# fabiojbg/LLMApiGateway

Measured on NVIDIA B200. Metric: sse_chunks_per_sec, higher is better.
Workload: dtype u8

## Files before the change

### llmapigateway_b200/csrc/lgw_engine.cu

```cuda
#include <cuda_runtime.h>
#include <stdio.h>
#include <string.h>
#include <string>
#include <vector>

#include "../../include/llmgw_b200.h"
#include "stream_machine.cuh"
#include "sse_kernels.cuh"
#include "rollup.cuh"
#include "body_kernels.cuh"
#include "doc_kernels.cuh"
#include "transcript.cuh"

using namespace lgw;

static_assert(sizeof(Val) == sizeof(lgw_val), "lgw_val layout");
static_assert(sizeof(UsageRec) == sizeof(lgw_usage_rec), "lgw_usage_rec layout");
static_assert(sizeof(StreamState) == sizeof(lgw_stream_state), "lgw_stream_state layout");
static_assert(sizeof(RowEvent) == sizeof(lgw_row_event), "lgw_row_event layout");
static_assert(sizeof(SegResult) == sizeof(lgw_seg_result), "lgw_seg_result layout");
static_assert(sizeof(RollupRow) == sizeof(lgw_rollup_row), "lgw_rollup_row layout");
static_assert(sizeof(DocUsage) == sizeof(lgw_doc_usage), "lgw_doc_usage layout");
static_assert(sizeof(TextMark) == sizeof(lgw_text_mark), "lgw_text_mark layout");

static thread_local std::string g_create_error;

struct lgw_engine {
    int device = 0;
    lgw_limits lim{};
    cudaStream_t own_stream = nullptr, stream = nullptr;
    cudaStream_t s_in = nullptr, s_out = nullptr;
    cudaEvent_t ev_in[16]{}, ev_k[16]{};
    DeviceTables t{};
    uint32_t* d_rowq_count = nullptr;
    RowEvent* d_rowq = nullptr;
    StepScratch scratch{};
    uint8_t *d_in = nullptr, *d_out = nullptr;
    uint32_t *d_chunk_off = nullptr, *d_seg_chunk = nullptr, *d_seg_slot = nullptr;
    SegResult* d_seg_out = nullptr;
    uint32_t* d_slots = nullptr; int32_t* d_status = nullptr; StreamState* d_state_stage = nullptr;
    cudaEvent_t ev[7]{};
    cudaEvent_t rev[4]{};
    float rms[2]{0, 0};
    RollupRow* d_rows = nullptr; uint64_t d_rows_cap = 0; unsigned long long* d_nrows = nullptr;
    uint8_t* d_partial = nullptr; size_t d_partial_cap = 0; uint32_t* d_tiles = nullptr; uint32_t d_tiles_cap = 0;
    bool rollup_attr_set = false, rollup_force_global = false;
    uint8_t* d_details = nullptr; size_t d_details_cap = 0;
    bool last_direct = false;
    float ms[5]{0, 0, 0, 0, 0};
    bool timed = false;
    uint64_t launches = 0;
    BodyPlan* d_plans = nullptr; BodyOp* d_ops = nullptr; uint8_t* d_blob = nullptr; uint32_t n_plans = 0, n_ops = 0;
    uint8_t *b_in = nullptr, *b_slots = nullptr, *b_out = nullptr, *b_models = nullptr;
    uint64_t *b_off = nullptr, *b_out_off = nullptr; uint32_t* b_plan_idx = nullptr; BodyResult* b_results = nullptr; BodyScan* b_scans = nullptr;
    uint64_t b_in_cap = 0, b_slots_cap = 0, b_out_cap = 0, b_n_cap = 0, b_models_cap = 0, b_redo_cap = 0;
    uint32_t* b_redo = nullptr;
    int body_mode = 0;
    cudaEvent_t bev[4]{};
    float bms[3]{0, 0, 0};
    bool per_kernel_timing = false;
    bool kernel_times_valid = false;
    int mode = 0;
    int sm_count = 148;
    bool text_on = false, text_pending = false, text_ready = false;
    TextTap* d_tap = nullptr; uint8_t* d_tcarry = nullptr; uint8_t* d_tsparse = nullptr; uint8_t* d_ttext = nullptr;
    uint32_t *d_piece_len = nullptr, *d_tseg_len = nullptr, *d_tseg_flags = nullptr, *d_markq_count = nullptr;
    unsigned long long* d_tseg_off = nullptr; TextMark* d_markq = nullptr;
    uint64_t text_total = 0; uint32_t text_marks = 0;
    cudaEvent_t tev[2]{}; float tms = 0;
    const uint8_t* last_bytes = nullptr; const uint32_t *last_chunk_off = nullptr, *last_seg_chunk = nullptr, *last_seg_slot = nullptr;
    const SegResult* last_seg_out = nullptr; uint32_t last_n_chunks = 0, last_n_segs = 0; uint64_t last_n_bytes = 0;
    std::string err;
};

#define CK(e, call) do { cudaError_t _r = (call); if (_r != cudaSuccess) { \
    (e)->err = std::string(#call) + ": " + cudaGetErrorString(_r); return LGW_ERR_CUDA; } } while (0)

extern "C" int lgw_abi_version(void) { return LGW_ABI_VERSION; }

extern "C" const char* lgw_last_error(const lgw_engine* e) { return e ? e->err.c_str() : g_create_error.c_str(); }

extern "C" int lgw_engine_create(int device, const lgw_limits* limits, lgw_engine** out) {
    if (!out || !limits) { g_create_error = "null argument"; return LGW_ERR_ARG; }
    int n = 0;
    if (cudaGetDeviceCount(&n) != cudaSuccess || n <= 0 || device < 0 || device >= n) {
        g_create_error = "no usable CUDA device (this engine has no CPU path)";
        return LGW_ERR_NO_DEVICE;
    }
    lgw_engine* e = new lgw_engine();
    e->device = device; e->lim = *limits;
    if (e->lim.max_streams == 0 || e->lim.carry_cap < 64 || e->lim.detail_cap < 64 || e->lim.max_step_chunks == 0 || e->lim.max_step_bytes == 0) {
        g_create_error = "limits out of range"; delete e; return LGW_ERR_ARG;
    }
    auto fail = [&](const char* what, cudaError_t r) { g_create_error = std::string(what) + ": " + cudaGetErrorString(r); lgw_engine_destroy(e); return LGW_ERR_CUDA; };
    cudaError_t r;
    if ((r = cudaSetDevice(device)) != cudaSuccess) return fail("cudaSetDevice", r);
    cudaDeviceProp prop;
    if ((r = cudaGetDeviceProperties(&prop, device)) != cudaSuccess) return fail("cudaGetDeviceProperties", r);
    e->sm_count = prop.multiProcessorCount;
    if ((r = cudaStreamCreateWithFlags(&e->own_stream, cudaStreamNonBlocking)) != cudaSuccess) return fail("cudaStreamCreate", r);
    e->stream = e->own_stream;
    if ((r = cudaStreamCreateWithFlags(&e->s_in, cudaStreamNonBlocking)) != cudaSuccess) return fail("cudaStreamCreate", r);
    if ((r = cudaStreamCreateWithFlags(&e->s_out, cudaStreamNonBlocking)) != cudaSuccess) return fail("cudaStreamCreate", r);
    for (int i = 0; i < 16; ++i) { if ((r = cudaEventCreateWithFlags(&e->ev_in[i], cudaEventDisableTiming)) != cudaSuccess) return fail("cudaEventCreate", r); if ((r = cudaEventCreateWithFlags(&e->ev_k[i], cudaEventDisableTiming)) != cudaSuccess) return fail("cudaEventCreate", r); }
    for (auto& ev : e->ev) if ((r = cudaEventCreate(&ev)) != cudaSuccess) return fail("cudaEventCreate", r);
    for (auto& ev : e->rev) if ((r = cudaEventCreate(&ev)) != cudaSuccess) return fail("cudaEventCreate", r);
    for (auto& ev : e->bev) if ((r = cudaEventCreate(&ev)) != cudaSuccess) return fail("cudaEventCreate", r);
    const size_t S = e->lim.max_streams, C = e->lim.max_step_chunks, B = e->lim.max_step_bytes;
#define ALLOC(ptr, bytes) if ((r = cudaMalloc((void**)&(ptr), (bytes))) != cudaSuccess) return fail("cudaMalloc " #ptr, r)
    ALLOC(e->t.state, S * sizeof(StreamState));
    ALLOC(e->t.carry_a, S * (size_t)e->lim.carry_cap);
    ALLOC(e->t.carry_b, S * (size_t)e->lim.carry_cap);
    ALLOC(e->t.detail, S * (size_t)e->lim.detail_cap);
    ALLOC(e->t.pending, S * (size_t)LGW_PENDING_STRIDE);
    e->t.carry_cap = e->lim.carry_cap; e->t.detail_cap = e->lim.detail_cap; e->t.max_streams = e->lim.max_streams;
    ALLOC(e->d_rowq, (size_t)(e->lim.rowq_cap + 1) * sizeof(RowEvent));
    ALLOC(e->d_rowq_count, 16);
    ALLOC(e->d_in, B + 64); ALLOC(e->d_out, B + 64);
    ALLOC(e->d_chunk_off, (C + 1) * 4); ALLOC(e->d_seg_chunk, (S + 1) * 4); ALLOC(e->d_seg_slot, S * 4);
    ALLOC(e->d_seg_out, S * sizeof(SegResult));
    ALLOC(e->d_slots, S * 4); ALLOC(e->d_status, S * 4); ALLOC(e->d_state_stage, S * sizeof(StreamState));
    if ((r = scratch_alloc(e->scratch, S, B, e->sm_count)) != cudaSuccess) return fail("scratch_alloc", r);
#undef ALLOC
    if ((r = cudaMemset(e->t.state, 0, S * sizeof(StreamState))) != cudaSuccess) return fail("cudaMemset", r);
    if ((r = cudaMemset(e->d_rowq_count, 0, 16)) != cudaSuccess) return fail("cudaMemset", r);
    const char* m = getenv("LGW_FORCE_GENERAL");
    e->mode = (m && m[0] == '1') ? 1 : 0;
    *out = e;
    return LGW_OK;
}

extern "C" int lgw_engine_destroy(lgw_engine* e) {
    if (!e) return LGW_OK;
    cudaSetDevice(e->device);
    cudaFree(e->t.state); cudaFree(e->t.carry_a); cudaFree(e->t.carry_b); cudaFree(e->t.detail); cudaFree(e->t.pending);
    cudaFree(e->d_rowq); cudaFree(e->d_rowq_count); cudaFree(e->d_in); cudaFree(e->d_out);
    cudaFree(e->d_chunk_off); cudaFree(e->d_seg_chunk); cudaFree(e->d_seg_slot); cudaFree(e->d_seg_out);
    cudaFree(e->d_slots); cudaFree(e->d_status); cudaFree(e->d_state_stage);
    scratch_free(e->scratch);
    for (auto& ev : e->ev) if (ev) cudaEventDestroy(ev);
    for (auto& ev : e->rev) if (ev) cudaEventDestroy(ev);
    cudaFree(e->d_rows); cudaFree(e->d_nrows); cudaFree(e->d_partial); cudaFree(e->d_tiles); cudaFree(e->d_details);
    cudaFree(e->d_plans); cudaFree(e->d_ops); cudaFree(e->d_blob);
    cudaFree(e->b_in); cudaFree(e->b_slots); cudaFree(e->b_out); cudaFree(e->b_models); cudaFree(e->b_off); cudaFree(e->b_out_off);
    cudaFree(e->b_plan_idx); cudaFree(e->b_results); cudaFree(e->b_scans); cudaFree(e->b_redo);
    for (auto& ev : e->bev) if (ev) cudaEventDestroy(ev);
    cudaFree(e->d_tap); cudaFree(e->d_tcarry); cudaFree(e->d_tsparse); cudaFree(e->d_ttext); cudaFree(e->d_piece_len); cudaFree(e->d_tseg_len);
    cudaFree(e->d_tseg_flags); cudaFree(e->d_markq_count); cudaFree(e->d_tseg_off); cudaFree(e->d_markq);
    for (auto& ev : e->tev) if (ev) cudaEventDestroy(ev);
    for (int i = 0; i < 16; ++i) { if (e->ev_in[i]) cudaEventDestroy(e->ev_in[i]); if (e->ev_k[i]) cudaEventDestroy(e->ev_k[i]); }
    if (e->s_in) cudaStreamDestroy(e->s_in);
    if (e->s_out) cudaStreamDestroy(e->s_out);
    if (e->own_stream) cudaStreamDestroy(e->own_stream);
    delete e;
    return LGW_OK;
}

extern "C" int lgw_engine_set_stream(lgw_engine* e, void* s) {
    if (!e) return LGW_ERR_ARG;
    e->stream = s ? (cudaStream_t)s : e->own_stream;
    return LGW_OK;
}

extern "C" int lgw_engine_set_kernel_timing(lgw_engine* e, int on) {
    if (!e) return LGW_ERR_ARG;
    e->per_kernel_timing = on != 0;
    return LGW_OK;
}

extern "C" int lgw_engine_set_mode(lgw_engine* e, int mode) {
    if (!e) return LGW_ERR_ARG;
    e->mode = mode; e->body_mode = mode;
    return LGW_OK;
}

extern "C" int lgw_streams_open(lgw_engine* e, const uint32_t* slots, const int32_t* http_status, uint32_t n) {
    if (!e || !slots || !http_status) return LGW_ERR_ARG;
    if (n == 0) return LGW_OK;
    if (n > e->lim.max_streams) { e->err = "more slots than max_streams"; return LGW_ERR_CAPACITY; }
    for (uint32_t i = 0; i < n; ++i) if (slots[i] >= e->lim.max_streams) { e->err = "slot out of range"; return LGW_ERR_ARG; }
    CK(e, cudaSetDevice(e->device));
    CK(e, cudaMemcpyAsync(e->d_slots, slots, n * 4, cudaMemcpyHostToDevice, e->stream));
    CK(e, cudaMemcpyAsync(e->d_status, http_status, n * 4, cudaMemcpyHostToDevice, e->stream));
    k_streams_open<<<(n + 127) / 128, 128, 0, e->stream>>>(e->t, e->d_slots, e->d_status, n);
    ++e->launches;
    if (e->text_on) { k_text_open<<<(n + 127) / 128, 128, 0, e->stream>>>(e->d_tap, e->d_slots, n); ++e->launches; }
    CK(e, cudaGetLastError());
    CK(e, cudaStreamSynchronize(e->stream));
    return LGW_OK;
}

static int gather_states(lgw_engine* e, const uint32_t* slots, uint32_t n, lgw_stream_state* out, int free_after) {
    if (!e || !slots || !out) return LGW_ERR_ARG;
    if (n == 0) return LGW_OK;
    if (n > e->lim.max_streams) { e->err = "more slots than max_streams"; return LGW_ERR_CAPACITY; }
    for (uint32_t i = 0; i < n; ++i) if (slots[i] >= e->lim.max_streams) { e->err = "slot out of range"; return LGW_ERR_ARG; }
    CK(e, cudaSetDevice(e->device));
    CK(e, cudaMemcpyAsync(e->d_slots, slots, n * 4, cudaMemcpyHostToDevice, e->stream));
    k_streams_gather<<<(n + 127) / 128, 128, 0, e->stream>>>(e->t, e->d_slots, n, e->d_state_stage, free_after);
    ++e->launches;
    CK(e, cudaGetLastError());
    CK(e, cudaMemcpyAsync(out, e->d_state_stage, n * sizeof(StreamState), cudaMemcpyDeviceToHost, e->stream));
    CK(e, cudaStreamSynchronize(e->stream));
    return LGW_OK;
}

extern "C" int lgw_streams_state(lgw_engine* e, const uint32_t* slots, uint32_t n, lgw_stream_state* out) { return gather_states(e, slots, n, out, 0); }
extern "C" int lgw_streams_close(lgw_engine* e, const uint32_t* slots, uint32_t n, lgw_stream_state* out) { return gather_states(e, slots, n, out, 1); }

extern "C" int lgw_stream_detail(lgw_engine* e, uint32_t slot, uint8_t* buf, uint32_t cap, uint32_t* len) {
    if (!e || !buf || !len || slot >= e->lim.max_streams) return LGW_ERR_ARG;
    CK(e, cudaSetDevice(e->device));
    StreamState st;
    CK(e, cudaMemcpyAsync(&st, e->t.state + slot, sizeof(st), cudaMemcpyDeviceToHost, e->stream));
    CK(e, cudaStreamSynchronize(e->stream));
    uint32_t n = st.h.detail_len < cap ? st.h.detail_len : cap;
    if (n) CK(e, cudaMemcpyAsync(buf, e->t.detail + (size_t)slot * e->lim.detail_cap, n, cudaMemcpyDeviceToHost, e->stream));
    CK(e, cudaStreamSynchronize(e->stream));
    *len = n;
    return LGW_OK;
}

namespace lgw {
__global__ void k_details_gather(DeviceTables t, const uint32_t* slots, uint32_t n, uint8_t* out, uint32_t stride, uint32_t* lens) {
    const uint32_t w = (blockIdx.x * blockDim.x + threadIdx.x) >> 5, lane = threadIdx.x & 31;
    if (w >= n) return;
    const uint32_t slot = slots[w];
    uint32_t len = t.state[slot].h.detail_len;
    if (len > t.detail_cap) len = t.detail_cap;
    if (len > stride) len = stride;
    const uint8_t* src = t.detail + (size_t)slot * t.detail_cap;
    uint8_t* dst = out + (size_t)w * stride;
    for (uint32_t i = lane; i < len; i += 32) dst[i] = src[i];
    if (lane == 0) lens[w] = len;
}
}

extern "C" int lgw_streams_details(lgw_engine* e, const uint32_t* slots, uint32_t n, uint8_t* buf, uint32_t stride, uint32_t* lens) {
    if (!e || (n && (!slots || !buf || !lens)) || stride == 0) return LGW_ERR_ARG;
    if (n == 0) return LGW_OK;
    for (uint32_t i = 0; i < n; ++i) if (slots[i] >= e->lim.max_streams) return LGW_ERR_ARG;
    CK(e, cudaSetDevice(e->device));
    const size_t need = (size_t)n * 8 + (size_t)n * stride;
    if (need > e->d_details_cap) {
        cudaFree(e->d_details); e->d_details = nullptr; e->d_details_cap = 0;
        CK(e, cudaMalloc((void**)&e->d_details, need + need / 2));
        e->d_details_cap = need + need / 2;
    }
    uint32_t* d_slots = (uint32_t*)e->d_details; uint32_t* d_lens = d_slots + n; uint8_t* d_out = e->d_details + (size_t)n * 8;
    CK(e, cudaMemcpyAsync(d_slots, slots, (size_t)n * 4, cudaMemcpyHostToDevice, e->stream));
    lgw::k_details_gather<<<(n * 32 + 255) / 256, 256, 0, e->stream>>>(e->t, d_slots, n, d_out, stride, d_lens);
    ++e->launches;
    CK(e, cudaMemcpyAsync(lens, d_lens, (size_t)n * 4, cudaMemcpyDeviceToHost, e->stream));
    CK(e, cudaMemcpyAsync(buf, d_out, (size_t)n * stride, cudaMemcpyDeviceToHost, e->stream));
    CK(e, cudaStreamSynchronize(e->stream));
    return LGW_OK;
}

static int step_device(lgw_engine* e, const uint8_t* d_bytes, uint64_t n_bytes, const uint32_t* d_chunk_off, uint32_t n_chunks,
                       const uint32_t* d_seg_chunk, const uint32_t* d_seg_slot, uint32_t n_segs,
                       uint8_t* d_out, SegResult* d_seg_out,
                       uint32_t s0 = 0, uint32_t s1 = 0xFFFFFFFFu, uint32_t c0 = 0, uint32_t c1 = 0xFFFFFFFFu,
                       uint32_t b0 = 0, uint64_t b1 = ~0ull, bool reset_rows = true) {
    if (n_segs > e->lim.max_streams || n_chunks > e->lim.max_step_chunks || n_bytes > e->lim.max_step_bytes) {
        e->err = "step exceeds the limits given to lgw_engine_create"; return LGW_ERR_CAPACITY;
    }
    if (n_bytes >= 0xFFFF0000ull) { e->err = "step larger than 4 GiB - 64 KiB"; return LGW_ERR_CAPACITY; }
    if (s1 == 0xFFFFFFFFu) { s1 = n_segs; c1 = n_chunks; b1 = n_bytes; }
    StepArgs a{};
    a.t = e->t; a.data = d_bytes; a.n_bytes = (uint32_t)b1; a.chunk_off = d_chunk_off; a.n_chunks = n_chunks;
    a.tile_base = b0; a.chunk_lo = c0; a.chunk_hi = c1;
    a.seg_chunk = d_seg_chunk + s0; a.seg_slot = d_seg_slot + s0; a.n_segs = s1 - s0; a.out = d_out; a.seg_out = d_seg_out + s0;
    a.rowq = e->d_rowq; a.rowq_count = e->d_rowq_count; a.rowq_cap = e->lim.rowq_cap; a.s = e->scratch;
    if (reset_rows) CK(e, cudaMemsetAsync(e->d_rowq_count, 0, 4, e->stream));
    int launched = 0;
    const bool pk = e->per_kernel_timing || e->mode == 1;
    cudaError_t r = launch_step(a, e->mode, e->sm_count, e->stream, e->ev, &launched, pk);
    e->kernel_times_valid = pk;
    e->launches += (uint64_t)launched;
    if (r != cudaSuccess) { e->err = std::string("step launch: ") + cudaGetErrorString(r); return LGW_ERR_CUDA; }
    e->timed = true;
    return LGW_OK;
}

extern "C" int lgw_sse_step_device(lgw_engine* e, const uint8_t* d_bytes, uint64_t n_bytes, const uint32_t* d_chunk_off, uint32_t n_chunks,
                                   const uint32_t* d_seg_chunk, const uint32_t* d_seg_slot, uint32_t n_segs,
                                   uint8_t* d_out, lgw_seg_result* d_seg_out) {
    if (!e || (!d_bytes && n_bytes) || !d_chunk_off || !d_seg_chunk || !d_seg_slot || (!d_out && n_bytes) || !d_seg_out) return LGW_ERR_ARG;
    CK(e, cudaSetDevice(e->device));
    e->last_bytes = d_bytes; e->last_n_bytes = n_bytes; e->last_chunk_off = d_chunk_off; e->last_n_chunks = n_chunks;
    e->last_seg_chunk = d_seg_chunk; e->last_seg_slot = d_seg_slot; e->last_n_segs = n_segs; e->last_seg_out = (const SegResult*)d_seg_out;
    e->text_pending = e->text_on; e->text_ready = false;
    return step_device(e, d_bytes, n_bytes, d_chunk_off, n_chunks, d_seg_chunk, d_seg_slot, n_segs, d_out, (SegResult*)d_seg_out);
}

extern "C" int lgw_fetch_rows(lgw_engine* e, lgw_row_event* rows_out, uint32_t rows_cap, uint32_t* n_rows) {
    if (!e || !n_rows || (!rows_out && rows_cap)) return LGW_ERR_ARG;
    CK(e, cudaSetDevice(e->device));
    uint32_t cnt = 0;
    CK(e, cudaMemcpyAsync(&cnt, e->d_rowq_count, 4, cudaMemcpyDeviceToHost, e->stream));
    CK(e, cudaStreamSynchronize(e->stream));
    if (cnt > e->lim.rowq_cap) cnt = e->lim.rowq_cap;
    if (cnt > rows_cap) cnt = rows_cap;
    if (cnt) CK(e, cudaMemcpyAsync(rows_out, e->d_rowq, (size_t)cnt * sizeof(RowEvent), cudaMemcpyDeviceToHost, e->stream));
    CK(e, cudaStreamSynchronize(e->stream));
    *n_rows = cnt;
    return LGW_OK;
}

extern "C" int lgw_sync(lgw_engine* e) {
    if (!e) return LGW_ERR_ARG;
    CK(e, cudaSetDevice(e->device));
    CK(e, cudaStreamSynchronize(e->stream));
    return LGW_OK;
}

extern "C" int lgw_sse_step(lgw_engine* e, const uint8_t* bytes, uint64_t n_bytes, const uint32_t* chunk_off, uint32_t n_chunks,
                            const uint32_t* seg_chunk, const uint32_t* seg_slot, uint32_t n_segs,
                            uint8_t* out_bytes, lgw_seg_result* seg_out, lgw_row_event* rows_out, uint32_t rows_cap, uint32_t* n_rows) {
    if (!e || (!bytes && n_bytes) || !chunk_off || !seg_chunk || !seg_slot || !seg_out || !n_rows) return LGW_ERR_ARG;
    if (n_segs > e->lim.max_streams || n_chunks > e->lim.max_step_chunks || n_bytes > e->lim.max_step_bytes) {
        e->err = "step exceeds the limits given to lgw_engine_create"; return LGW_ERR_CAPACITY;
    }
    if (chunk_off[0] != 0 || chunk_off[n_chunks] != n_bytes) { e->err = "chunk_off must start at 0 and end at n_bytes"; return LGW_ERR_ARG; }
    if (n_segs && (seg_chunk[0] != 0 || seg_chunk[n_segs] != n_chunks)) { e->err = "seg_chunk must cover all chunks"; return LGW_ERR_ARG; }
    for (uint32_t s = 0; s < n_segs; ++s) if (seg_chunk[s] > seg_chunk[s + 1] || seg_slot[s] >= e->lim.max_streams) { e->err = "bad segment table"; return LGW_ERR_ARG; }
    CK(e, cudaSetDevice(e->device));
    CK(e, cudaEventRecord(e->ev[5], e->stream));
    static const int allow = [] { const char* v = getenv("LGW_DIRECT"); if (!v || v[0] == '0') return 0; if (v[0] == 'b') return 3; if (v[0] == 'o') return 2; return 1; }();
    static const bool trace = [] { const char* v = getenv("LGW_TRACE"); return v && v[0] == '1'; }();
    const uint8_t* direct_in = nullptr; uint8_t* direct_out = nullptr;
    {
        cudaPointerAttributes pa{};
        const bool big = e->mode == 0 && n_bytes >= (1u << 20);
        if (big && (allow & 1) && ((uintptr_t)bytes & 15) == 0 && cudaPointerGetAttributes(&pa, bytes) == cudaSuccess && pa.type == cudaMemoryTypeHost && pa.devicePointer)
            direct_in = (const uint8_t*)pa.devicePointer;
        if (big && out_bytes && (allow & 2) && ((uintptr_t)out_bytes & 15) == 0 && cudaPointerGetAttributes(&pa, out_bytes) == cudaSuccess && pa.type == cudaMemoryTypeHost && pa.devicePointer)
            direct_out = (uint8_t*)pa.devicePointer;
        cudaGetLastError();
        e->last_direct = direct_in || direct_out;
    }
    e->last_bytes = direct_in ? direct_in : e->d_in; e->last_n_bytes = n_bytes; e->last_chunk_off = e->d_chunk_off; e->last_n_chunks = n_chunks;
    e->last_seg_chunk = e->d_seg_chunk; e->last_seg_slot = e->d_seg_slot; e->last_n_segs = n_segs; e->last_seg_out = e->d_seg_out;
    e->text_pending = e->text_on; e->text_ready = false;
    uint32_t n_slices = n_bytes >= (8u << 20) && n_segs >= 16 ? 8u : 1u;
    if (direct_in && direct_out) n_slices = 1;
    if (const char* sl = getenv("LGW_SLICES")) { int v = atoi(sl); if (v >= 1 && v <= 14) n_slices = (uint32_t)v; }
    if (e->mode == 1 || n_segs < n_slices) n_slices = 1;
    uint32_t cut[18]; cut[0] = 0;
    for (uint32_t j = 1; j < n_slices; ++j) {
        const uint64_t want = n_bytes * j / n_slices;
        uint32_t lo = cut[j - 1], hi = n_segs;
        while (lo < hi) { const uint32_t mid = (lo + hi) >> 1; if ((uint64_t)chunk_off[seg_chunk[mid]] < want) lo = mid + 1; else hi = mid; }
        cut[j] = lo;
    }
    cut[n_slices] = n_segs;
    CK(e, cudaMemsetAsync(e->d_rowq_count, 0, 4, e->stream));
    const bool piped = n_slices > 1;
    cudaStream_t sin = piped ? e->s_in : e->stream, sout = piped ? e->s_out : e->stream;
    if (piped) { CK(e, cudaEventRecord(e->ev_k[15], e->stream)); CK(e, cudaStreamWaitEvent(sin, e->ev_k[15], 0)); }
    {
        const uint32_t s1 = cut[1], c1 = seg_chunk[s1];
        CK(e, cudaMemcpyAsync(e->d_chunk_off, chunk_off, (size_t)(c1 + 1) * 4, cudaMemcpyHostToDevice, sin));
        CK(e, cudaMemcpyAsync(e->d_seg_chunk, seg_chunk, (size_t)(n_segs + 1) * 4, cudaMemcpyHostToDevice, sin));
        if (n_segs) CK(e, cudaMemcpyAsync(e->d_seg_slot, seg_slot, (size_t)n_segs * 4, cudaMemcpyHostToDevice, sin));
    }
    cudaEvent_t tr[3][16]; float tms[3][16];
    if (trace) for (int k = 0; k < 3; ++k) for (uint32_t j = 0; j < n_slices; ++j) cudaEventCreate(&tr[k][j]);
    int rc = LGW_OK;
    for (uint32_t j = 0; j < n_slices; ++j) {
        const uint32_t s0 = cut[j], s1 = cut[j + 1];
        if (s1 <= s0 && piped) continue;
        const uint32_t c0 = seg_chunk[s0], c1 = seg_chunk[s1];
        const uint32_t b0 = chunk_off[c0]; const uint64_t b1 = chunk_off[c1];
        if (!direct_in && b1 > b0) CK(e, cudaMemcpyAsync(e->d_in + b0, bytes + b0, b1 - b0, cudaMemcpyHostToDevice, sin));
        if (piped && (j == 0 || !direct_in)) { CK(e, cudaEventRecord(e->ev_in[j], sin)); CK(e, cudaStreamWaitEvent(e->stream, e->ev_in[j], 0)); }
        if (trace) cudaEventRecord(tr[0][j], sin);
        if (j == 0 && n_slices > 1 && n_chunks > seg_chunk[cut[1]]) {
            const uint32_t cc = seg_chunk[cut[1]];
            CK(e, cudaMemcpyAsync(e->d_chunk_off + cc + 1, chunk_off + cc + 1, (size_t)(n_chunks - cc) * 4, cudaMemcpyHostToDevice, sin));
            if (direct_in) { CK(e, cudaEventRecord(e->ev_in[1], sin)); CK(e, cudaStreamWaitEvent(e->stream, e->ev_in[1], 0)); }
        }
        rc = step_device(e, direct_in ? direct_in : e->d_in, n_bytes, e->d_chunk_off, n_chunks, e->d_seg_chunk, e->d_seg_slot, n_segs,
                         direct_out ? direct_out : e->d_out, e->d_seg_out, s0, s1, c0, c1, b0, b1, false);
        if (rc != LGW_OK) return rc;
        if (trace) cudaEventRecord(tr[1][j], e->stream);
        if (!direct_out) {
            if (piped) { CK(e, cudaEventRecord(e->ev_k[j], e->stream)); CK(e, cudaStreamWaitEvent(sout, e->ev_k[j], 0)); }
            if (b1 > b0 && out_bytes) CK(e, cudaMemcpyAsync(out_bytes + b0, e->d_out + b0, b1 - b0, cudaMemcpyDeviceToHost, sout));
        }
        if (trace) cudaEventRecord(tr[2][j], sout);
    }
    if (n_segs) CK(e, cudaMemcpyAsync(seg_out, e->d_seg_out, (size_t)n_segs * sizeof(SegResult), cudaMemcpyDeviceToHost, e->stream));
    if (piped) {
        CK(e, cudaEventRecord(e->ev_k[14], sout)); CK(e, cudaStreamWaitEvent(e->stream, e->ev_k[14], 0));
        CK(e, cudaEventRecord(e->ev_in[15], sin)); CK(e, cudaStreamWaitEvent(e->stream, e->ev_in[15], 0));
    }
    CK(e, cudaEventRecord(e->ev[6], e->stream));
    rc = lgw_fetch_rows(e, rows_out, rows_cap, n_rows);
    if (rc != LGW_OK) return rc;
    if (piped) { CK(e, cudaStreamSynchronize(e->s_out)); CK(e, cudaStreamSynchronize(e->s_in)); }
    float t = 0; if (cudaEventElapsedTime(&t, e->ev[5], e->ev[6]) == cudaSuccess) e->ms[4] = t;
    if (trace) {
        cudaDeviceSynchronize();
        fprintf(stderr, "[lgw trace] direct_in=%d direct_out=%d slices=%u total=%.3f ms; per slice (ms after step start): upload done | kernels done | download done\n", direct_in != nullptr, direct_out != nullptr, n_slices, t);
        for (uint32_t j = 0; j < n_slices; ++j) {
            for (int k = 0; k < 3; ++k) { tms[k][j] = -1; cudaEventElapsedTime(&tms[k][j], e->ev[5], tr[k][j]); cudaEventDestroy(tr[k][j]); }
            fprintf(stderr, "[lgw trace]   %2u  %.3f | %.3f | %.3f\n", j, tms[0][j], tms[1][j], tms[2][j]);
        }
        cudaGetLastError();
    }
    return LGW_OK;
}

static int read_step_ms(lgw_engine* e) {
    if (e->timed) {
        CK(e, cudaSetDevice(e->device));
        CK(e, cudaEventSynchronize(e->ev[4]));
        if (e->kernel_times_valid) {
            for (int i = 0; i < 4; ++i) { float t = 0; if (cudaEventElapsedTime(&t, e->ev[i], e->ev[i + 1]) == cudaSuccess) e->ms[i] = t; }
        } else {
            float t = 0; e->ms[0] = e->ms[2] = e->ms[3] = 0;
            if (cudaEventElapsedTime(&t, e->ev[0], e->ev[4]) == cudaSuccess) e->ms[1] = t;
        }
    }
    return LGW_OK;
}
extern "C" int lgw_last_step_ms(lgw_engine* e, float ms[4]) {
    if (!e || !ms) return LGW_ERR_ARG;
    const int rc = read_step_ms(e);
    if (rc != LGW_OK) return rc;
    ms[0] = e->ms[0]; ms[1] = e->ms[1]; ms[2] = e->ms[2] + e->ms[3]; ms[3] = e->ms[4];
    return LGW_OK;
}
extern "C" int lgw_last_step_kernel_ms(lgw_engine* e, float ms[4]) {
    if (!e || !ms) return LGW_ERR_ARG;
    const int rc = read_step_ms(e);
    if (rc != LGW_OK) return rc;
    for (int i = 0; i < 4; ++i) ms[i] = e->ms[i];
    return LGW_OK;
}

extern "C" int lgw_last_step_direct(lgw_engine* e) { return e && e->last_direct ? 1 : 0; }

extern "C" int lgw_launch_count(lgw_engine* e, uint64_t* out) {
    if (!e || !out) return LGW_ERR_ARG;
    *out = e->launches;
    return LGW_OK;
}

extern "C" int lgw_alloc_pinned(lgw_engine* e, uint64_t bytes, void** out) {
    if (!e || !out) return LGW_ERR_ARG;
    CK(e, cudaSetDevice(e->device));
    CK(e, cudaHostAlloc(out, bytes, cudaHostAllocDefault));
    return LGW_OK;
}
extern "C" int lgw_free_pinned(lgw_engine* e, void* p) {
    if (!e) return LGW_ERR_ARG;
    CK(e, cudaFreeHost(p));
    return LGW_OK;
}

extern "C" int64_t lgw_rollup_bucket_of(int64_t ts_us, int period) { return bucket_of(ts_us, period); }

extern "C" int lgw_usage_rollup_accum(lgw_engine* e, const int64_t* d_ts_us, const int32_t* d_model_rank,
                                      const int32_t* d_prompt, const int32_t* d_completion, const int32_t* d_total,
                                      const int32_t* d_reasoning, const int32_t* d_cached, const double* d_cost, uint64_t n,
                                      int period, int has_start, int64_t start_us, int has_end, int64_t end_us,
                                      int64_t bucket0, uint32_t n_buckets, uint32_t n_models,
                                      uint64_t* d_table, uint32_t* d_inexact, uint32_t* d_oob) {
    if (!e || !d_table || !d_inexact || !d_oob || period < 0 || period > 3 || n_buckets == 0 || n_models == 0) return LGW_ERR_ARG;
    if (n && (!d_ts_us || !d_model_rank || !d_prompt || !d_completion || !d_total || !d_reasoning || !d_cached || !d_cost)) return LGW_ERR_ARG;
    CK(e, cudaSetDevice(e->device));
    RollupArgs a{};
    a.ts_us = d_ts_us; a.model_rank = d_model_rank; a.tok[0] = d_prompt; a.tok[1] = d_completion; a.tok[2] = d_total;
    a.tok[3] = d_reasoning; a.tok[4] = d_cached; a.cost = d_cost; a.n = n; a.period = period;
    a.start_us = start_us; a.end_us = end_us; a.has_start = has_start; a.has_end = has_end;
    a.bucket0 = bucket0; a.n_buckets = n_buckets; a.n_models = n_models;
    a.table = (unsigned long long*)d_table; a.inexact = d_inexact; a.oob = d_oob;
    const uint64_t groups = (uint64_t)n_buckets * n_models;
    const bool privatised = groups <= LGW_ROLLUP_SMEM_GROUPS && n >= 65536 && n < 0xFFFFFFFFull && !e->rollup_force_global;
    if (privatised) {
        const size_t need = (size_t)e->sm_count * groups * (LGW_ROLLUP_CELLS * 8 + 4);
        if (need > e->d_partial_cap) {
            cudaFree(e->d_partial); e->d_partial = nullptr; e->d_partial_cap = 0;
            CK(e, cudaMalloc((void**)&e->d_partial, need));
            e->d_partial_cap = need;
        }
        if (!e->rollup_attr_set) {
            CK(e, cudaFuncSetAttribute(k_rollup_accum_smem, cudaFuncAttributeMaxDynamicSharedMemorySize, (int)rollup_smem_bytes(LGW_ROLLUP_SMEM_GROUPS)));
            e->rollup_attr_set = true;
        }
    }
    CK(e, cudaEventRecord(e->rev[0], e->stream));
    if (n && privatised) {
        const unsigned grid = (unsigned)e->sm_count;
        unsigned long long* partial = (unsigned long long*)e->d_partial;
        uint32_t* pflag = (uint32_t*)(e->d_partial + (size_t)grid * groups * LGW_ROLLUP_CELLS * 8);
        k_rollup_accum_smem<<<grid, 1024, rollup_smem_bytes((uint32_t)groups), e->stream>>>(a, partial, pflag);
        k_rollup_merge<<<dim3((unsigned)((groups * LGW_ROLLUP_CELLS + 255) / 256), LGW_ROLLUP_MERGE_SLICES), 256, 0, e->stream>>>(partial, pflag, grid, (uint32_t)groups, a.table, a.inexact);
        e->launches += 2;
    } else if (n) {
        const uint64_t want = (n + 255) / 256;
        const unsigned grid = (unsigned)(want < (uint64_t)e->sm_count * 16 ? want : (uint64_t)e->sm_count * 16);
        k_rollup_accum<<<grid, 256, 0, e->stream>>>(a);
        ++e->launches;
    }
    CK(e, cudaEventRecord(e->rev[1], e->stream));
    CK(e, cudaGetLastError());
    return LGW_OK;
}

extern "C" int lgw_usage_rollup_emit(lgw_engine* e, const uint64_t* d_table, const uint32_t* d_inexact,
                                     int64_t bucket0, uint32_t n_buckets, uint32_t n_models,
                                     lgw_rollup_row* rows_out, uint64_t rows_cap, uint64_t* n_rows) {
    if (!e || !d_table || !d_inexact || !n_rows || (!rows_out && rows_cap) || n_buckets == 0 || n_models == 0) return LGW_ERR_ARG;
    CK(e, cudaSetDevice(e->device));
    const uint64_t groups = (uint64_t)n_buckets * n_models;
    const uint64_t cap = rows_cap < groups ? rows_cap : groups;
    if (cap > e->d_rows_cap) {
        cudaFree(e->d_rows); e->d_rows = nullptr; e->d_rows_cap = 0;
        CK(e, cudaMalloc((void**)&e->d_rows, (cap ? cap : 1) * sizeof(RollupRow)));
        e->d_rows_cap = cap;
    }
    if (!e->d_nrows) CK(e, cudaMalloc((void**)&e->d_nrows, 8));
    const uint32_t n_tiles = (uint32_t)((groups + 1023) / 1024);
    if (n_tiles > e->d_tiles_cap) {
        cudaFree(e->d_tiles); e->d_tiles = nullptr; e->d_tiles_cap = 0;
        CK(e, cudaMalloc((void**)&e->d_tiles, (size_t)n_tiles * 4));
        e->d_tiles_cap = n_tiles;
    }
    CK(e, cudaEventRecord(e->rev[2], e->stream));
    k_rollup_count<<<n_tiles, 1024, 0, e->stream>>>((const unsigned long long*)d_table, n_buckets, n_models, e->d_tiles);
    k_rollup_scan<<<1, 1024, 0, e->stream>>>(e->d_tiles, n_tiles, e->d_nrows);
    k_rollup_write<<<n_tiles, 1024, 0, e->stream>>>((const unsigned long long*)d_table, d_inexact, n_buckets, n_models, bucket0, e->d_tiles, e->d_rows, cap);
    e->launches += 3;
    CK(e, cudaEventRecord(e->rev[3], e->stream));
    CK(e, cudaGetLastError());
    unsigned long long cnt = 0;
    CK(e, cudaMemcpyAsync(&cnt, e->d_nrows, 8, cudaMemcpyDeviceToHost, e->stream));
    CK(e, cudaStreamSynchronize(e->stream));
    *n_rows = cnt;
    const uint64_t take = cnt < cap ? cnt : cap;
    if (take) CK(e, cudaMemcpyAsync(rows_out, e->d_rows, take * sizeof(RollupRow), cudaMemcpyDeviceToHost, e->stream));
    CK(e, cudaStreamSynchronize(e->stream));
    return LGW_OK;
}

extern "C" int lgw_rollup_set_path(lgw_engine* e, int force_global) {
    if (!e) return LGW_ERR_ARG;
    e->rollup_force_global = force_global != 0;
    return LGW_OK;
}

extern "C" int lgw_rollup_last_ms(lgw_engine* e, float ms[2]) {
    if (!e || !ms) return LGW_ERR_ARG;
    CK(e, cudaSetDevice(e->device));
    cudaEventSynchronize(e->rev[1]); cudaEventSynchronize(e->rev[3]);
    float t = 0;
    if (cudaEventElapsedTime(&t, e->rev[0], e->rev[1]) == cudaSuccess) e->rms[0] = t;
    if (cudaEventElapsedTime(&t, e->rev[2], e->rev[3]) == cudaSuccess) e->rms[1] = t;
    ms[0] = e->rms[0]; ms[1] = e->rms[1];
    return LGW_OK;
}

extern "C" int lgw_transcripts_enable(lgw_engine* e) {
    if (!e) return LGW_ERR_ARG;
    if (e->text_on) return LGW_OK;
    CK(e, cudaSetDevice(e->device));
    const size_t S = e->lim.max_streams, C = e->lim.max_step_chunks, B = e->lim.max_step_bytes, cc = e->lim.carry_cap;
    CK(e, cudaMalloc((void**)&e->d_tap, S * sizeof(TextTap)));
    CK(e, cudaMemset(e->d_tap, 0, S * sizeof(TextTap)));
    CK(e, cudaMalloc((void**)&e->d_tcarry, S * cc));
    CK(e, cudaMalloc((void**)&e->d_tsparse, 2 * (B + S * cc) + 64));
    CK(e, cudaMalloc((void**)&e->d_ttext, 2 * (B + S * cc) + 64));
    CK(e, cudaMalloc((void**)&e->d_piece_len, (C + 1) * 4));
    CK(e, cudaMalloc((void**)&e->d_tseg_len, (S + 1) * 4));
    CK(e, cudaMalloc((void**)&e->d_tseg_flags, (S + 1) * 4));
    CK(e, cudaMalloc((void**)&e->d_tseg_off, (S + 2) * 8));
    CK(e, cudaMalloc((void**)&e->d_markq, (size_t)(e->lim.rowq_cap + 1) * sizeof(TextMark)));
    CK(e, cudaMalloc((void**)&e->d_markq_count, 16));
    for (auto& ev : e->tev) CK(e, cudaEventCreate(&ev));
    e->text_on = true;
    return LGW_OK;
}

extern "C" int lgw_step_transcript_run(lgw_engine* e, uint64_t* text_bytes, uint32_t* n_marks) {
    if (!e || !text_bytes || !n_marks) return LGW_ERR_ARG;
    if (!e->text_on) { e->err = "transcripts are not enabled (lgw_transcripts_enable)"; return LGW_ERR_ARG; }
    if (!e->text_pending) { e->err = "no step to tap (the transcript pass runs once after each lgw_sse_step / lgw_sse_step_device)"; return LGW_ERR_ARG; }
    CK(e, cudaSetDevice(e->device));
    e->text_pending = false;
    TextArgs a{};
    a.data = e->last_bytes; a.chunk_off = e->last_chunk_off; a.seg_chunk = e->last_seg_chunk; a.seg_slot = e->last_seg_slot; a.n_segs = e->last_n_segs;
    a.seg_res = e->last_seg_out; a.tap = e->d_tap; a.carry = e->d_tcarry; a.carry_cap = e->lim.carry_cap; a.sparse = e->d_tsparse;
    a.piece_len = e->d_piece_len; a.seg_len = e->d_tseg_len; a.seg_flags = e->d_tseg_flags; a.seg_off = e->d_tseg_off; a.text = e->d_ttext;
    a.markq = e->d_markq; a.markq_count = e->d_markq_count; a.markq_cap = e->lim.rowq_cap;
    CK(e, cudaMemsetAsync(e->d_markq_count, 0, 4, e->stream));
    CK(e, cudaEventRecord(e->tev[0], e->stream));
    const uint32_t n = a.n_segs;
    if (n) {
        k_text_extract<<<(n + TX_WARPS - 1) / TX_WARPS, TX_WARPS * 32, 0, e->stream>>>(a);
        k_text_scan<<<1, 1024, 0, e->stream>>>(a.seg_len, n, a.seg_off);
        k_text_pack<<<(n + TX_WARPS - 1) / TX_WARPS, TX_WARPS * 32, 0, e->stream>>>(a);
        e->launches += 3;
    } else CK(e, cudaMemsetAsync(e->d_tseg_off, 0, 8, e->stream));
    CK(e, cudaEventRecord(e->tev[1], e->stream));
    CK(e, cudaGetLastError());
    unsigned long long total = 0; uint32_t marks = 0;
    CK(e, cudaMemcpyAsync(&total, e->d_tseg_off + n, 8, cudaMemcpyDeviceToHost, e->stream));
    CK(e, cudaMemcpyAsync(&marks, e->d_markq_count, 4, cudaMemcpyDeviceToHost, e->stream));
    CK(e, cudaStreamSynchronize(e->stream));
    if (marks > e->lim.rowq_cap) marks = e->lim.rowq_cap;
    e->text_total = total; e->text_marks = marks; e->text_ready = true;
    float t = 0; if (cudaEventElapsedTime(&t, e->tev[0], e->tev[1]) == cudaSuccess) e->tms = t;
    *text_bytes = total; *n_marks = marks;
    return LGW_OK;
}

extern "C" int lgw_step_transcript_fetch(lgw_engine* e, uint8_t* text_out, uint64_t* seg_text_off, uint32_t* seg_flags, lgw_text_mark* marks_out) {
    if (!e || !seg_text_off || !seg_flags || (!text_out && e->text_total) || (!marks_out && e->text_marks)) return LGW_ERR_ARG;
    if (!e->text_ready) { e->err = "lgw_step_transcript_run has not run for the last step"; return LGW_ERR_ARG; }
    CK(e, cudaSetDevice(e->device));
    const uint32_t n = e->last_n_segs;
    if (e->text_total) CK(e, cudaMemcpyAsync(text_out, e->d_ttext, e->text_total, cudaMemcpyDeviceToHost, e->stream));
    CK(e, cudaMemcpyAsync(seg_text_off, e->d_tseg_off, (size_t)(n + 1) * 8, cudaMemcpyDeviceToHost, e->stream));
    if (n) CK(e, cudaMemcpyAsync(seg_flags, e->d_tseg_flags, (size_t)n * 4, cudaMemcpyDeviceToHost, e->stream));
    if (e->text_marks) CK(e, cudaMemcpyAsync(marks_out, e->d_markq, (size_t)e->text_marks * sizeof(TextMark), cudaMemcpyDeviceToHost, e->stream));
    CK(e, cudaStreamSynchronize(e->stream));
    return LGW_OK;
}

extern "C" int lgw_transcript_last_ms(lgw_engine* e, float* ms) {
    if (!e || !ms) return LGW_ERR_ARG;
    *ms = e->tms;
    return LGW_OK;
}

extern "C" int lgw_device_alloc(lgw_engine* e, uint64_t bytes, void** out) {
    if (!e || !out) return LGW_ERR_ARG;
    CK(e, cudaSetDevice(e->device));
    CK(e, cudaMalloc(out, bytes ? bytes : 1));
    return LGW_OK;
}
extern "C" int lgw_device_free(lgw_engine* e, void* p) { if (!e) return LGW_ERR_ARG; CK(e, cudaSetDevice(e->device)); CK(e, cudaFree(p)); return LGW_OK; }
extern "C" int lgw_device_upload(lgw_engine* e, void* d, const void* h, uint64_t bytes) {
    if (!e || (bytes && (!d || !h))) return LGW_ERR_ARG;
    CK(e, cudaSetDevice(e->device));
    CK(e, cudaMemcpyAsync(d, h, bytes, cudaMemcpyHostToDevice, e->stream)); CK(e, cudaStreamSynchronize(e->stream));
    return LGW_OK;
}
extern "C" int lgw_device_download(lgw_engine* e, void* h, const void* d, uint64_t bytes) {
    if (!e || (bytes && (!d || !h))) return LGW_ERR_ARG;
    CK(e, cudaSetDevice(e->device));
    CK(e, cudaMemcpyAsync(h, d, bytes, cudaMemcpyDeviceToHost, e->stream)); CK(e, cudaStreamSynchronize(e->stream));
    return LGW_OK;
}
extern "C" int lgw_device_zero(lgw_engine* e, void* d, uint64_t bytes) {
    if (!e || (bytes && !d)) return LGW_ERR_ARG;
    CK(e, cudaSetDevice(e->device));
    CK(e, cudaMemsetAsync(d, 0, bytes, e->stream));
    return LGW_OK;
}

#ifdef LGW_DEBUG_TIMING
extern "C" int lgw_debug_read(unsigned long long* out) { return cudaMemcpyFromSymbol(out, lgw::g_dbg, sizeof(unsigned long long) * 16) == cudaSuccess ? 0 : -2; }
#endif


static_assert(sizeof(BodyOp) == sizeof(lgw_body_op), "lgw_body_op");
static_assert(sizeof(BodyPlan) == sizeof(lgw_body_plan), "lgw_body_plan");
static_assert(sizeof(BodyResult) == sizeof(lgw_body_result), "lgw_body_result");
static_assert(sizeof(BodyScan) == sizeof(lgw_body_scan), "lgw_body_scan");

template <class T>
static cudaError_t grow(T*& p, uint64_t& cap, uint64_t need) {
    if (need <= cap && p) return cudaSuccess;
    if (p) { cudaError_t r = cudaFree(p); p = nullptr; cap = 0; if (r != cudaSuccess) return r; }
    const uint64_t n = need + need / 4 + 64;
    cudaError_t r = cudaMalloc((void**)&p, n * sizeof(T));
    if (r == cudaSuccess) cap = n;
    return r;
}

extern "C" int lgw_rules_load(lgw_engine* e, const lgw_body_plan* plans, uint32_t n_plans,
                              const lgw_body_op* ops, uint32_t n_ops, const uint8_t* blob, uint32_t blob_len) {
    if (!e || (n_plans && !plans) || (n_ops && !ops) || (blob_len && !blob)) return LGW_ERR_ARG;
    for (uint32_t i = 0; i < n_plans; ++i) {
        if (plans[i].op_begin > plans[i].op_end || plans[i].op_end > n_ops || plans[i].op_end - plans[i].op_begin > 32 || (plans[i].mode & 0xffu) > 2 || (plans[i].mode & ~0x1ffu)) {
            e->err = "lgw_rules_load: malformed plan"; return LGW_ERR_ARG; }
    }
    for (uint32_t i = 0; i < n_ops; ++i) {
        const lgw_body_op& o = ops[i];
        if ((uint64_t)o.key_off + o.key_len > blob_len || (uint64_t)o.rkey_off + o.rkey_len > blob_len || (uint64_t)o.rval_off + o.rval_len > blob_len) {
            e->err = "lgw_rules_load: op outside the blob"; return LGW_ERR_ARG; }
    }
    CK(e, cudaSetDevice(e->device));
    CK(e, cudaStreamSynchronize(e->stream));
    cudaFree(e->d_plans); cudaFree(e->d_ops); cudaFree(e->d_blob); e->d_plans = nullptr; e->d_ops = nullptr; e->d_blob = nullptr;
    CK(e, cudaMalloc((void**)&e->d_plans, (n_plans + 1) * sizeof(BodyPlan)));
    CK(e, cudaMalloc((void**)&e->d_ops, (n_ops + 1) * sizeof(BodyOp)));
    CK(e, cudaMalloc((void**)&e->d_blob, blob_len + 16));
    if (n_plans) CK(e, cudaMemcpyAsync(e->d_plans, plans, n_plans * sizeof(BodyPlan), cudaMemcpyHostToDevice, e->stream));
    if (n_ops) CK(e, cudaMemcpyAsync(e->d_ops, ops, n_ops * sizeof(BodyOp), cudaMemcpyHostToDevice, e->stream));
    if (blob_len) CK(e, cudaMemcpyAsync(e->d_blob, blob, blob_len, cudaMemcpyHostToDevice, e->stream));
    CK(e, cudaStreamSynchronize(e->stream));
    e->n_plans = n_plans; e->n_ops = n_ops;
    return LGW_OK;
}

static int bodies_stage_in(lgw_engine* e, const uint8_t* bodies, const uint64_t* body_off, uint32_t n) {
    const uint64_t n_bytes = body_off[n];
    for (uint32_t i = 0; i < n; ++i) if (body_off[i + 1] < body_off[i] || body_off[i + 1] - body_off[i] > 0xFFFFFFF0ull) { e->err = "body offsets not monotonic"; return LGW_ERR_ARG; }
    CK(e, grow(e->b_in, e->b_in_cap, n_bytes + 64));
    uint64_t ncap = e->b_n_cap;
    if (n + 1 > e->b_n_cap || !e->b_off) {
        uint64_t c1 = e->b_n_cap, c2 = e->b_n_cap, c3 = e->b_n_cap, c4 = e->b_n_cap, c5 = e->b_n_cap;
        CK(e, grow(e->b_off, c1, n + 1)); CK(e, grow(e->b_out_off, c2, n + 1)); CK(e, grow(e->b_plan_idx, c3, n + 1));
        CK(e, grow(e->b_results, c4, n + 1)); CK(e, grow(e->b_scans, c5, n + 1));
        ncap = c1;
    }
    e->b_n_cap = ncap;
    if (n_bytes) CK(e, cudaMemcpyAsync(e->b_in, bodies, n_bytes, cudaMemcpyHostToDevice, e->stream));
    CK(e, cudaMemcpyAsync(e->b_off, body_off, (n + 1) * sizeof(uint64_t), cudaMemcpyHostToDevice, e->stream));
    return LGW_OK;
}

extern "C" int lgw_bodies_scan(lgw_engine* e, const uint8_t* bodies, const uint64_t* body_off, uint32_t n,
                               uint32_t model_cap, lgw_body_scan* scans_out, uint8_t* models_out) {
    if (!e || !body_off || (!bodies && n && body_off[n]) || !scans_out || (model_cap && !models_out)) return LGW_ERR_ARG;
    if (n == 0) return LGW_OK;
    CK(e, cudaSetDevice(e->device));
    int rc = bodies_stage_in(e, bodies, body_off, n);
    if (rc != LGW_OK) return rc;
    CK(e, grow(e->b_models, e->b_models_cap, (uint64_t)n * model_cap + 16));
    k_body_scan<<<(n + LGW_BODY_WARPS - 1) / LGW_BODY_WARPS, 32 * LGW_BODY_WARPS, 0, e->stream>>>(e->b_in, e->b_off, n, model_cap, e->b_scans, e->b_models);
    ++e->launches;
    CK(e, cudaGetLastError());
    CK(e, cudaMemcpyAsync(scans_out, e->b_scans, n * sizeof(BodyScan), cudaMemcpyDeviceToHost, e->stream));
    if (model_cap) CK(e, cudaMemcpyAsync(models_out, e->b_models, (uint64_t)n * model_cap, cudaMemcpyDeviceToHost, e->stream));
    CK(e, cudaStreamSynchronize(e->stream));
    return LGW_OK;
}

static int bodies_launch(lgw_engine* e, const uint8_t* d_bodies, const uint64_t* d_body_off, uint32_t n, const uint32_t* d_plan_idx,
                         uint32_t slot_cap, uint8_t* d_out, uint64_t out_cap, uint64_t* d_out_off, BodyResult* d_results) {
    if (!e->d_plans) { e->err = "lgw_bodies_rewrite before lgw_rules_load"; return LGW_ERR_ARG; }
    CK(e, grow(e->b_slots, e->b_slots_cap, (uint64_t)n * slot_cap + 64));
    CK(e, grow(e->b_redo, e->b_redo_cap, (uint64_t)n + 4));
    uint32_t* redo_count = e->b_redo + n;
    const uint32_t seq_grid = (n + LGW_BODY_WARPS - 1) / LGW_BODY_WARPS < (uint32_t)e->sm_count * 4u ? (n + LGW_BODY_WARPS - 1) / LGW_BODY_WARPS : (uint32_t)e->sm_count * 4u;
    CK(e, cudaEventRecord(e->bev[0], e->stream));
    if (e->body_mode == 0) {
        CK(e, cudaMemsetAsync(redo_count, 0, 4, e->stream));
        k_body_fast<<<n, LGW_FAST_THREADS, 0, e->stream>>>(d_bodies, d_body_off, n, d_plan_idx, e->d_plans, e->n_plans, e->d_ops, e->d_blob,
                                                             e->b_slots, slot_cap, d_results, redo_count, e->b_redo);
        k_body_rewrite<<<seq_grid, 32 * LGW_BODY_WARPS, 0, e->stream>>>(d_bodies, d_body_off, n, d_plan_idx, e->d_plans, e->n_plans, e->d_ops, e->d_blob,
                                                                        e->b_slots, slot_cap, d_results, redo_count, e->b_redo);
        ++e->launches;
    } else {
        k_body_rewrite<<<seq_grid, 32 * LGW_BODY_WARPS, 0, e->stream>>>(d_bodies, d_body_off, n, d_plan_idx, e->d_plans, e->n_plans, e->d_ops, e->d_blob,
                                                                        e->b_slots, slot_cap, d_results, nullptr, nullptr);
    }
    CK(e, cudaEventRecord(e->bev[1], e->stream));
    k_body_offsets<<<1, 1024, 0, e->stream>>>(d_results, n, out_cap, d_out_off);
    CK(e, cudaEventRecord(e->bev[2], e->stream));
    const uint32_t grid = n < (uint32_t)e->sm_count * 8u ? n : (uint32_t)e->sm_count * 8u;
    k_body_pack<<<grid, 256, 0, e->stream>>>(e->b_slots, slot_cap, d_results, n, d_out_off, d_out, out_cap);
    CK(e, cudaEventRecord(e->bev[3], e->stream));
    e->launches += 3;
    CK(e, cudaGetLastError());
    return LGW_OK;
}

extern "C" int lgw_bodies_rewrite_device(lgw_engine* e, const uint8_t* d_bodies, const uint64_t* d_body_off, uint32_t n, uint64_t n_bytes,
                                         const uint32_t* d_plan_idx, uint32_t slot_cap, uint8_t* d_out, uint64_t out_cap,
                                         uint64_t* d_out_off, lgw_body_result* d_results) {
    (void)n_bytes;
    if (!e || !d_bodies || !d_body_off || !d_plan_idx || !d_out || !d_out_off || !d_results || slot_cap == 0) return LGW_ERR_ARG;
    if (n == 0) return LGW_OK;
    CK(e, cudaSetDevice(e->device));
    return bodies_launch(e, d_bodies, d_body_off, n, d_plan_idx, slot_cap, d_out, out_cap, d_out_off, (BodyResult*)d_results);
}

extern "C" int lgw_bodies_rewrite(lgw_engine* e, const uint8_t* bodies, const uint64_t* body_off, uint32_t n,
                                  const uint32_t* plan_idx, uint32_t slot_cap,
                                  uint8_t* out, uint64_t out_cap, uint64_t* out_off, lgw_body_result* results) {
    if (!e || !body_off || (!bodies && n && body_off[n]) || !plan_idx || (!out && out_cap) || !out_off || !results || slot_cap == 0) return LGW_ERR_ARG;
    if (n == 0) { out_off[0] = 0; return LGW_OK; }
    CK(e, cudaSetDevice(e->device));
    int rc = bodies_stage_in(e, bodies, body_off, n);
    if (rc != LGW_OK) return rc;
    CK(e, cudaMemcpyAsync(e->b_plan_idx, plan_idx, n * sizeof(uint32_t), cudaMemcpyHostToDevice, e->stream));
    CK(e, grow(e->b_out, e->b_out_cap, out_cap + 64));
    rc = bodies_launch(e, e->b_in, e->b_off, n, e->b_plan_idx, slot_cap, e->b_out, out_cap, e->b_out_off, e->b_results);
    if (rc != LGW_OK) return rc;
    CK(e, cudaMemcpyAsync(out_off, e->b_out_off, (n + 1) * sizeof(uint64_t), cudaMemcpyDeviceToHost, e->stream));
    CK(e, cudaMemcpyAsync(results, e->b_results, n * sizeof(BodyResult), cudaMemcpyDeviceToHost, e->stream));
    CK(e, cudaStreamSynchronize(e->stream));
    const uint64_t total = out_off[n] < out_cap ? out_off[n] : out_cap;
    if (total) CK(e, cudaMemcpyAsync(out, e->b_out, total, cudaMemcpyDeviceToHost, e->stream));
    CK(e, cudaStreamSynchronize(e->stream));
    return LGW_OK;
}

extern "C" int lgw_documents_usage(lgw_engine* e, const uint8_t* docs, const uint64_t* doc_off, uint32_t n, lgw_doc_usage* out) {
    if (!e || !doc_off || (!docs && n && doc_off[n]) || (!out && n)) return LGW_ERR_ARG;
    if (n == 0) return LGW_OK;
    CK(e, cudaSetDevice(e->device));
    int rc = bodies_stage_in(e, docs, doc_off, n);
    if (rc != LGW_OK) return rc;
    DocUsage* d_out = nullptr;
    CK(e, cudaMalloc((void**)&d_out, (size_t)n * sizeof(DocUsage)));
    const uint32_t grid = (n + LGW_DOC_WARPS - 1) / LGW_DOC_WARPS < (uint32_t)e->sm_count * 8u ? (n + LGW_DOC_WARPS - 1) / LGW_DOC_WARPS : (uint32_t)e->sm_count * 8u;
    k_docs_usage<<<grid, LGW_DOC_WARPS * 32, 0, e->stream>>>(e->b_in, e->b_off, n, d_out);
    ++e->launches;
    cudaError_t r = cudaGetLastError();
    if (r == cudaSuccess) r = cudaMemcpyAsync(out, d_out, (size_t)n * sizeof(DocUsage), cudaMemcpyDeviceToHost, e->stream);
    if (r == cudaSuccess) r = cudaStreamSynchronize(e->stream);
    cudaFree(d_out);
    if (r != cudaSuccess) { e->err = std::string("lgw_documents_usage: ") + cudaGetErrorString(r); return LGW_ERR_CUDA; }
    return LGW_OK;
}

extern "C" int lgw_documents_error_detail(lgw_engine* e, const uint8_t* docs, const uint64_t* doc_off, uint32_t n, lgw_doc_error* out, uint8_t* text, uint32_t text_stride) {
    if (!e || !doc_off || (!docs && n && doc_off[n]) || (n && (!out || !text)) || text_stride == 0) return LGW_ERR_ARG;
    if (n == 0) return LGW_OK;
    CK(e, cudaSetDevice(e->device));
    int rc = bodies_stage_in(e, docs, doc_off, n);
    if (rc != LGW_OK) return rc;
    DocError* d_out = nullptr; uint8_t* d_text = nullptr;
    CK(e, cudaMalloc((void**)&d_out, (size_t)n * sizeof(DocError)));
    cudaError_t r = cudaMalloc((void**)&d_text, (size_t)n * text_stride);
    if (r == cudaSuccess) {
        const uint32_t grid = (n + LGW_DOC_WARPS - 1) / LGW_DOC_WARPS < (uint32_t)e->sm_count * 8u ? (n + LGW_DOC_WARPS - 1) / LGW_DOC_WARPS : (uint32_t)e->sm_count * 8u;
        k_docs_error_detail<<<grid, LGW_DOC_WARPS * 32, 0, e->stream>>>(e->b_in, e->b_off, n, d_out, d_text, text_stride);
        ++e->launches;
        r = cudaGetLastError();
    }
    if (r == cudaSuccess) r = cudaMemcpyAsync(out, d_out, (size_t)n * sizeof(DocError), cudaMemcpyDeviceToHost, e->stream);
    if (r == cudaSuccess) r = cudaMemcpyAsync(text, d_text, (size_t)n * text_stride, cudaMemcpyDeviceToHost, e->stream);
    if (r == cudaSuccess) r = cudaStreamSynchronize(e->stream);
    cudaFree(d_out); cudaFree(d_text);
    if (r != cudaSuccess) { e->err = std::string("lgw_documents_error_detail: ") + cudaGetErrorString(r); return LGW_ERR_CUDA; }
    return LGW_OK;
}

extern "C" int lgw_bodies_last_ms(lgw_engine* e, float ms[3]) {
    if (!e || !ms) return LGW_ERR_ARG;
    CK(e, cudaSetDevice(e->device));
    cudaEventSynchronize(e->bev[3]);
    for (int i = 0; i < 3; ++i) { float t = 0; if (cudaEventElapsedTime(&t, e->bev[i], e->bev[i + 1]) == cudaSuccess) e->bms[i] = t; ms[i] = e->bms[i]; }
    return LGW_OK;
}

extern "C" int lgw_debug_counters(lgw_engine* e, uint32_t out[4]) {
    if (!e || !out) return LGW_ERR_ARG;
    CK(e, cudaSetDevice(e->device));
    CK(e, cudaStreamSynchronize(e->stream));
    CK(e, cudaMemcpy(out, e->scratch.counters, 16, cudaMemcpyDeviceToHost));
    return LGW_OK;
}

extern "C" int lgw_debug_template_cache(lgw_engine* e, uint32_t out[16], uint8_t* text, uint32_t cap) {
    if (!e || !out) return LGW_ERR_ARG;
    CK(e, cudaSetDevice(e->device));
    CK(e, cudaStreamSynchronize(e->stream));
    std::vector<uint8_t> buf(sizeof(TemplateCache2));
    CK(e, cudaMemcpy(buf.data(), e->scratch.tpl_cache2, sizeof(TemplateCache2), cudaMemcpyDeviceToHost));
    const TemplateCache2* h = reinterpret_cast<const TemplateCache2*>(buf.data());
    for (int i = 0; i < 4; ++i) { out[i] = h->state[i]; out[4 + i] = h->tpl[i].m.len; out[8 + i] = h->tpl[i].m.flags | (h->tpl[i].m.usage_ok << 31); out[12 + i] = h->hits[i]; }
    if (cap > R2_TEXT) cap = R2_TEXT;
    if (text) for (int i = 0; i < 4; ++i) memcpy(text + (size_t)i * cap, h->tpl[i].text, cap);
    return LGW_OK;
}
```

### llmapigateway_b200/csrc/relay2.cuh

```cuda
#pragma once

#if defined(__CUDACC__)
#define R2_DEV __device__ __forceinline__
#define R2_MEM __device__ __forceinline__
#define R2_DEV_NOINLINE __device__ __noinline__
#define R2_GLOBAL __global__
#define R2_TID (threadIdx.x)
#define R2_BID (blockIdx.x)
#define R2_NBLK (gridDim.x)
#define R2_NTHR (blockDim.x)
#define R2_HOST_EMU 0
#else
#define R2_DEV static inline
#define R2_MEM inline
#define R2_DEV_NOINLINE static
#define R2_GLOBAL static
#define R2_TID (simt::tid())
#define R2_BID (simt::bid())
#define R2_NBLK (simt::nblocks())
#define R2_NTHR (simt::nthreads())
#define R2_HOST_EMU 1
#endif

#ifndef R2_WARPS
#define R2_WARPS 16u
#endif
#define R2_THREADS (R2_WARPS * 32u)
#ifndef R2_TILE
#define R2_TILE 3072u
#endif
#ifndef R2_NBUF
#define R2_NBUF 2u
#endif
#define R2_SLOTS 4u
#define R2_TPL_MAX 504u
#define R2_TPL_MIN 16u
#define R2_TEXT 544u
#define R2_SPANS 32u
#define R2_FULL 0xFFFFFFFFu
#define R2_NONE 0xFFFFFFFFu
#define R2_MAX_STR 8192u

struct TplMeta {
    uint32_t len, P, recip, flags, cls, n_spans, usage_ok, full_flags;
    uint16_t sstart[R2_SPANS], send[R2_SPANS];
    uint8_t skind[R2_SPANS];
    uint8_t field_span[8];
};
struct Tpl2 {
    TplMeta m;
    uint8_t text[R2_TEXT];
    uint8_t lit[R2_TEXT];
    uint8_t span_id[R2_TPL_MAX + 8];
};
struct TemplateCache2 {
    uint32_t state[R2_SLOTS];
    uint32_t hits[R2_SLOTS];
    uint32_t general;
    uint32_t lock;
    uint32_t _pad[2];
    Tpl2 tpl[R2_SLOTS];
    UsageRaw raw[R2_SLOTS];
};

struct R2Shared {
    alignas(16) uint8_t fast_text[16 * R2_TEXT];
    alignas(16) uint8_t fast_lit[16 * R2_TEXT];
    alignas(16) Tpl2 tpl[R2_SLOTS];
    alignas(8) UsageRaw raw_tpl[R2_SLOTS];
    alignas(8) unsigned long long mbar[R2_WARPS * R2_NBUF];
    uint32_t slot_state[R2_SLOTS];
    uint32_t slot_gidx[R2_SLOTS];
    uint32_t hits[R2_SLOTS];
    uint32_t general;
    uint32_t dflt, fast_ready;
    uint32_t learn_lock;
    StepArgs args;
    alignas(4) uint8_t cls[256];
    alignas(4) uint8_t trans[LGW_LEAN_ROWS * 32];
};
#define R2_RING_BYTES (R2_WARPS * R2_NBUF * R2_TILE)
#define R2_SMEM_BYTES (R2_RING_BYTES + sizeof(R2Shared) + 128)

#if !R2_HOST_EMU
typedef uint32_t SPtr;
R2_DEV SPtr sptr(const void* p) { return (uint32_t)__cvta_generic_to_shared(p); }
R2_DEV uint4 sld128(SPtr a) { uint4 v; asm volatile("ld.shared.v4.u32 {%0,%1,%2,%3}, [%4];" : "=r"(v.x), "=r"(v.y), "=r"(v.z), "=r"(v.w) : "r"(a)); return v; }
R2_DEV uint32_t sld32(SPtr a) { uint32_t v; asm volatile("ld.shared.u32 %0, [%1];" : "=r"(v) : "r"(a)); return v; }
R2_DEV uint32_t sld8(SPtr a) { uint32_t v; asm volatile("ld.shared.u8 %0, [%1];" : "=r"(v) : "r"(a)); return v; }
R2_DEV void sst8(SPtr a, uint32_t v) { asm volatile("st.shared.u8 [%0], %1;" :: "r"(a), "r"(v) : "memory"); }
R2_DEV uint4 gld128(const uint8_t* p) { uint4 v; asm volatile("ld.global.nc.v4.u32 {%0,%1,%2,%3}, [%4];" : "=r"(v.x), "=r"(v.y), "=r"(v.z), "=r"(v.w) : "l"(p)); return v; }
R2_DEV void mbar_init(SPtr a, uint32_t n) { asm volatile("mbarrier.init.shared::cta.b64 [%0], %1;" :: "r"(a), "r"(n)); }
R2_DEV void mbar_fence_init() { asm volatile("fence.mbarrier_init.release.cluster;" ::: "memory"); }
R2_DEV void mbar_expect(SPtr a, uint32_t bytes) { asm volatile("mbarrier.arrive.expect_tx.shared::cta.b64 _, [%0], %1;" :: "r"(a), "r"(bytes) : "memory"); }
R2_DEV void mbar_wait(SPtr a, uint32_t parity) {
    asm volatile("{\n.reg .pred p;\nWAIT_%=:\nmbarrier.try_wait.parity.shared::cta.b64 p, [%0], %1;\n@p bra DONE_%=;\nbra WAIT_%=;\nDONE_%=:\n}" :: "r"(a), "r"(parity) : "memory");
}
R2_DEV void tma_load(SPtr dst, const void* src, uint32_t bytes, SPtr mbar) {
    asm volatile("cp.async.bulk.shared::cluster.global.mbarrier::complete_tx::bytes [%0], [%1], %2, [%3];" :: "r"(dst), "l"(src), "r"(bytes), "r"(mbar) : "memory");
}
R2_DEV void tma_store(void* dst, SPtr src, uint32_t bytes) {
    asm volatile("fence.proxy.async.shared::cta;\ncp.async.bulk.global.shared::cta.bulk_group [%0], [%1], %2;\ncp.async.bulk.commit_group;" :: "l"(dst), "r"(src), "r"(bytes) : "memory");
}
R2_DEV void tma_store_commit_empty() { asm volatile("cp.async.bulk.commit_group;" ::: "memory"); }
R2_DEV void tma_wait_read1() { asm volatile("cp.async.bulk.wait_group.read 1;" ::: "memory"); }
R2_DEV void tma_wait_all() { asm volatile("cp.async.bulk.wait_group 0;" ::: "memory"); }
R2_DEV uint8_t* smem_base() { extern __shared__ __align__(128) uint8_t r2_smem[]; return r2_smem; }
R2_DEV void griddep_wait() { asm volatile("griddepcontrol.wait;" ::: "memory"); }
R2_DEV void griddep_launch() { asm volatile("griddepcontrol.launch_dependents;" ::: "memory"); }
#else
typedef uint8_t* SPtr;
R2_DEV SPtr sptr(const void* p) { return (uint8_t*)p; }
R2_DEV uint4 sld128(SPtr a) { uint4 v; memcpy(&v, a, 16); return v; }
R2_DEV uint32_t sld32(SPtr a) { uint32_t v; memcpy(&v, a, 4); return v; }
R2_DEV uint32_t sld8(SPtr a) { return *a; }
R2_DEV void sst8(SPtr a, uint32_t v) { *a = (uint8_t)v; }
R2_DEV uint4 gld128(const uint8_t* p) { uint4 v; memcpy(&v, p, 16); return v; }
R2_DEV void mbar_init(SPtr a, uint32_t) { memset(a, 0, 8); }
R2_DEV void mbar_fence_init() {}
R2_DEV void mbar_expect(SPtr, uint32_t) {}
R2_DEV void mbar_wait(SPtr, uint32_t) {}
R2_DEV void tma_load(SPtr dst, const void* src, uint32_t bytes, SPtr) { memcpy(dst, src, bytes); }
R2_DEV void tma_store(void* dst, SPtr src, uint32_t bytes) { memcpy(dst, src, bytes); }
R2_DEV void tma_store_commit_empty() {}
R2_DEV void tma_wait_read1() {}
R2_DEV void tma_wait_all() {}
R2_DEV uint8_t* smem_base() { return simt::g_dyn_smem; }
R2_DEV void griddep_wait() {}
R2_DEV void griddep_launch() {}
#endif
R2_DEV uint32_t r2_min(uint32_t a, uint32_t b) { return a < b ? a : b; }
R2_DEV uint32_t r2_max(uint32_t a, uint32_t b) { return a > b ? a : b; }

R2_DEV uint32_t span_ok(uint32_t w, uint32_t m) {
    const uint32_t w7 = w & 0x7f7f7f7fu;
    const uint32_t a = w7 + 0x60606060u;
    const uint32_t b = (w7 ^ 0x22222222u) + 0x7f7f7f7fu;
    const uint32_t c = (w7 ^ 0x5c5c5c5cu) + 0x7f7f7f7fu;
    return (a & b & c) | w | m;
}
R2_DEV uint32_t nonzero_bytes(uint32_t x) { return (((x & 0x7f7f7f7fu) + 0x7f7f7f7fu) | x) & 0x80808080u; }
R2_DEV uint32_t movemask4(uint32_t m) { return (((m >> 7) * 0x00204081u) >> 21) & 0xFu; }
R2_DEV uint32_t lf_mask16(const uint4& d) {
    const uint32_t a = ~nonzero_bytes(d.x ^ 0x0a0a0a0au) & 0x80808080u, b = ~nonzero_bytes(d.y ^ 0x0a0a0a0au) & 0x80808080u;
    const uint32_t c = ~nonzero_bytes(d.z ^ 0x0a0a0a0au) & 0x80808080u, e = ~nonzero_bytes(d.w ^ 0x0a0a0a0au) & 0x80808080u;
    return movemask4(a) | (movemask4(b) << 4) | (movemask4(c) << 8) | (movemask4(e) << 12);
}

struct R2Ctx {
    const StepArgs* a;
    R2Shared* sh;
    uint32_t lane;
    SPtr ring; SPtr bars;
    uint32_t base;
    uint32_t n_tiles;
    uint32_t k;
    uint32_t tile_lo, tile_hi;
    SPtr buf;
    uint32_t n_bytes;
    uint32_t seg, tb, te, kept_end;
    uint32_t in_kept, primed, kept_tried;
    uint32_t ev_a, ev_b, a_usage;
    uint32_t high;
    uint32_t walk_lo;
    uint32_t t, pos, s_open;
    uint32_t dflt, fast;
    uint32_t ready, free_slots;
    uint32_t last_ra;
    uint32_t hits_d;
    uint32_t single;
};

struct R2Io {
    const uint8_t* data; const R2Shared* sh;
    uint32_t n_bytes, tile_lo, tile_hi; SPtr buf;
};
R2_DEV R2Io io_of(const R2Ctx& c) { R2Io io; io.data = c.a->data; io.sh = c.sh; io.n_bytes = c.n_bytes; io.tile_lo = c.tile_lo; io.tile_hi = c.tile_hi; io.buf = c.buf; return io; }
R2_DEV uint8_t io_byte(const R2Io& io, uint32_t p) {
    if (p >= io.tile_lo && p < io.tile_hi) return (uint8_t)sld8(io.buf + (p - io.tile_lo));
    return p < io.n_bytes ? __ldg(io.data + p) : (uint8_t)0;
}
R2_DEV uint8_t ring_byte(const R2Ctx& c, uint32_t p) {
    if (p >= c.tile_lo && p < c.tile_hi) return (uint8_t)sld8(c.buf + (p - c.tile_lo));
    return p < c.n_bytes ? __ldg(c.a->data + p) : (uint8_t)0;
}
struct R2Bytes {
    R2Io io;
    R2_MEM uint32_t at(uint32_t p) const { return io_byte(io, p); }
    R2_MEM uint32_t cls(uint32_t ch) const { return io.sh->cls[ch]; }
    R2_MEM uint32_t trans(uint32_t i) const { return io.sh->trans[i]; }
};
struct R2Glob {
    const uint8_t* data; uint32_t n_bytes;
    R2_MEM uint32_t at(uint32_t p) const { return p < n_bytes ? (uint32_t)__ldg(data + p) : 0u; }
};
R2_DEV uint4 ld16(const R2Ctx& c, uint32_t p) {
    if (p >= c.tile_lo && p + 16 <= c.tile_hi) return sld128(c.buf + (p - c.tile_lo));
    if (p + 16 <= c.n_bytes) return gld128(c.a->data + p);
    uint32_t w0 = 0, w1 = 0, w2 = 0, w3 = 0;
    for (uint32_t i = 0; i < 16 && p + i < c.n_bytes; ++i) {
        const uint32_t v = (uint32_t)ring_byte(c, p + i) << (8 * (i & 3));
        if (i < 4) w0 |= v; else if (i < 8) w1 |= v; else if (i < 12) w2 |= v; else w3 |= v;
    }
    return make_uint4(w0, w1, w2, w3);
}

R2_DEV uint32_t tile_bytes(const R2Ctx& c, uint32_t k) {
    const uint32_t lo = c.base + k * R2_TILE;
    return c.n_bytes - lo < R2_TILE ? c.n_bytes - lo : R2_TILE;
}
R2_DEV void pipe_issue_load(const R2Ctx& c, uint32_t k) {
    const uint32_t b = k % R2_NBUF, n16 = tile_bytes(c, k) & ~15u;
    if (n16) { mbar_expect(c.bars + 8 * b, n16); tma_load(c.ring + b * R2_TILE, c.a->data + c.base + k * R2_TILE, n16, c.bars + 8 * b); }
}
R2_DEV void pipe_start(R2Ctx& c) {
    c.k = R2_NONE; c.tile_lo = c.tile_hi = c.base; c.buf = c.ring;
    if (c.lane == 0) for (uint32_t k = 0; k < R2_NBUF - 1 && k < c.n_tiles; ++k) pipe_issue_load(c, k);
}
struct PipeState { uint32_t k, tile_lo, tile_hi; SPtr buf; };
R2_DEV PipeState pipe_advance_impl(const StepArgs* ap, SPtr ring, SPtr bars, uint32_t base, uint32_t n_tiles, uint32_t n_bytes, uint32_t k_prev, uint32_t lane) {
    const uint32_t k = k_prev == R2_NONE ? 0u : k_prev + 1u;
    __syncwarp();
    const uint32_t lo = base + k * R2_TILE;
    const uint32_t b = k % R2_NBUF, nb = n_bytes - lo < R2_TILE ? n_bytes - lo : R2_TILE, n16 = nb & ~15u;
    PipeState ps; ps.k = k; ps.tile_lo = lo; ps.tile_hi = lo + nb; ps.buf = ring + b * R2_TILE;
    if (n16) mbar_wait(bars + 8 * b, (k / R2_NBUF) & 1u);
    if (nb != n16) {
        const uint32_t i = n16 + lane;
        if (lane < 16) {
            const uint32_t v = i < nb ? (uint32_t)__ldg(ap->data + lo + i) : 0u;
            sst8(ps.buf + i, v);
            if (i < nb) ap->out[lo + i] = (uint8_t)v;
        }
        __syncwarp();
    }
    if (lane == 0) {
        if (n16) tma_store(ap->out + lo, ps.buf, n16); else tma_store_commit_empty();
        tma_wait_read1();
        const uint32_t kn = k + R2_NBUF - 1;
        if (kn < n_tiles) {
            const uint32_t bn = kn % R2_NBUF, lon = base + kn * R2_TILE, nn = (n_bytes - lon < R2_TILE ? n_bytes - lon : R2_TILE) & ~15u;
            if (nn) { mbar_expect(bars + 8 * bn, nn); tma_load(ring + bn * R2_TILE, ap->data + lon, nn, bars + 8 * bn); }
        }
    }
    return ps;
}
R2_DEV void pipe_advance(R2Ctx& c) {
    const PipeState ps = pipe_advance_impl(c.a, c.ring, c.bars, c.base, c.n_tiles, c.n_bytes, c.k, c.lane);
    c.k = ps.k; c.tile_lo = ps.tile_lo; c.tile_hi = ps.tile_hi; c.buf = ps.buf;
}

R2_DEV void build_fast_tables(R2Shared* sh, uint32_t slot, uint32_t lane, uint32_t step) {
    const Tpl2& tp = sh->tpl[slot];
    const uint32_t P = tp.m.P, recip = tp.m.recip;
    for (uint32_t i4 = lane; i4 < 16 * R2_TEXT / 4; i4 += step) {
        const uint32_t i = i4 * 4u, cpy = i / R2_TEXT, j = i - cpy * R2_TEXT;
        uint32_t x = j + cpy; x -= __umulhi(x, recip) * P;
        uint32_t wt = 0, wl = 0;
        for (uint32_t b = 0; b < 4; ++b) { wt |= (uint32_t)tp.text[x] << (8 * b); wl |= (uint32_t)tp.lit[x] << (8 * b); if (++x == P) x = 0; }
        reinterpret_cast<uint32_t*>(sh->fast_text)[i4] = wt; reinterpret_cast<uint32_t*>(sh->fast_lit)[i4] = wl;
    }
}

template <class RD>
R2_DEV_NOINLINE bool build_template2(const RD& rd, Tpl2* tp, UsageRaw* raw_out, uint32_t ps, uint32_t limit) {
    uint32_t cls = PC_NONE;
    const uint32_t c0 = rd.at(ps);
    if (c0 == '{') cls = PC_BRACE;
    else if (c0 == 'd' && rd.at(ps + 1) == 'a' && rd.at(ps + 2) == 't' && rd.at(ps + 3) == 'a' && rd.at(ps + 4) == ':' && rd.at(ps + 5) == ' ' && rd.at(ps + 6) == '{') cls = PC_DATA;
    if (cls == PC_NONE) return false;
    TplMeta& m = tp->m;
    LeanMachine lm;
    lm.reset(cls == PC_DATA);
    const uint32_t skip = cls == PC_DATA ? 6u : 0u;
    for (uint32_t k = 0; k < R2_TPL_MAX + 8; ++k) tp->span_id[k] = 0xff;
    for (uint32_t k = 0; k < R2_TEXT; ++k) tp->lit[k] = 0xff;
    uint32_t pos = ps + skip, n_ids = 0, cur_s = 0xff, cur_n = 0xff;
    for (;;) {
        if (pos + 1 >= limit || pos - ps >= R2_TPL_MAX) return false;
        const uint32_t c = rd.at(pos);
        if (c == '\n' && rd.at(pos + 1) == '\n') break;
        const uint32_t prev = lm.st;
        const bool in_str = (prev == L_STR || prev == L_STR_ESC || prev == L_STR_U) && !lm.in_key;
        const bool in_num = prev >= L_NUM_MINUS && prev <= L_NUM_EXP;
        const uint32_t x = pos - ps;
        if (in_str && cur_s != 0xff) {
            tp->span_id[x] = (uint8_t)cur_s;
            if (prev == L_STR && c == '"') m.send[cur_s] = (uint16_t)x;
            else tp->lit[x] = 0x00;
        }
        lm.step(c, pos, rd);
        const bool now_num = lm.st >= L_NUM_MINUS && lm.st <= L_NUM_EXP;
        if (in_num && cur_n != 0xff) {
            tp->span_id[x] = (uint8_t)cur_n;
            if (!now_num) { m.send[cur_n] = (uint16_t)x; cur_n = 0xff; }
        }
        if (prev < LGW_LEAN_ROWS && lm.st == L_STR && !lm.in_key) {
            cur_s = n_ids < R2_SPANS ? n_ids++ : 0xffu;
            if (cur_s != 0xff) { m.skind[cur_s] = 0; m.sstart[cur_s] = (uint16_t)(x + 1); m.send[cur_s] = 0xffff; }
        }
        if (!in_num && now_num) {
            cur_n = n_ids < R2_SPANS ? n_ids++ : 0xffu;
            if (cur_n != 0xff) { m.skind[cur_n] = 1; m.sstart[cur_n] = (uint16_t)x; m.send[cur_n] = 0xffff; tp->span_id[x] = (uint8_t)cur_n; }
        }
        if (lm.st == L_ERR) return false;
        ++pos;
    }
    const uint32_t f = lm.finish();
    if (!(f & PF_VALID_A) || (f & (TK_ERROR | TK_DETAIL | TK_CODE))) return false;
    if (pos + 2 < limit && rd.at(pos + 2) == '\n') return false;
    const uint32_t len = pos - ps;
    if (len < R2_TPL_MIN) return false;
    for (uint32_t k = 0; k < n_ids; ++k) if (m.send[k] >= len) return false;
    const uint32_t P = len + 2;
    for (uint32_t k = 0; k < R2_TEXT; ++k) {
        uint32_t x = k; while (x >= P) x -= P;
        tp->text[k] = x < len ? (uint8_t)rd.at(ps + x) : (uint8_t)'\n';
        if (k >= len) tp->lit[k] = x < len ? tp->lit[x] : (uint8_t)0xff;
    }
    m.len = len; m.P = P; m.recip = (uint32_t)((0x100000000ull + P - 1) / P); m.flags = f; m.cls = cls; m.n_spans = n_ids;
    m.usage_ok = 0; m.full_flags = 0;
    for (uint32_t k = 0; k < 8; ++k) m.field_span[k] = 0xff;
    if (f & TK_USAGE) {
        JsonMachine<true> jm; ValueTrack trk; trk.reset();
        jm.reset(raw_out, cls == PC_DATA); jm.trk = &trk;
        for (uint32_t i = skip; i < len; ++i) { trk.pos = i; jm.feed(rd.at(ps + i)); if (jm.failed()) break; }
        const uint32_t ff = jm.finish();
        m.full_flags = ff;
        bool ok = !jm.failed() && (ff & PF_VALID_B) && !(ff & PF_EXOTIC) && !((ff & TK_CHOICES) && (ff & PF_TYPE_ERROR)) && !trk.dup && n_ids <= R2_SPANS;
        if (ok && (ff & TK_CHOICES)) for (uint32_t k = 0; k < n_ids; ++k) if (m.send[k] >= trk.choices_lo && m.sstart[k] <= trk.choices_hi) ok = false;
        for (uint32_t fi = 0; ok && fi < UF_N; ++fi) {
            if (trk.fstart[fi] == 0xFFFFFFFFu) continue;
            if (trk.fstart[fi] == 0xFFFFFFFEu) { ok = false; break; }
            uint32_t j = 0xff;
            for (uint32_t k = 0; k < n_ids; ++k) {
                if (m.skind[k] == 1 && m.sstart[k] == trk.fstart[fi] && m.send[k] == trk.fend[fi]) j = k;
                if (m.skind[k] == 0 && (uint32_t)m.sstart[k] == trk.fstart[fi] + 1 && (uint32_t)m.send[k] + 1 == trk.fend[fi]) j = k;
            }
            if (j != 0xff && (m.skind[j] == 1) != (fi < UF_MODEL)) ok = false;
            m.field_span[fi] = (uint8_t)j;
            if (j == 0xff) for (uint32_t k = 0; k < n_ids; ++k) if (m.sstart[k] < trk.fend[fi] && m.send[k] >= trk.fstart[fi]) ok = false;
        }
        m.usage_ok = ok ? 1u : 0u;
    }
    return true;
}

template <class RD>
R2_DEV_NOINLINE Val parse_number_span(const RD& rd, uint32_t p, uint32_t n) {
    DecAcc num; num.reset();
    uint32_t i = 0;
    if (i < n && rd.at(p) == '-') { num.neg = 1; ++i; }
    for (; i < n; ++i) { const uint32_t c = rd.at(p + i); if (c - '0' >= 10u) break; num.digit(c - '0', false); }
    if (i < n && rd.at(p + i) == '.') { ++i; for (; i < n; ++i) { const uint32_t c = rd.at(p + i); if (c - '0' >= 10u) break; num.is_float = 1; num.digit(c - '0', true); } }
    if (i < n && (rd.at(p + i) | 0x20u) == 'e') {
        num.is_float = 1; ++i;
        if (i < n && rd.at(p + i) == '+') ++i; else if (i < n && rd.at(p + i) == '-') { num.exp_neg = 1; ++i; }
        for (; i < n; ++i) num.exp_digit(rd.at(p + i) - '0');
    }
    uint8_t kind; int64_t bits; bool truthy;
    num.finish(kind, bits, truthy);
    Val v; v.kind = kind; v.bits = bits;
    return v;
}
template <class RD>
R2_DEV_NOINLINE void decode_string_span(const RD& rd, uint32_t p, uint32_t n, char* dst, uint8_t& dlen, uint8_t& dflags) {
    uint32_t len = 0, flags = 0, pending_high = 0;
    auto put = [&](uint32_t b) { if (len < LGW_STR_CAP) dst[len++] = (char)b; else flags |= 1; };
    auto put_cp = [&](uint32_t cp) {
        if (cp < 0x80) put(cp);
        else if (cp < 0x800) { put(0xC0 | (cp >> 6)); put(0x80 | (cp & 63)); }
        else if (cp < 0x10000) { put(0xE0 | (cp >> 12)); put(0x80 | ((cp >> 6) & 63)); put(0x80 | (cp & 63)); }
        else { put(0xF0 | (cp >> 18)); put(0x80 | ((cp >> 12) & 63)); put(0x80 | ((cp >> 6) & 63)); put(0x80 | (cp & 63)); }
    };
    auto flush_high = [&]() { if (pending_high) { flags |= 2; pending_high = 0; } };
    for (uint32_t i = 0; i < n; ++i) {
        uint32_t c = rd.at(p + i);
        if (c != '\\') { flush_high(); put(c); continue; }
        const uint32_t e = rd.at(p + ++i);
        if (e != 'u') { c = e == 'b' ? 8u : e == 'f' ? 12u : e == 'n' ? 10u : e == 'r' ? 13u : e == 't' ? 9u : e; flush_high(); put(c); continue; }
        uint32_t cp = 0;
        for (int d = 0; d < 4; ++d) { const uint32_t h = rd.at(p + ++i); cp = (cp << 4) | (h - '0' < 10u ? h - '0' : (h | 0x20u) - 'a' + 10u); }
        if (cp < 0x80) { flush_high(); put(cp); }
        else if (cp >= 0xD800 && cp <= 0xDBFF) { flush_high(); pending_high = cp; }
        else if (cp >= 0xDC00 && cp <= 0xDFFF) { if (pending_high) { put_cp(0x10000 + ((pending_high - 0xD800) << 10) + (cp - 0xDC00)); pending_high = 0; } else flags |= 2; }
        else { flush_high(); put_cp(cp); }
    }
    flush_high();
    dlen = (uint8_t)len; dflags = (uint8_t)flags;
}

R2_DEV void flush_counts(R2Ctx& c) {
    if (c.lane == 0 && c.seg != R2_NONE) {
        SegPlan* pl = c.a->s.plan + c.seg;
        if (c.ev_a) atomicAdd(&pl->n_events_a, c.ev_a);
        if (c.ev_b) atomicAdd(&pl->n_events_b, c.ev_b);
        if (c.a_usage) pl->a_usage = 1;
    }
    c.ev_a = c.ev_b = c.a_usage = 0;
}
R2_DEV void mark_irregular(R2Ctx& c) { if (c.lane == 0 && c.seg != R2_NONE) c.a->s.plan[c.seg].irregular = 1; }

R2_DEV_NOINLINE bool chunks_utf8_ok(const StepArgs* ap, uint32_t lane, uint32_t seg, uint32_t lo, uint32_t hi) {
    const StepArgs& a = *ap;
    uint32_t c0 = __ldg(a.seg_chunk + seg), c1 = __ldg(a.seg_chunk + seg + 1);
    {
        uint32_t l = c0, h = c1;
        while (l < h) { const uint32_t mid = (l + h) >> 1; if (__ldg(a.chunk_off + mid + 1) <= lo) l = mid + 1; else h = mid; }
        c0 = l;
    }
    bool ok = true;
    for (uint32_t ch = c0 + lane; ch < c1; ch += 32) {
        const uint32_t o = __ldg(a.chunk_off + ch), e = __ldg(a.chunk_off + ch + 1);
        if (o >= hi) break;
        if (e > a.n_bytes) { ok = false; break; }
        if (!utf8_valid(a.data + o, e - o)) ok = false;
    }
    return __all_sync(R2_FULL, ok);
}

R2_DEV uint32_t find_lflf(R2Ctx& c, uint32_t from, uint32_t end, uint32_t& high) {
    uint32_t wb = from & ~15u;
    for (;;) {
        if (wb >= end) return R2_NONE;
        const uint32_t lp = wb + 16 * c.lane;
        const uint4 d = lp < end ? ld16(c, lp) : make_uint4(0, 0, 0, 0);
        high |= d.x | d.y | d.z | d.w;
        const uint32_t lf = lf_mask16(d);
        const uint32_t nxt = __shfl_down_sync(R2_FULL, lf, 1);
        uint32_t pair = lf & ((lf >> 1) | ((c.lane < 31 ? nxt & 1u : 0u) << 15));
        if (lp < from) pair &= from - lp >= 16 ? 0u : (0xFFFFu << (from - lp));
        if (lp + 17 > end) pair &= end <= lp + 1 ? 0u : (0xFFFFu >> (lp + 17 - end));
        const uint32_t any = __ballot_sync(R2_FULL, pair != 0);
        if (any) {
            const uint32_t fl = (uint32_t)__ffs(any) - 1u;
            const uint32_t pr = __shfl_sync(R2_FULL, pair, (int)fl);
            return wb + 16 * fl + ((uint32_t)__ffs(pr) - 1u);
        }
        wb += 31 * 16;
    }
}

struct LeanOut { uint32_t e, cls, f, high; };
R2_DEV_NOINLINE LeanOut lean_event(R2Io io, uint32_t lane, uint32_t ps, uint32_t end) {
    uint32_t e = R2_NONE, cls = PC_NONE, f = 0, hi = 0;
    if (lane == 0) {
        R2Bytes rd{io};
        const uint32_t c0 = ps < end ? rd.at(ps) : 0u;
        if (c0 == '{') cls = PC_BRACE;
        else if (c0 == 'd' && ps + 7 <= end && rd.at(ps + 1) == 'a' && rd.at(ps + 2) == 't' && rd.at(ps + 3) == 'a' && rd.at(ps + 4) == ':' && rd.at(ps + 5) == ' ' && rd.at(ps + 6) == '{') cls = PC_DATA;
        LeanMachine lm; lm.reset(cls == PC_DATA);
        uint32_t pos = ps;
        const uint32_t body = ps + (cls == PC_DATA ? 6u : 0u);
        for (; pos < end; ++pos) {
            const uint32_t ch = rd.at(pos);
            hi |= ch;
            if (ch == '\n' && pos + 1 < end && rd.at(pos + 1) == '\n') { e = pos; break; }
            if (cls != PC_NONE && pos >= body) lm.step(ch, pos, rd);
        }
        if (e != R2_NONE && cls != PC_NONE) f = lm.finish();
    }
    LeanOut o;
    o.e = __shfl_sync(R2_FULL, e, 0); o.cls = __shfl_sync(R2_FULL, cls, 0); o.f = __shfl_sync(R2_FULL, f, 0); o.high = __shfl_sync(R2_FULL, hi, 0);
    return o;
}

R2_DEV void refresh_slots(R2Ctx& c) {
    uint32_t r = 0, f = 0, fast = 0;
    if (c.lane == 0) {
        for (uint32_t k = 0; k < R2_SLOTS; ++k) { const uint32_t st = *(volatile uint32_t*)&c.sh->slot_state[k]; if (st == 2u) r |= 1u << k; else if (st == 0u) f |= 1u << k; }
        fast = *(volatile uint32_t*)&c.sh->fast_ready;
    }
    c.ready = __shfl_sync(R2_FULL, r, 0); c.free_slots = __shfl_sync(R2_FULL, f, 0); c.fast = __shfl_sync(R2_FULL, fast, 0);
}
R2_DEV bool tpl_same(const Tpl2& x, const Tpl2& y) {
    if (x.m.len != y.m.len || x.m.cls != y.m.cls) return false;
    for (uint32_t k = 0; k < x.m.len; ++k) if (x.lit[k] != y.lit[k] || (x.lit[k] && x.text[k] != y.text[k])) return false;
    return true;
}
R2_DEV_NOINLINE void learn_template(const StepArgs* ap, R2Shared* sh, R2Io io, UsageRaw* block_raw, uint32_t lane, uint32_t ready_before, uint32_t ps, uint32_t end) {
    uint32_t got = 0;
    if (lane == 0) got = atomicCAS(&sh->learn_lock, 0u, 1u) == 0u ? 1u : 0u;
    got = __shfl_sync(R2_FULL, got, 0);
    if (!got) return;
    uint32_t ready = 0, free_slots = 0;
    if (lane == 0) for (uint32_t k = 0; k < R2_SLOTS; ++k) { const uint32_t st = *(volatile uint32_t*)&sh->slot_state[k]; if (st == 2u) ready |= 1u << k; else if (st == 0u) free_slots |= 1u << k; }
    ready = __shfl_sync(R2_FULL, ready, 0); free_slots = __shfl_sync(R2_FULL, free_slots, 0);
    uint32_t slot = R2_NONE;
    if (ready == ready_before && free_slots) {
        if (lane == 0) {
            slot = (uint32_t)__ffs(free_slots) - 1u;
            atomicExch(&sh->slot_state[slot], 1u);
            R2Bytes rd{io};
            TemplateCache2* tc = ap->s.tpl_cache2;
            UsageRaw* raw = block_raw + slot;
            if (build_template2(rd, &sh->tpl[slot], raw, ps, end)) {
                sh->slot_gidx[slot] = R2_NONE;
                if (atomicCAS(&tc->lock, 0u, 1u) == 0u) {
                    bool dup = false; uint32_t dst = R2_NONE;
                    for (uint32_t k = 0; k < R2_SLOTS; ++k) {
                        const uint32_t st = *(volatile uint32_t*)&tc->state[k];
                        if (st == 2u) { if (tpl_same(tc->tpl[k], sh->tpl[slot])) dup = true; }
                        else if (st == 0u && dst == R2_NONE) dst = k;
                    }
                    sh->slot_gidx[slot] = R2_NONE;
                    if (!dup && dst != R2_NONE) {
                        tc->tpl[dst] = sh->tpl[slot]; tc->raw[dst] = *raw; tc->hits[dst] = 0;
                        __threadfence();
                        atomicExch(&tc->state[dst], 2u);
                        sh->slot_gidx[slot] = dst;
                    }
                    __threadfence();
                    atomicExch(&tc->lock, 0u);
                }
            } else { atomicExch(&sh->slot_state[slot], 0u); slot = R2_NONE; }
        }
        slot = __shfl_sync(R2_FULL, slot, 0);
    }
    if (slot != R2_NONE) {
        uint32_t need_fast = 0;
        if (lane == 0) need_fast = (slot == sh->dflt && !*(volatile uint32_t*)&sh->fast_ready) ? 1u : 0u;
        need_fast = __shfl_sync(R2_FULL, need_fast, 0);
        if (need_fast) {
            build_fast_tables(sh, slot, lane, 32);
            __threadfence_block();
            __syncwarp();
            if (lane == 0) *(volatile uint32_t*)&sh->fast_ready = 1u;
        }
        __threadfence_block();
        if (lane == 0) atomicExch(&sh->slot_state[slot], 2u);
    }
    __syncwarp();
    if (lane == 0) { __threadfence_block(); atomicExch(&sh->learn_lock, 0u); }
    __syncwarp();
}

R2_DEV bool enter_segment(R2Ctx& c, uint32_t seg, uint32_t from, uint32_t range_hi) {
    const SegPlan* pl = c.a->s.plan + seg;
    c.seg = seg; c.ev_a = c.ev_b = c.a_usage = 0; c.high = 0; c.in_kept = 0; c.primed = 0; c.kept_tried = 0;
    const uint32_t tb = pl->relay_begin, te = pl->seg_end;
    c.tb = tb; c.te = te;
    const uint32_t kept = pl->kept_chunk != 0xFFFFFFFFu ? pl->kept_end : 0u;
    c.kept_end = kept;
    c.pos = te; c.walk_lo = te;
    c.t = 0;
    uint32_t irr = 0;
    if (c.lane == 0) irr = *(volatile const uint32_t*)&pl->irregular;
    irr = __shfl_sync(R2_FULL, irr, 0);
    if (irr || tb >= te) return false;
    if (from <= tb) {
        if (tb >= range_hi) return false;
        if (kept) c.in_kept = 1u;
        c.pos = c.s_open = c.walk_lo = tb;
        c.last_ra = R2_NONE;
        return true;
    }
    if (from >= te) return false;
    c.walk_lo = from;
    if (kept && from < kept) {
        if (kept >= range_hi || kept >= te) return false;
        c.pos = c.s_open = kept;
        c.last_ra = R2_NONE;
        return true;
    }
    const uint32_t p = find_lflf(c, from - tb >= 2u ? from - 2u : tb, te, c.high);
    if (p == R2_NONE) return false;
    const uint32_t s = p + 2u;
    if (s >= range_hi && s != te) return false;
    if ((p > tb && ring_byte(c, p - 1) == '\n') || (s < te && ring_byte(c, s) == '\n')) { mark_irregular(c); return false; }
    if (s >= te) return false;
    c.pos = c.s_open = s;
    c.last_ra = R2_NONE;
    return true;
}


R2_DEV void leave_segment(R2Ctx& c, uint32_t range_hi) {
    if (c.seg == R2_NONE) return;
    if (__any_sync(R2_FULL, (c.high & 0x80808080u) != 0)) {
        if (!chunks_utf8_ok(c.a, c.lane, c.seg, c.walk_lo, r2_min(c.te, r2_max(c.pos, range_hi)))) mark_irregular(c);
    }
    flush_counts(c);
    c.seg = R2_NONE;
}

struct SingleOut { uint32_t ok, e, high, f_start, f_len, f_esc; };
R2_DEV_NOINLINE SingleOut match_single(R2Io io, const Tpl2* tp, uint32_t lane, uint32_t ps, uint32_t ev_end) {
    const TplMeta& m = tp->m;
    SingleOut o; o.ok = 0; o.e = 0; o.high = 0; o.f_start = 0; o.f_len = 0; o.f_esc = 0;
    const uint32_t my_span = lane < 8u ? (uint32_t)m.field_span[lane] : 0xffu;
    const uint32_t n_spans = m.n_spans, len = m.len;
    uint32_t pos = ps, ta = 0, high = 0;
    for (uint32_t j = 0; j <= n_spans; ++j) {
        const uint32_t tb = j < n_spans ? (uint32_t)m.sstart[j] : len + 2u;
        bool same = true;
        for (uint32_t off = lane; off < tb - ta; off += 32) {
            const uint32_t c = pos + off < ev_end ? (uint32_t)io_byte(io, pos + off) : 0x100u;
            if (c != (uint32_t)tp->text[ta + off]) same = false;
            high |= c;
        }
        if (!__all_sync(R2_FULL, same)) return o;
        pos += tb - ta;
        if (j == n_spans) break;
        uint32_t span_len = 0, esc = 0;
        if (m.skind[j] == 1) {
            const uint32_t c = pos + lane < ev_end ? (uint32_t)io_byte(io, pos + lane) : 0u;
            const uint32_t cl = io.sh->cls[c & 0xffu];
            const uint32_t isnum = __ballot_sync(R2_FULL, cl >= C_MINUS && cl <= C_EXP);
            const uint32_t isdig = __ballot_sync(R2_FULL, cl == C_ZERO || cl == C_DIGIT);
            const uint32_t run = (uint32_t)__ffs(~isnum) - 1u;
            if (run == 0u || run >= 32u) return o;
            const uint32_t runmask = (1u << run) - 1u;
            const uint32_t first = __shfl_sync(R2_FULL, c, 0);
            if ((isdig & runmask) != runmask || (run > 1u && first == '0')) {
                uint32_t good = 0;
                if (lane == 0) {
                    uint32_t st = L_VALUE;
                    for (uint32_t k = 0; k < run && st != L_ERR; ++k) st = io.sh->trans[st * 32 + io.sh->cls[io_byte(io, pos + k)]] & 31u;
                    good = (st == L_NUM_ZERO || st == L_NUM_INT || st == L_NUM_FRAC || st == L_NUM_EXP) ? 1u : 0u;
                }
                if (!__shfl_sync(R2_FULL, good, 0)) return o;
            }
            span_len = run;
        } else {
            uint32_t q = pos;
            for (;;) {
                const uint32_t c = q + lane < ev_end ? (uint32_t)io_byte(io, q + lane) : 0u;
                high |= c;
                const uint32_t sp = __ballot_sync(R2_FULL, c < 0x20u || c == '"' || c == '\\');
                if (!sp) { q += 32; if (q - pos > R2_MAX_STR) return o; continue; }
                const uint32_t k = (uint32_t)__ffs(sp) - 1u, x = q + k;
                const uint32_t ch = __shfl_sync(R2_FULL, c, (int)k);
                if (ch == '"') { q = x; break; }
                if (ch != '\\') return o;
                const uint32_t e1 = x + 1 < ev_end ? (uint32_t)io_byte(io, x + 1) : 0u;
                uint32_t el = 0;
                if (e1 == 'u') { el = 6; for (uint32_t h4 = 2; h4 < 6; ++h4) { const uint32_t h = x + h4 < ev_end ? (uint32_t)io_byte(io, x + h4) : 0u; if (!(h - '0' < 10u || (h | 0x20u) - 'a' < 6u)) el = 0; } }
                else if (e1 == '"' || e1 == '\\' || e1 == '/' || e1 == 'b' || e1 == 'f' || e1 == 'n' || e1 == 'r' || e1 == 't') el = 2;
                if (el == 0) return o;
                esc = 1; q = x + el;
                if (q - pos > R2_MAX_STR) return o;
            }
            span_len = q - pos;
        }
        if (my_span == j) { o.f_start = pos; o.f_len = span_len; o.f_esc = esc; }
        pos += span_len; ta = m.send[j];
    }
    o.ok = 1; o.e = pos - 2u; o.high = high;
    return o;
}


struct Acct { uint32_t ok, ev_a, ev_b, a_usage, primed; };
R2_DEV Acct account(const StepArgs* ap, uint32_t lane, uint32_t seg, uint32_t in_kept, uint32_t primed, uint32_t cls, uint32_t f, uint32_t n, uint32_t ps, uint32_t e) {
    Acct r; r.ok = 1; r.ev_a = 0; r.ev_b = 0; r.a_usage = 0; r.primed = primed;
    if (cls == PC_NONE) return r;
    if (cls == PC_DATA) {
        if (in_kept) {
            if (!primed) { if (!(f & PF_VALID_A) || (f & (TK_ERROR | TK_DETAIL))) { r.ok = 0; return r; } r.primed = 1; }
        } else {
            r.ev_a = n;
            if ((f & PF_VALID_A) && !(f & TK_CODE) && (f & TK_USAGE)) r.a_usage = 1;
        }
    }
    if (f & PF_VALID_B) {
        r.ev_b = n;
        if (f & TK_ERROR) { r.ok = 0; return r; }
        if ((f & TK_USAGE) && lane == 0) {
            SegPlan* pl = ap->s.plan + seg;
            atomicAdd(&pl->n_usage_b, n);
            atomicMax(&pl->last_usage, ((unsigned long long)(ps + 1) << 32) | (e - ps));
        }
    }
    return r;
}

struct FastOut { uint32_t k, tile_lo, tile_hi; SPtr buf; uint32_t pos, t, s_open, nfast, high; };
R2_DEV_NOINLINE FastOut fast_run(const StepArgs* ap, const R2Shared* sh, SPtr ring, SPtr bars, uint32_t base, uint32_t n_tiles, uint32_t n_bytes,
                                 uint32_t k, uint32_t tile_lo, uint32_t tile_hi, SPtr buf, uint32_t pos, uint32_t t, uint32_t s_open,
                                 const uint32_t stop, const uint32_t P, const uint32_t recip, const uint32_t lane) {
    const SPtr ft = sptr(sh->fast_text), fl = sptr(sh->fast_lit);
    uint32_t nfast = 0, high = 0;
    for (;;) {
        if (pos >= tile_hi) {
            if (k + 1 >= n_tiles) break;
            const PipeState ps = pipe_advance_impl(ap, ring, bars, base, n_tiles, n_bytes, k, lane);
            k = ps.k; tile_lo = ps.tile_lo; tile_hi = ps.tile_hi; buf = ps.buf;
        }
        const uint32_t u = t + 16u * lane;
        const uint32_t tl = u - __umulhi(u, recip) * P;
        const uint32_t ad = (tl & 15u) * R2_TEXT + (tl & ~15u);
        const SPtr dp = buf + (pos + 16u * lane - tile_lo);
        if (pos + 1024u <= tile_hi && pos + 1024u <= stop) {
            const uint32_t ub = u + 512u;
            const uint32_t tlb = ub - __umulhi(ub, recip) * P;
            const uint32_t adb = (tlb & 15u) * R2_TEXT + (tlb & ~15u);
            const uint4 d = sld128(dp), e = sld128(dp + 512u);
            const uint4 tx = sld128(ft + ad), mk = sld128(fl + ad), txb = sld128(ft + adb), mkb = sld128(fl + adb);
            high |= d.x | d.y | d.z | d.w | e.x | e.y | e.z | e.w;
            const uint32_t lit = ((d.x ^ tx.x) & mk.x) | ((d.y ^ tx.y) & mk.y) | ((d.z ^ tx.z) & mk.z) | ((d.w ^ tx.w) & mk.w);
            const uint32_t litb = ((e.x ^ txb.x) & mkb.x) | ((e.y ^ txb.y) & mkb.y) | ((e.z ^ txb.z) & mkb.z) | ((e.w ^ txb.w) & mkb.w);
            const uint32_t ok = span_ok(d.x, mk.x) & span_ok(d.y, mk.y) & span_ok(d.z, mk.z) & span_ok(d.w, mk.w);
            const uint32_t okb = span_ok(e.x, mkb.x) & span_ok(e.y, mkb.y) & span_ok(e.z, mkb.z) & span_ok(e.w, mkb.w);
            if (!__ballot_sync(R2_FULL, (lit | litb | (~(ok & okb) & 0x80808080u)) != 0)) {
                const uint32_t u2 = t + 1024u;
                const uint32_t nwr = __umulhi(u2, recip);
                t = u2 - nwr * P; pos += 1024u; nfast += nwr;
                if (nwr) s_open = pos - t;
                continue;
            }
        }
        const uint32_t lim = r2_min(pos + 512u, tile_hi);
        if (lim > stop || (lim & 15u)) break;
        uint32_t bad = 0;
        if (pos + 16u * lane < lim) {
            const uint4 d = sld128(dp);
            const uint4 tx = sld128(ft + ad), mk = sld128(fl + ad);
            high |= d.x | d.y | d.z | d.w;
            const uint32_t lit = ((d.x ^ tx.x) & mk.x) | ((d.y ^ tx.y) & mk.y) | ((d.z ^ tx.z) & mk.z) | ((d.w ^ tx.w) & mk.w);
            const uint32_t ok = span_ok(d.x, mk.x) & span_ok(d.y, mk.y) & span_ok(d.z, mk.z) & span_ok(d.w, mk.w);
            bad = lit | (~ok & 0x80808080u);
        }
        if (__ballot_sync(R2_FULL, bad != 0)) break;
        const uint32_t u2 = t + (lim - pos);
        const uint32_t nwr = __umulhi(u2, recip);
        t = u2 - nwr * P; pos = lim; nfast += nwr;
        if (nwr) s_open = pos - t;
    }
    FastOut o; o.k = k; o.tile_lo = tile_lo; o.tile_hi = tile_hi; o.buf = buf; o.pos = pos; o.t = t; o.s_open = s_open; o.nfast = nfast; o.high = high;
    return o;
}

struct PassOut { uint32_t pos, t, s_open, nwr, kind, last_ra, high, reanchored; };
R2_DEV_NOINLINE PassOut pass_step(R2Io io, uint32_t lane, uint32_t slot, uint32_t fast, uint32_t pos0, uint32_t t0, uint32_t s_open0, uint32_t last_ra,
                                  uint32_t sub_end, uint32_t range_hi, uint32_t in_kept, uint32_t carry_cap) {
    const R2Shared* sh = io.sh;
    const TplMeta& m = sh->tpl[slot].m;
    const uint32_t P = m.P;
    PassOut o; o.pos = pos0; o.t = t0; o.s_open = s_open0; o.nwr = 0; o.kind = 0; o.last_ra = last_ra; o.high = 0; o.reanchored = 0;
    const uint32_t wbase = pos0 & ~15u;
    uint32_t lim = r2_min(sub_end, wbase + 512u);
    if (pos0 >= io.tile_lo && pos0 < io.tile_hi) lim = r2_min(lim, io.tile_hi);
    if (wbase + 512u > range_hi && !in_kept) {
        const uint32_t nb = pos0 + (P - t0);
        uint32_t b = nb;
        if (b < range_hi) b = nb + __umulhi(range_hi - nb + P - 1u, m.recip) * P;
        lim = r2_min(lim, b);
    }
    const uint32_t lp = wbase + 16u * lane;
    const uint32_t u = t0 + P + 16u * lane - (pos0 & 15u);
    const uint32_t tl = u - __umulhi(u, m.recip) * P;
    uint4 tx, mk;
    if (fast) {
        const uint32_t ad = (tl & 15u) * R2_TEXT + (tl & ~15u);
        tx = sld128(sptr(sh->fast_text) + ad); mk = sld128(sptr(sh->fast_lit) + ad);
    } else {
        const SPtr tp = sptr(sh->tpl[slot].text) + (tl & ~3u), lpm = sptr(sh->tpl[slot].lit) + (tl & ~3u);
        const uint32_t shf = 8 * (tl & 3u);
        const uint32_t a0 = sld32(tp), a1 = sld32(tp + 4), a2 = sld32(tp + 8), a3 = sld32(tp + 12), a4 = sld32(tp + 16);
        const uint32_t b0 = sld32(lpm), b1 = sld32(lpm + 4), b2 = sld32(lpm + 8), b3 = sld32(lpm + 12), b4 = sld32(lpm + 16);
        tx = make_uint4(__funnelshift_r(a0, a1, shf), __funnelshift_r(a1, a2, shf), __funnelshift_r(a2, a3, shf), __funnelshift_r(a3, a4, shf));
        mk = make_uint4(__funnelshift_r(b0, b1, shf), __funnelshift_r(b1, b2, shf), __funnelshift_r(b2, b3, shf), __funnelshift_r(b3, b4, shf));
    }
    const bool active = lp < lim;
    uint4 d = make_uint4(0, 0, 0, 0);
    if (active) {
        if (lp >= io.tile_lo && lp + 16 <= io.tile_hi) d = sld128(io.buf + (lp - io.tile_lo));
        else if (lp + 16 <= io.n_bytes) d = gld128(io.data + lp);
        else { uint32_t w[4] = {0, 0, 0, 0}; for (uint32_t i = 0; i < 16; ++i) w[i >> 2] |= (uint32_t)io_byte(io, lp + i) << (8 * (i & 3)); d = make_uint4(w[0], w[1], w[2], w[3]); }
    }
    o.high = d.x | d.y | d.z | d.w;
    const uint32_t r0 = (d.x ^ tx.x) & mk.x, r1 = (d.y ^ tx.y) & mk.y, r2 = (d.z ^ tx.z) & mk.z, r3 = (d.w ^ tx.w) & mk.w;
    const uint32_t s0 = ~span_ok(d.x, mk.x) & 0x80808080u, s1 = ~span_ok(d.y, mk.y) & 0x80808080u;
    const uint32_t s2 = ~span_ok(d.z, mk.z) & 0x80808080u, s3 = ~span_ok(d.w, mk.w) & 0x80808080u;
    uint32_t bm = 0xFFFFu;
    if (lp < pos0) bm &= pos0 - lp >= 16u ? 0u : (0xFFFFu << (pos0 - lp));
    if (lp + 16u > lim) bm &= lp >= lim ? 0u : (0xFFFFu >> (lp + 16u - lim));
    const uint32_t bb = (movemask4(nonzero_bytes(r0) | s0) | (movemask4(nonzero_bytes(r1) | s1) << 4) | (movemask4(nonzero_bytes(r2) | s2) << 8) | (movemask4(nonzero_bytes(r3) | s3) << 12)) & bm;
    const uint32_t any = __ballot_sync(R2_FULL, active && bb != 0);
    uint32_t mpos = lim;
    if (any) {
        const uint32_t fl = (uint32_t)__ffs(any) - 1u;
        const uint32_t b1 = __shfl_sync(R2_FULL, bb, (int)fl);
        mpos = wbase + 16u * fl + ((uint32_t)__ffs(b1) - 1u);
    }
    const uint32_t u2 = t0 + (mpos - pos0);
    const uint32_t nwr = __umulhi(u2, m.recip);
    const uint32_t t2 = u2 - nwr * P;
    o.nwr = nwr; o.pos = mpos; o.t = t2;
    if (nwr) o.s_open = mpos - t2;
    if (!any) return o;
    const uint32_t id = (t2 < m.len && mpos != last_ra) ? sh->tpl[slot].span_id[t2] : 0xffu;
    if (id != 0xffu) {
        const uint32_t sstart = m.sstart[id], send = m.send[id];
        const uint32_t ev_end = r2_min(sub_end, o.s_open + carry_cap + 2u);
        if (m.skind[id] == 0) {
            uint32_t q = mpos;
            for (;;) {
                const uint32_t c = q + lane < ev_end ? (uint32_t)io_byte(io, q + lane) : 0u;
                o.high |= c;
                const uint32_t sp = __ballot_sync(R2_FULL, c < 0x20u || c == '"' || c == '\\');
                if (!sp) { q += 32; if (q - mpos > R2_MAX_STR) break; continue; }
                const uint32_t k = (uint32_t)__ffs(sp) - 1u, x = q + k;
                const uint32_t ch = __shfl_sync(R2_FULL, c, (int)k);
                if (ch == '"') { o.pos = x; o.t = send; o.reanchored = 1; return o; }
                if (ch != '\\') break;
                const uint32_t e1 = x + 1 < ev_end ? (uint32_t)io_byte(io, x + 1) : 0u;
                uint32_t el = 0;
                if (e1 == 'u') { el = 6; for (uint32_t h4 = 2; h4 < 6; ++h4) { const uint32_t h = x + h4 < ev_end ? (uint32_t)io_byte(io, x + h4) : 0u; if (!(h - '0' < 10u || (h | 0x20u) - 'a' < 6u)) el = 0; } }
                else if (e1 == '"' || e1 == '\\' || e1 == '/' || e1 == 'b' || e1 == 'f' || e1 == 'n' || e1 == 'r' || e1 == 't') el = 2;
                if (el == 0) break;
                q = x + el;
                if (q - mpos > R2_MAX_STR) break;
            }
        } else {
            const uint32_t bs = mpos - (t2 - sstart);
            uint32_t x2 = 0, good = 0;
            if (lane == 0) {
                uint32_t st = L_VALUE, p = bs;
                for (;;) {
                    if (p >= ev_end) break;
                    const uint32_t cl = sh->cls[io_byte(io, p)];
                    if (cl < C_MINUS || cl > C_EXP) break;
                    st = sh->trans[st * 32 + cl] & 31u;
                    if (st == L_ERR) break;
                    ++p;
                }
                good = (st == L_NUM_ZERO || st == L_NUM_INT || st == L_NUM_FRAC || st == L_NUM_EXP) ? 1u : 0u;
                x2 = p;
            }
            x2 = __shfl_sync(R2_FULL, x2, 0); good = __shfl_sync(R2_FULL, good, 0);
            if (good && x2 >= mpos) { o.pos = x2; o.t = send; o.last_ra = x2; o.reanchored = 1; return o; }
        }
    }
    o.kind = 1; o.pos = o.s_open; o.t = 0; o.last_ra = R2_NONE;
    return o;
}

R2_DEV bool head_differs(const R2Io& io, const Tpl2* tp, uint32_t lane, uint32_t ps, uint32_t ev_end) {
    bool diff = false;
    if (lane < tp->m.len && tp->lit[lane]) diff = ps + lane >= ev_end || (uint32_t)io_byte(io, ps + lane) != (uint32_t)tp->text[lane];
    return __any_sync(R2_FULL, diff) != 0;
}

struct OddOut { uint32_t e, status, ev_a, ev_b, a_usage, primed, high; };
R2_DEV_NOINLINE OddOut odd_event(const StepArgs* ap, R2Shared* sh, R2Io io, uint32_t lane, uint32_t seg, uint32_t tb, uint32_t ps, uint32_t sub_end,
                                 uint32_t in_kept, uint32_t primed, uint32_t skip_slot) {
    OddOut o; o.e = R2_NONE; o.status = 0; o.ev_a = o.ev_b = o.a_usage = 0; o.primed = primed; o.high = 0;
    TemplateCache2* tc = ap->s.tpl_cache2;
    const uint32_t ev_end = r2_min(sub_end, ps + ap->t.carry_cap + 2u);
    uint32_t ready = 0, free_slots = 0;
    if (lane == 0) for (uint32_t k = 0; k < R2_SLOTS; ++k) { const uint32_t st = *(volatile uint32_t*)&sh->slot_state[k]; if (st == 2u) ready |= 1u << k; else if (st == 0u) free_slots |= 1u << k; }
    ready = __shfl_sync(R2_FULL, ready, 0); free_slots = __shfl_sync(R2_FULL, free_slots, 0);
    {
        const uint32_t want = lane < 14u ? (uint32_t)(uint8_t)"data: [DONE]\n\n"[lane] : 0u;
        const bool fits = ps + 14u <= ev_end;
        const bool same = lane >= 14u || (fits && (uint32_t)io_byte(io, ps + lane) == want);
        if (__all_sync(R2_FULL, same)) {
            const bool third_lf = ps + 14u < sub_end && io_byte(io, ps + 14u) == '\n';
            if (!third_lf) { o.e = ps + 12u; return o; }
        }
    }
    for (uint32_t slot = 0; slot < R2_SLOTS; ++slot) {
        if (!(ready & (1u << slot)) || slot == skip_slot) continue;
        if (head_differs(io, &sh->tpl[slot], lane, ps, ev_end)) continue;
        const TplMeta& m = sh->tpl[slot].m;
        const SingleOut so = match_single(io, &sh->tpl[slot], lane, ps, ev_end);
        if (!so.ok) continue;
        o.high |= so.high;
        if (lane == 0 && sh->slot_gidx[slot] != R2_NONE) atomicAdd(&tc->hits[sh->slot_gidx[slot]], 1u);
        const Acct ac = account(ap, lane, seg, in_kept, primed, m.cls, m.flags, 1, ps, so.e);
        if (!ac.ok) { o.status = 1; return o; }
        if ((m.flags & TK_USAGE) && (m.flags & PF_VALID_B) && m.usage_ok && so.e - ps <= LGW_PENDING_CAP && sh->slot_gidx[slot] != R2_NONE) {
            uint2* uf = ap->s.usage_fields + (size_t)seg * 9u;
            if (lane < 8u) uf[lane] = m.field_span[lane] != 0xffu ? make_uint2(so.f_start, so.f_len | (so.f_esc << 31)) : make_uint2(0u, 0xFFFFFFFFu);
            if (lane == 0) { uf[8] = make_uint2(sh->slot_gidx[slot], m.full_flags); ap->s.plan[seg].cand_ps = ps + 1u; }
        }
        o.e = so.e; o.ev_a = ac.ev_a; o.ev_b = ac.ev_b; o.a_usage = ac.a_usage; o.primed = ac.primed;
        return o;
    }
    if (ps > tb && io_byte(io, ps) == '\n') { o.status = 1; return o; }
    const LeanOut lo = lean_event(io, lane, ps, ev_end);
    o.high |= lo.high;
    if (lo.e == R2_NONE) { if (ev_end < sub_end) o.status = 1; return o; }
    if (lo.e + 2 < sub_end && io_byte(io, lo.e + 2) == '\n') { o.status = 1; return o; }
    if (lo.cls != PC_NONE && lane == 0) atomicAdd(&tc->general, 1u);
    const Acct ac = account(ap, lane, seg, in_kept, primed, lo.cls, lo.f, 1, ps, lo.e);
    if (!ac.ok) { o.status = 1; return o; }
    if (lo.cls != PC_NONE && (lo.f & PF_VALID_A) && !(lo.f & (TK_ERROR | TK_DETAIL | TK_CODE)) && lo.e - ps >= R2_TPL_MIN && lo.e - ps <= R2_TPL_MAX && free_slots)
        learn_template(ap, sh, io, sh->raw_tpl, lane, ready, ps, sub_end);
    o.e = lo.e; o.ev_a = ac.ev_a; o.ev_b = ac.ev_b; o.a_usage = ac.a_usage; o.primed = ac.primed;
    return o;
}

R2_DEV bool walk_segment(R2Ctx& c, const uint32_t range_hi) {
    R2Shared* sh = c.sh;
    const uint32_t lane = c.lane;
    for (;;) {
        if (c.in_kept == 2u && c.s_open >= c.kept_end) {
            const TplMeta& dm = sh->tpl[c.dflt].m;
            c.ev_a -= __umulhi(c.kept_end - c.tb, dm.recip);
            if (lane == 0) c.a->s.plan[c.seg].prime_ok = 1;
            c.in_kept = 0;
        }
        const uint32_t sub_end = c.in_kept == 1u ? c.kept_end : c.te;
        if (c.pos >= sub_end) {
            if (c.in_kept == 2u) { c.in_kept = 1u; c.pos = c.s_open = c.tb; c.t = 0; c.ev_a = c.ev_b = c.a_usage = 0; c.primed = 0; c.last_ra = R2_NONE; continue; }
            if (c.in_kept) {
                if (c.s_open != c.kept_end || !c.primed) { mark_irregular(c); return false; }
                if (lane == 0) c.a->s.plan[c.seg].prime_ok = 1;
                c.in_kept = 0;
                continue;
            }
            if (lane == 0) c.a->s.plan[c.seg].tail_start = c.s_open;
            return false;
        }
        if (c.s_open >= range_hi && c.pos == c.s_open && !c.in_kept) return true;
        while (c.pos >= c.tile_hi && c.k + 1 < c.n_tiles) pipe_advance(c);

        const bool have_dflt = (c.ready & (1u << c.dflt)) != 0u && !(sh->tpl[c.dflt].m.flags & TK_USAGE);
        if (c.in_kept == 1u && c.pos == c.tb && have_dflt && c.kept_end > c.tb && c.kept_end < c.te) {
            const TplMeta& dm = sh->tpl[c.dflt].m;
            const uint32_t n = c.kept_end - c.tb, q = __umulhi(n, dm.recip);
            if (dm.cls == PC_DATA && q * dm.P == n && !c.kept_tried) { c.in_kept = 2u; c.kept_tried = 1u; }
        }
        if (have_dflt && c.fast && c.in_kept != 1u && (c.pos & 15u) == 0u && c.pos >= c.tile_lo && c.pos < c.tile_hi) {
            const TplMeta& dm = sh->tpl[c.dflt].m;
            const FastOut fo = fast_run(c.a, sh, c.ring, c.bars, c.base, c.n_tiles, c.n_bytes, c.k, c.tile_lo, c.tile_hi, c.buf,
                                        c.pos, c.t, c.s_open, r2_min(sub_end, range_hi), dm.P, dm.recip, lane);
            c.k = fo.k; c.tile_lo = fo.tile_lo; c.tile_hi = fo.tile_hi; c.buf = fo.buf;
            c.high |= fo.high;
            if (fo.nfast) {
                c.single = 0u;
                c.hits_d += fo.nfast; c.s_open = fo.s_open;
                if (dm.cls == PC_DATA) c.ev_a += fo.nfast;
                if (dm.flags & PF_VALID_B) c.ev_b += fo.nfast;
            }
            if (fo.pos != c.pos) { c.pos = fo.pos; c.t = fo.t; continue; }
        }
        bool try_pass = have_dflt;
        if (have_dflt && c.single && c.t == 0u && c.pos == c.s_open && c.in_kept != 2u) {
            const SingleOut so = match_single(io_of(c), &sh->tpl[c.dflt], lane, c.pos, r2_min(sub_end, c.pos + c.a->t.carry_cap + 2u));
            if (so.ok) {
                const TplMeta& dm = sh->tpl[c.dflt].m;
                c.high |= so.high; ++c.hits_d;
                if (dm.cls == PC_DATA) { if (c.in_kept == 1u) c.primed = 1; else ++c.ev_a; }
                if (dm.flags & PF_VALID_B) ++c.ev_b;
                c.pos = c.s_open = so.e + 2u; c.last_ra = R2_NONE;
                continue;
            }
            try_pass = false;
        }
        if (try_pass && c.t == 0u && c.pos == c.s_open && head_differs(io_of(c), &sh->tpl[c.dflt], lane, c.pos, sub_end)) try_pass = false;
        if (try_pass) {
            const PassOut po = pass_step(io_of(c), lane, c.dflt, c.fast, c.pos, c.t, c.s_open, c.last_ra, sub_end, range_hi, c.in_kept == 1u ? 1u : 0u, c.a->t.carry_cap);
            c.high |= po.high;
            if (po.nwr) {
                const TplMeta& dm = sh->tpl[c.dflt].m;
                c.hits_d += po.nwr;
                if (dm.cls == PC_DATA) { if (c.in_kept == 1u) c.primed = 1; else c.ev_a += po.nwr; }
                if (dm.flags & PF_VALID_B) c.ev_b += po.nwr;
            }
            c.pos = po.pos; c.t = po.t; c.s_open = po.s_open; c.last_ra = po.last_ra;
            if (po.reanchored) c.single = 1u;
            if (c.in_kept == 2u && (po.kind || po.reanchored) && c.s_open < c.kept_end) {
                c.in_kept = 1u; c.pos = c.s_open = c.tb; c.t = 0; c.ev_a = c.ev_b = c.a_usage = 0; c.primed = 0; c.last_ra = R2_NONE;
                continue;
            }
            if (po.kind == 0 && po.reanchored && po.nwr && c.in_kept != 2u) { c.pos = c.s_open; c.t = 0u; c.last_ra = R2_NONE; continue; }
            if (po.kind == 0) continue;
        } else if (c.in_kept == 2u && c.s_open < c.kept_end) {
            c.in_kept = 1u; c.pos = c.s_open = c.tb; c.t = 0; c.ev_a = c.ev_b = c.a_usage = 0; c.primed = 0; c.last_ra = R2_NONE;
            continue;
        }
        {
            const OddOut oo = odd_event(c.a, sh, io_of(c), lane, c.seg, c.tb, c.s_open, sub_end, c.in_kept == 1u ? 1u : 0u, c.primed, have_dflt ? c.dflt : R2_NONE);
            c.high |= oo.high;
            if (oo.status) { mark_irregular(c); return false; }
            refresh_slots(c);
            if (oo.e == R2_NONE) { c.pos = sub_end; continue; }
            c.ev_a += oo.ev_a; c.ev_b += oo.ev_b; c.a_usage |= oo.a_usage; c.primed = oo.primed;
            c.pos = c.s_open = oo.e + 2u; c.t = 0; c.last_ra = R2_NONE;
        }
    }
}

R2_GLOBAL void
#if !R2_HOST_EMU
#ifdef R2_MAXREG
__maxnreg__(R2_MAXREG)
#else
__launch_bounds__(R2_THREADS, 1)
#endif
#endif
k_relay2(StepArgs a, uint32_t n_tiles_total, uint32_t tiles_per_warp, uint32_t base0) {
    uint8_t* smem = smem_base();
    R2Shared* sh = reinterpret_cast<R2Shared*>(smem + R2_RING_BYTES);
    const uint32_t tid = R2_TID, warp = tid >> 5, lane = tid & 31u;
    TemplateCache2* tc = a.s.tpl_cache2;
    UsageRaw* block_raw = sh->raw_tpl;

    griddep_launch();
    for (uint32_t k = tid; k < 64 + LGW_LEAN_ROWS * 8; k += R2_THREADS) {
        if (k < 64) reinterpret_cast<uint32_t*>(sh->cls)[k] = reinterpret_cast<const uint32_t*>(lean_tables().cls)[k];
        else reinterpret_cast<uint32_t*>(sh->trans)[k - 64] = reinterpret_cast<const uint32_t*>(lean_tables().trans)[k - 64];
    }
    if (tid == 0) { sh->fast_ready = 0; sh->learn_lock = 0; sh->args = a; }
    if (lane == 0) for (uint32_t b = 0; b < R2_NBUF; ++b) mbar_init(sptr(&sh->mbar[warp * R2_NBUF + b]), 1);
    mbar_fence_init();
    __syncthreads();
    const uint32_t gw = R2_BID * R2_WARPS + warp;
    const uint32_t t_first = gw * tiles_per_warp;
    R2Ctx c;
    c.a = &sh->args; c.sh = sh; c.lane = lane;
    c.ring = sptr(smem) + warp * R2_NBUF * R2_TILE; c.bars = sptr(&sh->mbar[warp * R2_NBUF]);
    c.n_bytes = a.n_bytes;
    c.base = base0 + t_first * R2_TILE;
    c.n_tiles = t_first >= n_tiles_total ? 0u : r2_min(tiles_per_warp, n_tiles_total - t_first);
    pipe_start(c);
    griddep_wait();
    if (tid < R2_SLOTS) { sh->slot_state[tid] = (*(volatile uint32_t*)&tc->state[tid] == 2u) ? 2u : 0u; sh->slot_gidx[tid] = tid; }
    __syncthreads();
    for (uint32_t s = 0; s < R2_SLOTS; ++s) {
        if (sh->slot_state[s] != 2u) continue;
        const uint32_t* src = reinterpret_cast<const uint32_t*>(&tc->tpl[s]);
        uint32_t* dst = reinterpret_cast<uint32_t*>(&sh->tpl[s]);
        for (uint32_t k = tid; k < sizeof(Tpl2) / 4; k += R2_THREADS) dst[k] = src[k];
        const uint32_t* rs = reinterpret_cast<const uint32_t*>(&tc->raw[s]);
        uint32_t* rd = reinterpret_cast<uint32_t*>(&block_raw[s]);
        for (uint32_t k = tid; k < sizeof(UsageRaw) / 4; k += R2_THREADS) rd[k] = rs[k];
    }
    if (tid == 0) {
        uint32_t d = 0, best = 0; bool have = false;
        for (uint32_t s = 0; s < R2_SLOTS; ++s) if (sh->slot_state[s] == 2u) { const uint32_t h = tc->hits[s]; if (!have || h > best) { d = s; best = h; have = true; } }
        sh->dflt = d;
    }
    __syncthreads();
    if (sh->slot_state[sh->dflt] == 2u) {
        build_fast_tables(sh, sh->dflt, tid, R2_THREADS);
        __syncthreads();
        if (tid == 0) sh->fast_ready = 1;
    }
    __syncthreads();

    c.dflt = sh->dflt; c.last_ra = R2_NONE; c.hits_d = 0; c.single = 0;
    refresh_slots(c);
    c.seg = R2_NONE; c.ev_a = c.ev_b = c.a_usage = 0; c.high = 0;
    c.t = 0; c.pos = c.s_open = 0;
    c.in_kept = c.primed = c.kept_tried = 0; c.tb = c.te = c.kept_end = 0; c.walk_lo = 0;
    if (c.n_tiles == 0) return;
    const uint32_t range_lo = r2_max(c.base, a.tile_base);
    const uint32_t range_hi = r2_min(c.base + c.n_tiles * R2_TILE, a.n_bytes);
    pipe_advance(c);

    for (uint32_t seg = a.s.tile_seg[t_first]; seg < a.n_segs; ++seg) {
        const uint32_t seg_first = seg ? a.s.plan[seg - 1].seg_end : a.tile_base;
        if (seg_first >= range_hi) break;
        const bool done = enter_segment(c, seg, r2_max(range_lo, seg_first), range_hi) && walk_segment(c, range_hi);
        leave_segment(c, range_hi);
        if (done) break;
    }
    while (c.k + 1 < c.n_tiles) pipe_advance(c);
    __syncwarp();
    if (lane == 0) {
        tma_wait_all();
        if (c.hits_d && sh->slot_gidx[c.dflt] != R2_NONE) atomicAdd(&tc->hits[sh->slot_gidx[c.dflt]], c.hits_d);
    }
}

R2_GLOBAL void k_prime2(StepArgs a) {
    griddep_launch();
    const uint32_t i = R2_BID * R2_NTHR + R2_TID;
    if (i == 0) {
        TemplateCache2* tc = a.s.tpl_cache2;
        uint32_t total = 0, full = 1, lo = 0;
        for (uint32_t s = 0; s < R2_SLOTS; ++s) { total += tc->hits[s]; if (tc->state[s] != 2u) full = 0; if (tc->hits[s] < tc->hits[lo]) lo = s; }
        if (full && tc->general && (tc->hits[lo] == 0 || (tc->general > 64u && tc->general > total / 2u))) { tc->state[lo] = 0; tc->hits[lo] = 0; }
        for (uint32_t s = 0; s < R2_SLOTS; ++s) tc->hits[s] >>= 1;
        tc->general >>= 1;
    }
    if (i >= a.n_segs) return;
    const uint32_t seg = i, c0 = a.seg_chunk[seg], c1 = a.seg_chunk[seg + 1];
    const uint32_t slot = a.seg_slot[seg];
    const StreamHdr st = a.t.state[slot].h;
    SegPlan p;
    p.seg_end = a.chunk_off[c1]; p.relay_begin = p.seg_end; p.irregular = 0; p.last_usage = 0; p.a_usage = 0;
    p.n_events_a = p.n_events_b = p.n_usage_b = 0; p.tail_start = 0xFFFFFFFFu; p.cand_ps = 0;
    p.kept_chunk = 0xFFFFFFFFu; p.kept_end = 0; p.prime_ok = 0;
    p.resume_chunk = c0; p.emit_chunk_begin = (st.phase == PH_COMMITTED) ? c0 : c1;
    if (st.phase == PH_COMMITTED && c0 < c1) {
        if ((st.flags & SF_SYNCED) && st.carry_a_len == 0) p.relay_begin = a.chunk_off[c0];
        else p.irregular = 1;
    } else if (st.phase == PH_PRIMING && c0 < c1) {
        uint32_t c = c0;
        while (c < c1 && a.chunk_off[c + 1] == a.chunk_off[c]) ++c;
        if (c < c1 && st.carry_a_len == 0) {
            p.kept_chunk = c; p.kept_end = a.chunk_off[c + 1]; p.relay_begin = a.chunk_off[c]; p.emit_chunk_begin = c;
        } else if (c < c1) p.irregular = 1;
    }
    a.s.plan[seg] = p;
    const uint32_t base0 = a.tile_base & ~15u;
    const uint32_t b0 = a.chunk_off[c0], b1 = p.seg_end;
    if (b1 > b0) {
        uint32_t t_lo = seg == 0 ? 0u : (b0 - base0 + R2_TILE - 1) / R2_TILE;
        const uint32_t t_hi = (b1 - 1 - base0) / R2_TILE;
        for (uint32_t t = t_lo; t <= t_hi; ++t) a.s.tile_seg[t] = seg;
    }
}

#define R2_CWARPS 8u
#ifndef R2_CBLOCKS
#define R2_CBLOCKS 6
#endif
R2_DEV_NOINLINE uint32_t commit_sequential(StepIO io, const uint8_t* data, const uint32_t* chunk_off, uint32_t c_from, uint32_t c_to, uint32_t emit_begin) {
    run_chunks(io, data, chunk_off, c_from, c_to, emit_begin, false);
    return emit_begin;
}
R2_DEV_NOINLINE void commit_usage_event(StepIO io, const uint8_t* text, uint32_t n) {
    StreamHdr& st = *io.st;
    Rope r{nullptr, 0, text, n};
    const uint8_t cls = classify_part(r, 0, n);
    UsageRaw raw;
    const uint32_t f = parse_part<true>(r, 0, n, cls, &raw);
    if (f & PF_EXOTIC) { ++st.n_exotic; st.flags |= SF_EXOTIC_SEEN; return; }
    if ((f & TK_CHOICES) && (f & PF_TYPE_ERROR)) return;
    normalise_usage(raw, f, *io.rec);
    st.flags |= SF_REC_VALID; ++st.n_usage_b;
    if (io.rec->exotic) { ++st.n_exotic; st.flags |= SF_EXOTIC_SEEN; }
}
struct TextReader {
    const uint8_t* text; uint32_t base, n;
    R2_MEM uint32_t at(uint32_t p) const { return p - base < n ? (uint32_t)text[p - base] : 0u; }
};
R2_DEV_NOINLINE void commit_usage_fields(const uint8_t* text, uint32_t ups, uint32_t ulen, uint32_t full_flags, const UsageRaw* tpl_raw, UsageRaw* raw, UsageRec* cand, uint32_t lane,
                                         uint32_t f_start, uint32_t f_word) {
    TextReader rd{text, ups, ulen};
    const bool has_span = lane < 8u && f_word != 0xFFFFFFFFu;
    const uint32_t f_len = f_word & 0x7FFFFFFFu, f_esc = has_span ? f_word >> 31 : 0u;
    const uint32_t span_mask = __ballot_sync(R2_FULL, has_span);
    Val v; v.kind = KD_ABSENT; v.bits = 0;
    for (uint32_t k = lane; k < sizeof(UsageRaw) / 4; k += 32) reinterpret_cast<uint32_t*>(raw)[k] = reinterpret_cast<const uint32_t*>(tpl_raw)[k];
    __syncwarp();
    const uint32_t slow_str = __ballot_sync(R2_FULL, has_span && lane >= UF_MODEL && f_esc != 0u);
    if (has_span) {
        if (lane < UF_MODEL) v = parse_number_span(rd, f_start, f_len);
        else if (f_esc) {
            if (lane == UF_MODEL) decode_string_span(rd, f_start, f_len, raw->model, raw->model_len, raw->model_flags);
            else decode_string_span(rd, f_start, f_len, raw->provider, raw->provider_len, raw->provider_flags);
        } else if (lane == UF_MODEL) { raw->model_len = 0; raw->model_flags = 0; }
        else { raw->provider_len = 0; raw->provider_flags = 0; }
    }
    __syncwarp();
    for (uint32_t fi = 0; fi < UF_MODEL; ++fi) {
        const unsigned long long vb = __shfl_sync(R2_FULL, (unsigned long long)v.bits, (int)fi);
        const uint32_t vk = __shfl_sync(R2_FULL, (uint32_t)v.kind, (int)fi);
        if (lane == 0 && (span_mask & (1u << fi))) {
            Val x; x.bits = (int64_t)vb; x.kind = (uint8_t)vk;
            if (fi == UF_PROMPT) raw->prompt = x; else if (fi == UF_COMPLETION) raw->completion = x; else if (fi == UF_TOTAL) raw->total = x;
            else if (fi == UF_COST) raw->cost = x; else if (fi == UF_REASONING) raw->reasoning = x; else raw->cached = x;
        }
    }
    uint32_t has = 0;
    if (lane == 0) {
        normalise_usage(*raw, full_flags, *cand);
        has = (cand->model_val.kind == KD_STR ? 1u : 0u) | (cand->provider_val.kind == KD_STR ? 2u : 0u);
    }
    has = __shfl_sync(R2_FULL, has, 0);
    for (uint32_t which = 0; which < 2; ++which) {
        const uint32_t fl = UF_MODEL + which;
        const uint32_t st = __shfl_sync(R2_FULL, f_start, (int)fl), ln = __shfl_sync(R2_FULL, f_len, (int)fl);
        if (!(span_mask & (1u << fl)) || (slow_str & (1u << fl)) || !(has & (1u << which))) continue;
        const uint32_t n = ln < LGW_STR_CAP ? ln : (uint32_t)LGW_STR_CAP;
        char* dst = which == 0 ? cand->model : cand->provider;
        for (uint32_t k = lane; k < n; k += 32) dst[k] = (char)rd.at(st + k);
        if (lane == 0) {
            if (which == 0) cand->model_len = (uint8_t)n; else cand->provider_len = (uint8_t)n;
            if (ln > LGW_STR_CAP) { cand->str_flags |= which == 0 ? 1u : 4u; cand->exotic = 1; }
        }
    }
    __syncwarp();
}

R2_DEV_NOINLINE void commit_settle_pending(StepIO io) { resolve_pending(io); }
#if !R2_HOST_EMU
R2_DEV uint4 commit_ld16(const uint8_t* p) { return __ldg(reinterpret_cast<const uint4*>(p)); }
#else
R2_DEV uint4 commit_ld16(const uint8_t* p) { uint4 v; memcpy(&v, p, 16); return v; }
#endif

R2_GLOBAL void
#if !R2_HOST_EMU
__launch_bounds__(R2_CWARPS * 32, R2_CBLOCKS)
#endif
k_commit2(StepArgs a) {
#if !R2_HOST_EMU
    __shared__ __align__(16) uint8_t stage[R2_CWARPS][LGW_PENDING_STRIDE];
    __shared__ __align__(16) UsageRaw stage_raw[R2_CWARPS];
#else
    alignas(16) static uint8_t stage[R2_CWARPS][LGW_PENDING_STRIDE];
    static UsageRaw stage_raw[R2_CWARPS];
#endif
    const uint32_t seg = (R2_BID * R2_NTHR + R2_TID) >> 5, lane = R2_TID & 31u, warp = (R2_TID >> 5) % R2_CWARPS;
    if (seg >= a.n_segs) return;
    const uint32_t c0 = __ldg(a.seg_chunk + seg), c1 = __ldg(a.seg_chunk + seg + 1);
    const uint32_t slot = __ldg(a.seg_slot + seg);
    StreamHdr st = a.t.state[slot].h;
    bool empty = false;
    if ((st.phase == PH_COMMITTED || st.phase == PH_PRIMING) && c0 < c1) {
        for (uint32_t c = c0 + lane; c < c1; c += 32 * 8) {
            uint32_t lo[8], hi[8];
#pragma unroll
            for (uint32_t j = 0; j < 8; ++j) { const uint32_t cc = c + 32 * j; lo[j] = cc < c1 ? __ldg(a.chunk_off + cc) : 0u; hi[j] = cc < c1 ? __ldg(a.chunk_off + cc + 1) : 1u; }
#pragma unroll
            for (uint32_t j = 0; j < 8; ++j) if (lo[j] == hi[j]) empty = true;
        }
    }
    const bool any_empty = __any_sync(R2_FULL, empty);
    griddep_wait();
    const SegPlan p = a.s.plan[seg];
    const StepIO io = make_io(a, slot, &st);
    uint32_t emit_begin = p.emit_chunk_begin;
    const bool speculated = p.kept_chunk != 0xFFFFFFFFu;
    if ((st.phase == PH_COMMITTED || st.phase == PH_PRIMING) && p.resume_chunk < c1) {
        const uint8_t* __restrict__ d = a.data;
        const uint32_t ups = (uint32_t)(p.last_usage >> 32) - 1u, ulen = (uint32_t)p.last_usage;
        const bool staged = p.last_usage && ulen <= LGW_PENDING_CAP && (uint64_t)ups + ulen <= a.n_bytes;
        const bool has_cand = staged && p.cand_ps == ups + 1u;
        uint2 fld = make_uint2(0u, 0xFFFFFFFFu), gf = make_uint2(0u, 0u);
        if (has_cand) { const uint2* uf = a.s.usage_fields + (size_t)seg * 9u; if (lane < 8u) fld = uf[lane]; gf = uf[8]; }
        const uint32_t ab = ups & ~15u, skew = ups - ab;
        const bool d_aligned = (reinterpret_cast<uintptr_t>(d) & 15u) == 0u;
        const uint8_t* const utext = stage[warp] + skew;
        if (staged) {
            const uint32_t nvec = (skew + ulen + 15u) >> 4;
            for (uint32_t k = lane; k < nvec; k += 32) {
                const uint32_t o = ab + (k << 4);
                if (o + 16u <= a.n_bytes && d_aligned) *reinterpret_cast<uint4*>(stage[warp] + (k << 4)) = commit_ld16(d + o);
                else for (uint32_t j = 0; j < 16u && o + j < a.n_bytes; ++j) stage[warp][(k << 4) + j] = __ldg(d + o + j);
            }
        }
        bool sequential = p.irregular || p.n_usage_b > 1 || any_empty;
        if (st.phase == PH_PRIMING && !(speculated && p.prime_ok)) sequential = true;
        if (!sequential && p.last_usage && !staged) sequential = true;
        if (!sequential && p.tail_start == 0xFFFFFFFFu) sequential = true;
        if (lane == 0) atomicAdd(a.s.counters + (sequential ? 0 : 1), 1u);
        if (sequential) {
            if (lane == 0) emit_begin = commit_sequential(io, a.data, a.chunk_off, p.resume_chunk, c1, (st.phase == PH_COMMITTED) ? p.resume_chunk : c1);
        } else {
            uint32_t first = p.resume_chunk;
            if (speculated) {
                st.phase = PH_COMMITTED; st.verdict = VD_OK;
                st.flags |= SF_EMITTED_ANY | SF_SYNCED;
                st.carry_a_len = st.carry_b_len = 0;
                ++st.n_events_a;
                first = p.kept_chunk;
            }
            const uint32_t nch = c1 - first, nby = p.seg_end - p.relay_begin;
            st.n_chunks_in += nch; st.n_chunks_emitted += nch; st.bytes_in += nby; st.bytes_emitted += nby;
            st.n_events_a += p.n_events_a; st.n_events_b += p.n_events_b;
            if (p.a_usage) st.flags |= SF_A_USAGE_BOUND;
            if (p.last_usage) {
                if (lane == 0 && (st.flags & SF_PENDING)) commit_settle_pending(io);
                __syncwarp();
                if (has_cand) {
                    commit_usage_fields(utext, ups, ulen, gf.y, &a.s.tpl_cache2->raw[gf.x], &stage_raw[warp], io.rec, lane, fld.x, fld.y);
                    __syncwarp();
                    st.flags |= SF_REC_VALID; ++st.n_usage_b;
                    if (io.rec->exotic) { ++st.n_exotic; st.flags |= SF_EXOTIC_SEEN; }
                    if (lane == 0) atomicAdd(a.s.counters + 2, 1u);
                } else {
                    if (lane == 0) { commit_usage_event(io, utext, ulen); atomicAdd(a.s.counters + 3, 1u); }
                }
            }
            const uint32_t tail = p.tail_start, n = p.seg_end - tail;
            if (n > a.t.carry_cap) { st.carry_a_len = 0; st.flags |= SF_CARRY_OVERFLOW; }
            else { for (uint32_t k = lane; k < n; k += 32) io.carry_a[k] = d[tail + k]; st.carry_a_len = n; }
        }
        __syncwarp();
        if (lane == 0) a.t.state[slot].h = st;
    }
    if (lane == 0) {
        SegResult res;
        fill_seg_result(st, emit_begin, c1, res);
        a.seg_out[seg] = res;
    }
}

#if !R2_HOST_EMU
static inline cudaError_t launch_step_fast(const StepArgs& a, int sm_count, cudaStream_t stream, cudaEvent_t* ev, int* launched, bool per_kernel) {
    cudaError_t r;
    const uint32_t base0 = a.tile_base & ~15u;
    const uint32_t n_tiles = a.n_bytes > base0 ? (a.n_bytes - base0 + R2_TILE - 1) / R2_TILE : 0u;
    cudaLaunchAttribute attr[1];
    attr[0].id = cudaLaunchAttributeProgrammaticStreamSerialization;
    attr[0].val.programmaticStreamSerializationAllowed = 1;
    if (a.n_segs) { k_prime2<<<(a.n_segs + 127) / 128, 128, 0, stream>>>(a); ++*launched; }
    if (per_kernel && (r = cudaEventRecord(ev[1], stream)) != cudaSuccess) return r;
    if (n_tiles) {
        const uint32_t max_warps = (uint32_t)sm_count * R2_WARPS;
        const uint32_t tpw = (n_tiles + max_warps - 1) / max_warps;
        const uint32_t warps = (n_tiles + tpw - 1) / tpw;
        const uint32_t blocks = (warps + R2_WARPS - 1) / R2_WARPS;
        cudaLaunchConfig_t cfg = {};
        cfg.gridDim = dim3(blocks); cfg.blockDim = dim3(R2_THREADS); cfg.dynamicSmemBytes = R2_SMEM_BYTES; cfg.stream = stream;
        cfg.attrs = attr; cfg.numAttrs = per_kernel ? 0 : 1;
        if ((r = cudaLaunchKernelEx(&cfg, k_relay2, a, n_tiles, tpw, base0)) != cudaSuccess) return r;
        ++*launched;
    }
    if (per_kernel && (r = cudaEventRecord(ev[2], stream)) != cudaSuccess) return r;
    if (a.n_segs) {
        cudaLaunchConfig_t cfg = {};
        cfg.gridDim = dim3((a.n_segs + R2_CWARPS - 1) / R2_CWARPS); cfg.blockDim = dim3(R2_CWARPS * 32); cfg.dynamicSmemBytes = 0; cfg.stream = stream;
        cfg.attrs = attr; cfg.numAttrs = per_kernel ? 0 : 1;
        if ((r = cudaLaunchKernelEx(&cfg, k_commit2, a)) != cudaSuccess) return r;
        ++*launched;
    }
    if (per_kernel && (r = cudaEventRecord(ev[3], stream)) != cudaSuccess) return r;
    if ((r = cudaEventRecord(ev[4], stream)) != cudaSuccess) return r;
    return cudaGetLastError();
}
#endif
```

### llmapigateway_b200/csrc/sse_kernels.cuh

```cuda
#pragma once
#include <cuda_runtime.h>
#include "stream_machine.cuh"
#include "lean_json.cuh"
#include "step_types.cuh"

namespace lgw {

__global__ void k_streams_open(DeviceTables t, const uint32_t* slots, const int32_t* status, uint32_t n) {
    const uint32_t i = blockIdx.x * blockDim.x + threadIdx.x;
    if (i >= n) return;
    init_stream(t.state[slots[i]], status[i]);
}

__global__ void k_streams_gather(DeviceTables t, const uint32_t* slots, uint32_t n, StreamState* out, int free_after) {
    const uint32_t i = blockIdx.x * blockDim.x + threadIdx.x;
    if (i >= n) return;
    const uint32_t slot = slots[i];
    StreamState* s = t.state + slot;
    if (s->h.flags & SF_PENDING) {
        StreamHdr st = s->h;
        StepIO io;
        io.st = &st; io.rec = &s->rec; io.pending = t.pending + (size_t)slot * LGW_PENDING_STRIDE;
        io.carry_a = io.carry_b = io.detail = nullptr; io.carry_cap = io.detail_cap = 0;
        io.rowq = nullptr; io.rowq_count = nullptr; io.rowq_cap = 0; io.slot = slot;
        resolve_pending(io);
        s->h = st;
    }
    out[i] = *s;
    if (free_after) s->h.phase = PH_FREE;
}

__global__ void __launch_bounds__(64) k_general(StepArgs a) {
    const uint32_t seg = blockIdx.x * blockDim.x + threadIdx.x;
    if (seg >= a.n_segs) return;
    const uint32_t slot = a.seg_slot[seg];
    StreamHdr st = a.t.state[slot].h;
    const StepIO io = make_io(a, slot, &st);
    SegResult res;
    run_segment(io, a.data, a.chunk_off, a.seg_chunk[seg], a.seg_chunk[seg + 1], res);
    a.t.state[slot].h = st;
    a.seg_out[seg] = res;
}

__global__ void __launch_bounds__(256) k_copy(const uint8_t* __restrict__ in, uint8_t* __restrict__ out, uint32_t n) {
    const uint32_t nvec = n >> 4;
    const uint4* __restrict__ vi = reinterpret_cast<const uint4*>(in);
    uint4* __restrict__ vo = reinterpret_cast<uint4*>(out);
    for (uint32_t i = blockIdx.x * blockDim.x + threadIdx.x; i < nvec; i += gridDim.x * blockDim.x) vo[i] = __ldg(vi + i);
    const uint32_t tail = nvec << 4;
    if (blockIdx.x == 0 && threadIdx.x < (n - tail)) out[tail + threadIdx.x] = in[tail + threadIdx.x];
}

#include "relay2.cuh"

static inline cudaError_t scratch_alloc(StepScratch& s, size_t max_streams, size_t max_bytes, int sm_count) {
    cudaError_t r;
    if ((r = cudaMalloc((void**)&s.plan, max_streams * sizeof(SegPlan))) != cudaSuccess) return r;
    if ((r = cudaMalloc((void**)&s.tpl_cache2, sizeof(TemplateCache2))) != cudaSuccess) return r;
    if ((r = cudaMemset(s.tpl_cache2, 0, sizeof(TemplateCache2))) != cudaSuccess) return r;
    (void)sm_count;
    if ((r = cudaMalloc((void**)&s.usage_fields, max_streams * 9 * sizeof(uint2))) != cudaSuccess) return r;
    if ((r = cudaMalloc((void**)&s.tile_seg, (max_bytes / R2_TILE + 4) * 4)) != cudaSuccess) return r;
    if ((r = cudaMemset(s.tile_seg, 0, (max_bytes / R2_TILE + 4) * 4)) != cudaSuccess) return r;
    if ((r = cudaMalloc((void**)&s.counters, 64)) != cudaSuccess) return r;
    if ((r = cudaMemset(s.counters, 0, 64)) != cudaSuccess) return r;
    if ((r = cudaFuncSetAttribute(k_relay2, cudaFuncAttributeMaxDynamicSharedMemorySize, (int)R2_SMEM_BYTES)) != cudaSuccess) return r;
    return cudaSuccess;
}
static inline void scratch_free(StepScratch& s) {
    cudaFree(s.plan); cudaFree(s.tpl_cache2); cudaFree(s.usage_fields); cudaFree(s.counters); s.counters = nullptr; cudaFree(s.tile_seg); s.tile_seg = nullptr;
    s.plan = nullptr; s.tpl_cache2 = nullptr; s.usage_fields = nullptr;
}

static inline cudaError_t launch_step(const StepArgs& a, int mode, int sm_count, cudaStream_t stream, cudaEvent_t* ev, int* launched, bool per_kernel) {
    *launched = 0;
    cudaError_t r;
    if ((r = cudaEventRecord(ev[0], stream)) != cudaSuccess) return r;
    if (mode == 1) {
        if ((r = cudaEventRecord(ev[1], stream)) != cudaSuccess) return r;
        if (a.n_bytes) { k_copy<<<sm_count * 8, 256, 0, stream>>>(a.data, a.out, a.n_bytes); ++*launched; }
        if ((r = cudaEventRecord(ev[2], stream)) != cudaSuccess) return r;
        if (a.n_segs) { k_general<<<(a.n_segs + 63) / 64, 64, 0, stream>>>(a); ++*launched; }
        if ((r = cudaEventRecord(ev[3], stream)) != cudaSuccess) return r;
        if ((r = cudaEventRecord(ev[4], stream)) != cudaSuccess) return r;
        return cudaGetLastError();
    }
    return launch_step_fast(a, sm_count, stream, ev, launched, per_kernel);
}

}
```

### llmapigateway_b200/csrc/step_types.cuh

```cuda
#pragma once
#include "stream_machine.cuh"
#include "lean_json.cuh"

namespace lgw {

struct DeviceTables {
    StreamState* state;
    uint8_t* carry_a; uint8_t* carry_b; uint8_t* detail; uint8_t* pending;
    uint32_t carry_cap, detail_cap, max_streams;
};

struct SegPlan {
    uint32_t resume_chunk;
    uint32_t relay_begin;
    uint32_t seg_end;
    uint32_t emit_chunk_begin;
    uint32_t irregular;
    uint32_t a_usage;
    unsigned long long last_usage;
    uint32_t n_events_a, n_events_b, n_usage_b;
    uint32_t kept_chunk;
    uint32_t kept_end;
    uint32_t prime_ok;
    uint32_t tail_start;
    uint32_t cand_ps;
};
static_assert(sizeof(SegPlan) == 64, "SegPlan");

struct TemplateCache2;

struct StepScratch {
    SegPlan* plan;
    TemplateCache2* tpl_cache2;
    uint2* usage_fields;
    uint32_t* tile_seg;
    uint32_t* counters;
};

struct StepArgs {
    DeviceTables t;
    const uint8_t* data; uint32_t n_bytes;
    const uint32_t* chunk_off; uint32_t n_chunks;
    uint32_t tile_base;
    uint32_t chunk_lo, chunk_hi;
    const uint32_t* seg_chunk; const uint32_t* seg_slot; uint32_t n_segs;
    uint8_t* out; SegResult* seg_out;
    RowEvent* rowq; uint32_t* rowq_count; uint32_t rowq_cap;
    StepScratch s;
};

LGW_HD StepIO make_io(const StepArgs& a, uint32_t slot, StreamHdr* local_hdr) {
    StepIO io;
    io.st = local_hdr;
    io.rec = &a.t.state[slot].rec;
    io.pending = a.t.pending + (size_t)slot * LGW_PENDING_STRIDE;
    io.carry_a = a.t.carry_a + (size_t)slot * a.t.carry_cap;
    io.carry_b = a.t.carry_b + (size_t)slot * a.t.carry_cap;
    io.detail = a.t.detail + (size_t)slot * a.t.detail_cap;
    io.carry_cap = a.t.carry_cap; io.detail_cap = a.t.detail_cap;
    io.rowq = a.rowq; io.rowq_count = a.rowq_count; io.rowq_cap = a.rowq_cap; io.slot = slot;
    return io;
}

}
```

### llmapigateway_b200/engine.py

```python
from __future__ import annotations

import ctypes as C
from dataclasses import dataclass

import numpy as np

from . import _abi, _native

SEG_DTYPE = np.dtype([("emit_chunk_begin", "<u4"), ("phase", "u1"), ("verdict", "u1"), ("flags", "<u2"), ("detail_len", "<u4")])
assert SEG_DTYPE.itemsize == C.sizeof(_abi.SegResult)


class EngineError(RuntimeError):
    pass


@dataclass
class StepResult:
    out: np.ndarray
    segs: np.ndarray
    rows: list

    def keep_mask(self, seg_chunk: np.ndarray, n_chunks: int) -> np.ndarray:
        keep = np.zeros(n_chunks, dtype=bool)
        for s in range(len(self.segs)):
            keep[int(self.segs["emit_chunk_begin"][s]):int(seg_chunk[s + 1])] = True
        return keep


@dataclass
class StepText:
    text: np.ndarray
    seg_off: np.ndarray
    flags: np.ndarray
    marks: list

    def segment(self, s: int) -> bytes:
        return self.text[int(self.seg_off[s]):int(self.seg_off[s + 1])].tobytes()


def _ptr(a: np.ndarray):
    return a.ctypes.data_as(C.c_void_p)


class Engine:
    def __init__(self, device: int = 0, max_streams: int = 8192, carry_cap: int = 65536, detail_cap: int = 4096,
                 rowq_cap: int = 4096, max_step_chunks: int = 1 << 22, max_step_bytes: int = 1 << 28):
        self._lib = _native.load()
        self.limits = _abi.Limits(max_streams, carry_cap, detail_cap, rowq_cap, max_step_chunks, max_step_bytes)
        h = C.c_void_p()
        rc = self._lib.lgw_engine_create(device, C.byref(self.limits), C.byref(h))
        if rc != 0:
            raise EngineError(f"lgw_engine_create failed ({rc}): {self._lib.lgw_last_error(None).decode()}")
        self._h = h
        self.device = device

    def _ck(self, rc: int, what: str):
        if rc != 0:
            raise EngineError(f"{what} failed ({rc}): {self._lib.lgw_last_error(self._h).decode()}")

    def close_engine(self):
        if getattr(self, "_h", None):
            self._lib.lgw_engine_destroy(self._h)
            self._h = None

    def __del__(self):
        try:
            self.close_engine()
        except Exception:
            pass

    def alloc_pinned(self, nbytes: int) -> np.ndarray:
        p = C.c_void_p()
        self._ck(self._lib.lgw_alloc_pinned(self._h, nbytes, C.byref(p)), "alloc_pinned")
        return np.ctypeslib.as_array((C.c_uint8 * nbytes).from_address(p.value))

    def set_stream(self, cuda_stream_ptr: int | None):
        self._ck(self._lib.lgw_engine_set_stream(self._h, C.c_void_p(cuda_stream_ptr or 0)), "set_stream")

    def set_mode(self, mode: int):
        self._ck(self._lib.lgw_engine_set_mode(self._h, mode), "set_mode")

    def open(self, slots, http_status=None):
        slots = np.ascontiguousarray(slots, dtype=np.uint32)
        st = np.full(len(slots), 200, dtype=np.int32) if http_status is None else np.ascontiguousarray(http_status, dtype=np.int32)
        self._ck(self._lib.lgw_streams_open(self._h, _ptr(slots), _ptr(st), len(slots)), "streams_open")

    def _states(self, fn, slots):
        slots = np.ascontiguousarray(slots, dtype=np.uint32)
        if len(slots) == 0:
            return []
        out = (_abi.StreamState * len(slots))()
        self._ck(fn(self._h, _ptr(slots), len(slots), out), "streams_state")
        return out

    def state(self, slots):
        return self._states(self._lib.lgw_streams_state, slots)

    def close(self, slots):
        return self._states(self._lib.lgw_streams_close, slots)

    def detail(self, slot: int) -> bytes:
        buf = C.create_string_buffer(self.limits.detail_cap)
        n = C.c_uint32(0)
        self._ck(self._lib.lgw_stream_detail(self._h, slot, buf, self.limits.detail_cap, C.byref(n)), "stream_detail")
        return buf.raw[:n.value]

    def details(self, slots, stride: int | None = None) -> list:
        slots = np.ascontiguousarray(slots, dtype=np.uint32)
        n = len(slots)
        if n == 0:
            return []
        stride = stride or min(self.limits.detail_cap, 1024)
        buf = np.empty(n * stride, dtype=np.uint8)
        lens = np.zeros(n, dtype=np.uint32)
        self._ck(self._lib.lgw_streams_details(self._h, _ptr(slots), n, _ptr(buf), stride, _ptr(lens)), "streams_details")
        if int(lens.max()) >= stride and stride < self.limits.detail_cap:
            return self.details(slots, self.limits.detail_cap)
        raw = buf.tobytes()
        return [raw[i * stride:i * stride + int(lens[i])] for i in range(n)]

    def step(self, data: np.ndarray, chunk_off: np.ndarray, seg_chunk: np.ndarray, seg_slot: np.ndarray,
             out: np.ndarray | None = None, relay_from_host: bool = False) -> StepResult:
        data = np.ascontiguousarray(data, dtype=np.uint8)
        chunk_off = np.ascontiguousarray(chunk_off, dtype=np.uint32)
        seg_chunk = np.ascontiguousarray(seg_chunk, dtype=np.uint32)
        seg_slot = np.ascontiguousarray(seg_slot, dtype=np.uint32)
        n_bytes, n_chunks, n_segs = data.size, chunk_off.size - 1, seg_slot.size
        if relay_from_host:
            out = None
        elif out is None:
            out = np.empty(max(n_bytes, 1), dtype=np.uint8)
        segs = np.zeros(max(n_segs, 1), dtype=SEG_DTYPE)
        cap = self.limits.rowq_cap
        rows = getattr(self, "_rows_buf", None)
        if rows is None:
            rows = self._rows_buf = (_abi.RowEvent * max(cap, 1))()
        n_rows = C.c_uint32(0)
        self._last_n_segs = n_segs
        self._ck(self._lib.lgw_sse_step(self._h, _ptr(data), n_bytes, _ptr(chunk_off), n_chunks, _ptr(seg_chunk), _ptr(seg_slot),
                                        n_segs, _ptr(out) if out is not None else None, _ptr(segs), rows, cap, C.byref(n_rows)), "sse_step")
        return StepResult((out if out is not None else data)[:n_bytes], segs[:n_segs], [_abi.RowEvent.from_buffer_copy(rows[i]) for i in range(n_rows.value)])

    def step_device(self, d_data: int, n_bytes: int, d_chunk_off: int, n_chunks: int, d_seg_chunk: int, d_seg_slot: int,
                    n_segs: int, d_out: int, d_segs: int):
        self._last_n_segs = n_segs
        self._ck(self._lib.lgw_sse_step_device(self._h, d_data, n_bytes, d_chunk_off, n_chunks, d_seg_chunk, d_seg_slot,
                                               n_segs, d_out, d_segs), "sse_step_device")

    def fetch_rows(self):
        cap = self.limits.rowq_cap
        rows = (_abi.RowEvent * max(cap, 1))()
        n_rows = C.c_uint32(0)
        self._ck(self._lib.lgw_fetch_rows(self._h, rows, cap, C.byref(n_rows)), "fetch_rows")
        return [rows[i] for i in range(n_rows.value)]

    def enable_transcripts(self):
        self._ck(self._lib.lgw_transcripts_enable(self._h), "transcripts_enable")
        self._text_on = True

    def step_transcript(self) -> StepText:
        total, n_marks = C.c_uint64(0), C.c_uint32(0)
        self._ck(self._lib.lgw_step_transcript_run(self._h, C.byref(total), C.byref(n_marks)), "step_transcript_run")
        n_segs = self._last_n_segs
        text = np.empty(max(total.value, 1), dtype=np.uint8)
        seg_off = np.zeros(n_segs + 1, dtype=np.uint64)
        flags = np.zeros(max(n_segs, 1), dtype=np.uint32)
        marks = (_abi.TextMark * max(n_marks.value, 1))()
        self._ck(self._lib.lgw_step_transcript_fetch(self._h, _ptr(text), _ptr(seg_off), _ptr(flags), marks), "step_transcript_fetch")
        return StepText(text[:total.value], seg_off, flags[:n_segs], [(marks[i].slot, marks[i].seq, marks[i].text_pos) for i in range(n_marks.value)])

    def transcript_last_ms(self) -> float:
        ms = C.c_float(0)
        self._ck(self._lib.lgw_transcript_last_ms(self._h, C.byref(ms)), "transcript_last_ms")
        return ms.value

    def last_step_direct(self) -> bool:
        return bool(self._lib.lgw_last_step_direct(self._h))

    def sync(self):
        self._ck(self._lib.lgw_sync(self._h), "sync")

    def last_step_ms(self):
        ms, k = (C.c_float * 4)(), (C.c_float * 4)()
        self._ck(self._lib.lgw_last_step_ms(self._h, C.byref(ms)), "last_step_ms")
        self._ck(self._lib.lgw_last_step_kernel_ms(self._h, C.byref(k)), "last_step_kernel_ms")
        return dict(prime=k[0], relay=k[1], commit=k[2], host_step=ms[3])

    def set_kernel_timing(self, on: bool):
        self._ck(self._lib.lgw_engine_set_kernel_timing(self._h, 1 if on else 0), "set_kernel_timing")

    def debug_counters(self):
        out = (C.c_uint32 * 4)()
        self._ck(self._lib.lgw_debug_counters(self._h, out), "debug_counters")
        return dict(sequential=out[0], bulk=out[1], from_template=out[2], stashed=out[3])

    def launch_count(self) -> int:
        n = C.c_uint64(0)
        self._ck(self._lib.lgw_launch_count(self._h, C.byref(n)), "launch_count")
        return n.value

    def load_rules(self, plans) -> None:
        from . import rewrite as rw
        p, o, blob = plans.packed()
        assert p.dtype == rw.PLAN_DTYPE and o.dtype == rw.OP_DTYPE
        self._ck(self._lib.lgw_rules_load(self._h, _ptr(p) if len(p) else None, len(p), _ptr(o) if len(o) else None, len(o),
                                          _ptr(blob), len(blob)), "rules_load")
        self._plan_growth = plans.max_growth()

    def scan_packed(self, buf: np.ndarray, off: np.ndarray, model_cap: int = 256):
        from . import rewrite as rw
        n = len(off) - 1
        scans = np.zeros(max(n, 1), dtype=rw.SCAN_DTYPE)
        models = np.zeros((max(n, 1), model_cap), dtype=np.uint8)
        self._ck(self._lib.lgw_bodies_scan(self._h, _ptr(buf), _ptr(off), n, model_cap, _ptr(scans), _ptr(models)), "bodies_scan")
        return scans[:n], models[:n]

    def scan_bodies(self, bodies, model_cap: int = 256):
        from . import rewrite as rw
        buf, off = rw.pack_bodies(bodies)
        scans, models = self.scan_packed(buf, off, model_cap)
        lens = np.minimum(scans["model_len"], model_cap)
        return scans, [bytes(models[i, :int(lens[i])]) for i in range(len(bodies))]

    def rewrite_packed(self, buf: np.ndarray, off: np.ndarray, plan_idx: np.ndarray, slot_cap: int, out: np.ndarray | None = None):
        from . import rewrite as rw
        n = len(off) - 1
        plan_idx = np.ascontiguousarray(plan_idx, dtype=np.uint32)
        assert len(plan_idx) == n and off.dtype == np.uint64 and buf.dtype == np.uint8
        if out is None:
            growth = getattr(self, "_plan_growth", 0) + 64
            out = np.empty(min(n * slot_cap, 6 * int(off[n]) + n * growth) + 64, dtype=np.uint8)
        out_off = np.zeros(n + 1, dtype=np.uint64)
        res = np.zeros(max(n, 1), dtype=rw.RESULT_DTYPE)
        self._ck(self._lib.lgw_bodies_rewrite(self._h, _ptr(buf), _ptr(off), n, _ptr(plan_idx), slot_cap,
                                              _ptr(out), out.nbytes, _ptr(out_off), _ptr(res)), "bodies_rewrite")
        return out, out_off, res[:n]

    def rewrite_bodies(self, bodies, plan_idx, slot_cap: int | None = None, with_matched: bool = False):
        from . import rewrite as rw
        buf, off = rw.pack_bodies(bodies)
        if slot_cap is None:
            longest = max((len(b) for b in bodies), default=0)
            slot_cap = 6 * longest + getattr(self, "_plan_growth", 0) + 64
            slot_cap = (slot_cap + 15) & ~15
        out, out_off, res = self.rewrite_packed(buf, off, np.asarray(plan_idx, dtype=np.uint32), slot_cap)
        rows = [(int(res["status"][i]), bytes(out[int(out_off[i]):int(out_off[i + 1])]) if res["status"][i] == rw.BODY_OK else b"")
                for i in range(len(bodies))]
        if with_matched:
            return [(st, b, int(res["matched"][i]), int(res["root_kind"][i])) for i, (st, b) in enumerate(rows)]
        return rows

    def documents_usage(self, docs):
        from . import rewrite as rw
        buf, off = rw.pack_bodies(docs)
        n = len(docs)
        out = (_abi.DocUsage * max(n, 1))()
        self._ck(self._lib.lgw_documents_usage(self._h, _ptr(buf), _ptr(off), n, out), "documents_usage")
        res = []
        for i in range(n):
            row = _abi.usage_rec_to_dict(out[i].rec)
            res.append(([dict(row), row] if out[i].error_row else [row], bool(out[i].exotic)))
        return res

    def documents_error_detail(self, docs, text_stride: int = 4096):
        from . import rewrite as rw
        buf, off = rw.pack_bodies(docs)
        n = len(docs)
        out = (_abi.DocError * max(n, 1))()
        text = np.zeros(max(n, 1) * text_stride, dtype=np.uint8)
        self._ck(self._lib.lgw_documents_error_detail(self._h, _ptr(buf), _ptr(off), n, out, _ptr(text), text_stride), "documents_error_detail")
        return [(out[i], bytes(text[i * text_stride:i * text_stride + out[i].text_len])) for i in range(n)]

    def bodies_last_ms(self):
        ms = (C.c_float * 3)()
        self._ck(self._lib.lgw_bodies_last_ms(self._h, C.byref(ms)), "bodies_last_ms")
        return dict(rewrite=ms[0], offsets=ms[1], pack=ms[2])
```

Baseline: 15.76 billion.

## Defer tail events from relay to commit kernel via per-segment tail list

Tail SSE events that match a cached template head are no longer fully classified in the relay kernel. The relay kernel now only locates each event's terminator and records up to four (start, end) pairs per segment. The commit kernel then stages each recorded event's text, judges it against the template cache and does the event and usage accounting there, replacing the earlier candidate usage-field handoff. The intent is to move per-event template matching off the relay critical path, at the cost of extra staging and judging work in commit and a sequential fallback when more than four tails occur.

```diff
diff --git a/llmapigateway_b200/csrc/lgw_engine.cu b/llmapigateway_b200/csrc/lgw_engine.cu
--- a/llmapigateway_b200/csrc/lgw_engine.cu
+++ b/llmapigateway_b200/csrc/lgw_engine.cu
@@ -854,11 +854,11 @@
     return LGW_OK;
 }
 
-extern "C" int lgw_debug_counters(lgw_engine* e, uint32_t out[4]) {
+extern "C" int lgw_debug_counters(lgw_engine* e, uint32_t out[5]) {
     if (!e || !out) return LGW_ERR_ARG;
     CK(e, cudaSetDevice(e->device));
     CK(e, cudaStreamSynchronize(e->stream));
-    CK(e, cudaMemcpy(out, e->scratch.counters, 16, cudaMemcpyDeviceToHost));
+    CK(e, cudaMemcpy(out, e->scratch.counters, 20, cudaMemcpyDeviceToHost));
     return LGW_OK;
 }
 
diff --git a/llmapigateway_b200/csrc/relay2.cuh b/llmapigateway_b200/csrc/relay2.cuh
--- a/llmapigateway_b200/csrc/relay2.cuh
+++ b/llmapigateway_b200/csrc/relay2.cuh
@@ -33,6 +33,7 @@
 #define R2_NBUF 2u
 #endif
 #define R2_SLOTS 4u
+#define R2_TAILS 4u
 #define R2_TPL_MAX 504u
 #define R2_TPL_MIN 16u
 #define R2_TEXT 544u
@@ -194,12 +195,12 @@
     const uint8_t* data; uint32_t n_bytes;
     R2_MEM uint32_t at(uint32_t p) const { return p < n_bytes ? (uint32_t)__ldg(data + p) : 0u; }
 };
-R2_DEV uint4 ld16(const R2Ctx& c, uint32_t p) {
-    if (p >= c.tile_lo && p + 16 <= c.tile_hi) return sld128(c.buf + (p - c.tile_lo));
-    if (p + 16 <= c.n_bytes) return gld128(c.a->data + p);
+R2_DEV uint4 ld16(const R2Io& io, uint32_t p) {
+    if (p >= io.tile_lo && p + 16 <= io.tile_hi) return sld128(io.buf + (p - io.tile_lo));
+    if (p + 16 <= io.n_bytes) return gld128(io.data + p);
     uint32_t w0 = 0, w1 = 0, w2 = 0, w3 = 0;
-    for (uint32_t i = 0; i < 16 && p + i < c.n_bytes; ++i) {
-        const uint32_t v = (uint32_t)ring_byte(c, p + i) << (8 * (i & 3));
+    for (uint32_t i = 0; i < 16 && p + i < io.n_bytes; ++i) {
+        const uint32_t v = (uint32_t)io_byte(io, p + i) << (8 * (i & 3));
         if (i < 4) w0 |= v; else if (i < 8) w1 |= v; else if (i < 12) w2 |= v; else w3 |= v;
     }
     return make_uint4(w0, w1, w2, w3);
@@ -419,16 +420,16 @@
     return __all_sync(R2_FULL, ok);
 }
 
-R2_DEV uint32_t find_lflf(R2Ctx& c, uint32_t from, uint32_t end, uint32_t& high) {
+R2_DEV uint32_t find_lflf(const R2Io& io, uint32_t lane, uint32_t from, uint32_t end, uint32_t& high) {
     uint32_t wb = from & ~15u;
     for (;;) {
         if (wb >= end) return R2_NONE;
-        const uint32_t lp = wb + 16 * c.lane;
-        const uint4 d = lp < end ? ld16(c, lp) : make_uint4(0, 0, 0, 0);
+        const uint32_t lp = wb + 16 * lane;
+        const uint4 d = lp < end ? ld16(io, lp) : make_uint4(0, 0, 0, 0);
         high |= d.x | d.y | d.z | d.w;
         const uint32_t lf = lf_mask16(d);
         const uint32_t nxt = __shfl_down_sync(R2_FULL, lf, 1);
-        uint32_t pair = lf & ((lf >> 1) | ((c.lane < 31 ? nxt & 1u : 0u) << 15));
+        uint32_t pair = lf & ((lf >> 1) | ((lane < 31 ? nxt & 1u : 0u) << 15));
         if (lp < from) pair &= from - lp >= 16 ? 0u : (0xFFFFu << (from - lp));
         if (lp + 17 > end) pair &= end <= lp + 1 ? 0u : (0xFFFFu >> (lp + 17 - end));
         const uint32_t any = __ballot_sync(R2_FULL, pair != 0);
@@ -563,7 +564,7 @@
         c.last_ra = R2_NONE;
         return true;
     }
-    const uint32_t p = find_lflf(c, from - tb >= 2u ? from - 2u : tb, te, c.high);
+    const uint32_t p = find_lflf(io_of(c), c.lane, from - tb >= 2u ? from - 2u : tb, te, c.high);
     if (p == R2_NONE) return false;
     const uint32_t s = p + 2u;
     if (s >= range_hi && s != te) return false;
@@ -585,7 +586,8 @@
 }
 
 struct SingleOut { uint32_t ok, e, high, f_start, f_len, f_esc; };
-R2_DEV_NOINLINE SingleOut match_single(R2Io io, const Tpl2* tp, uint32_t lane, uint32_t ps, uint32_t ev_end) {
+template <class RD>
+R2_DEV_NOINLINE SingleOut match_single(const RD rd, const Tpl2* tp, uint32_t lane, uint32_t ps, uint32_t ev_end) {
     const TplMeta& m = tp->m;
     SingleOut o; o.ok = 0; o.e = 0; o.high = 0; o.f_start = 0; o.f_len = 0; o.f_esc = 0;
     const uint32_t my_span = lane < 8u ? (uint32_t)m.field_span[lane] : 0xffu;
@@ -595,7 +597,7 @@
         const uint32_t tb = j < n_spans ? (uint32_t)m.sstart[j] : len + 2u;
         bool same = true;
         for (uint32_t off = lane; off < tb - ta; off += 32) {
-            const uint32_t c = pos + off < ev_end ? (uint32_t)io_byte(io, pos + off) : 0x100u;
+            const uint32_t c = pos + off < ev_end ? (uint32_t)rd.at(pos + off) : 0x100u;
             if (c != (uint32_t)tp->text[ta + off]) same = false;
             high |= c;
         }
@@ -604,8 +606,8 @@
         if (j == n_spans) break;
         uint32_t span_len = 0, esc = 0;
         if (m.skind[j] == 1) {
-            const uint32_t c = pos + lane < ev_end ? (uint32_t)io_byte(io, pos + lane) : 0u;
-            const uint32_t cl = io.sh->cls[c & 0xffu];
+            const uint32_t c = pos + lane < ev_end ? (uint32_t)rd.at(pos + lane) : 0u;
+            const uint32_t cl = rd.cls(c & 0xffu);
             const uint32_t isnum = __ballot_sync(R2_FULL, cl >= C_MINUS && cl <= C_EXP);
             const uint32_t isdig = __ballot_sync(R2_FULL, cl == C_ZERO || cl == C_DIGIT);
             const uint32_t run = (uint32_t)__ffs(~isnum) - 1u;
@@ -616,7 +618,7 @@
                 uint32_t good = 0;
                 if (lane == 0) {
                     uint32_t st = L_VALUE;
-                    for (uint32_t k = 0; k < run && st != L_ERR; ++k) st = io.sh->trans[st * 32 + io.sh->cls[io_byte(io, pos + k)]] & 31u;
+                    for (uint32_t k = 0; k < run && st != L_ERR; ++k) st = rd.trans(st * 32 + rd.cls(rd.at(pos + k))) & 31u;
                     good = (st == L_NUM_ZERO || st == L_NUM_INT || st == L_NUM_FRAC || st == L_NUM_EXP) ? 1u : 0u;
                 }
                 if (!__shfl_sync(R2_FULL, good, 0)) return o;
@@ -625,7 +627,7 @@
         } else {
             uint32_t q = pos;
             for (;;) {
-                const uint32_t c = q + lane < ev_end ? (uint32_t)io_byte(io, q + lane) : 0u;
+                const uint32_t c = q + lane < ev_end ? (uint32_t)rd.at(q + lane) : 0u;
                 high |= c;
                 const uint32_t sp = __ballot_sync(R2_FULL, c < 0x20u || c == '"' || c == '\\');
                 if (!sp) { q += 32; if (q - pos > R2_MAX_STR) return o; continue; }
@@ -633,9 +635,9 @@
                 const uint32_t ch = __shfl_sync(R2_FULL, c, (int)k);
                 if (ch == '"') { q = x; break; }
                 if (ch != '\\') return o;
-                const uint32_t e1 = x + 1 < ev_end ? (uint32_t)io_byte(io, x + 1) : 0u;
+                const uint32_t e1 = x + 1 < ev_end ? (uint32_t)rd.at(x + 1) : 0u;
                 uint32_t el = 0;
-                if (e1 == 'u') { el = 6; for (uint32_t h4 = 2; h4 < 6; ++h4) { const uint32_t h = x + h4 < ev_end ? (uint32_t)io_byte(io, x + h4) : 0u; if (!(h - '0' < 10u || (h | 0x20u) - 'a' < 6u)) el = 0; } }
+                if (e1 == 'u') { el = 6; for (uint32_t h4 = 2; h4 < 6; ++h4) { const uint32_t h = x + h4 < ev_end ? (uint32_t)rd.at(x + h4) : 0u; if (!(h - '0' < 10u || (h | 0x20u) - 'a' < 6u)) el = 0; } }
                 else if (e1 == '"' || e1 == '\\' || e1 == '/' || e1 == 'b' || e1 == 'f' || e1 == 'n' || e1 == 'r' || e1 == 't') el = 2;
                 if (el == 0) return o;
                 esc = 1; q = x + el;
@@ -837,9 +839,10 @@
     return o;
 }
 
-R2_DEV bool head_differs(const R2Io& io, const Tpl2* tp, uint32_t lane, uint32_t ps, uint32_t ev_end) {
+template <class RD>
+R2_DEV bool head_differs(const RD& rd, const Tpl2* tp, uint32_t lane, uint32_t ps, uint32_t ev_end) {
     bool diff = false;
-    if (lane < tp->m.len && tp->lit[lane]) diff = ps + lane >= ev_end || (uint32_t)io_byte(io, ps + lane) != (uint32_t)tp->text[lane];
+    if (lane < tp->m.len && tp->lit[lane]) diff = ps + lane >= ev_end || rd.at(ps + lane) != (uint32_t)tp->text[lane];
     return __any_sync(R2_FULL, diff) != 0;
 }
 
@@ -852,30 +855,16 @@
     uint32_t ready = 0, free_slots = 0;
     if (lane == 0) for (uint32_t k = 0; k < R2_SLOTS; ++k) { const uint32_t st = *(volatile uint32_t*)&sh->slot_state[k]; if (st == 2u) ready |= 1u << k; else if (st == 0u) free_slots |= 1u << k; }
     ready = __shfl_sync(R2_FULL, ready, 0); free_slots = __shfl_sync(R2_FULL, free_slots, 0);
-    {
-        const uint32_t want = lane < 14u ? (uint32_t)(uint8_t)"data: [DONE]\n\n"[lane] : 0u;
-        const bool fits = ps + 14u <= ev_end;
-        const bool same = lane >= 14u || (fits && (uint32_t)io_byte(io, ps + lane) == want);
-        if (__all_sync(R2_FULL, same)) {
-            const bool third_lf = ps + 14u < sub_end && io_byte(io, ps + 14u) == '\n';
-            if (!third_lf) { o.e = ps + 12u; return o; }
-        }
-    }
     for (uint32_t slot = 0; slot < R2_SLOTS; ++slot) {
         if (!(ready & (1u << slot)) || slot == skip_slot) continue;
-        if (head_differs(io, &sh->tpl[slot], lane, ps, ev_end)) continue;
+        if (head_differs(R2Bytes{io}, &sh->tpl[slot], lane, ps, ev_end)) continue;
         const TplMeta& m = sh->tpl[slot].m;
-        const SingleOut so = match_single(io, &sh->tpl[slot], lane, ps, ev_end);
+        const SingleOut so = match_single(R2Bytes{io}, &sh->tpl[slot], lane, ps, ev_end);
         if (!so.ok) continue;
         o.high |= so.high;
         if (lane == 0 && sh->slot_gidx[slot] != R2_NONE) atomicAdd(&tc->hits[sh->slot_gidx[slot]], 1u);
         const Acct ac = account(ap, lane, seg, in_kept, primed, m.cls, m.flags, 1, ps, so.e);
         if (!ac.ok) { o.status = 1; return o; }
-        if ((m.flags & TK_USAGE) && (m.flags & PF_VALID_B) && m.usage_ok && so.e - ps <= LGW_PENDING_CAP && sh->slot_gidx[slot] != R2_NONE) {
-            uint2* uf = ap->s.usage_fields + (size_t)seg * 9u;
-            if (lane < 8u) uf[lane] = m.field_span[lane] != 0xffu ? make_uint2(so.f_start, so.f_len | (so.f_esc << 31)) : make_uint2(0u, 0xFFFFFFFFu);
-            if (lane == 0) { uf[8] = make_uint2(sh->slot_gidx[slot], m.full_flags); ap->s.plan[seg].cand_ps = ps + 1u; }
-        }
         o.e = so.e; o.ev_a = ac.ev_a; o.ev_b = ac.ev_b; o.a_usage = ac.a_usage; o.primed = ac.primed;
         return o;
     }
@@ -890,6 +879,37 @@
     if (lo.cls != PC_NONE && (lo.f & PF_VALID_A) && !(lo.f & (TK_ERROR | TK_DETAIL | TK_CODE)) && lo.e - ps >= R2_TPL_MIN && lo.e - ps <= R2_TPL_MAX && free_slots)
         learn_template(ap, sh, io, sh->raw_tpl, lane, ready, ps, sub_end);
     o.e = lo.e; o.ev_a = ac.ev_a; o.ev_b = ac.ev_b; o.a_usage = ac.a_usage; o.primed = ac.primed;
+    return o;
+}
+
+R2_DEV bool done_event(const R2Io& io, uint32_t lane, uint32_t ps, uint32_t sub_end, uint32_t carry_cap) {
+    const uint32_t want = lane < 14u ? (uint32_t)(uint8_t)"data: [DONE]\n\n"[lane] : 0u;
+    const bool fits = ps + 14u <= r2_min(sub_end, ps + carry_cap + 2u);
+    const bool same = lane >= 14u || (fits && (uint32_t)io_byte(io, ps + lane) == want);
+    if (!__all_sync(R2_FULL, same)) return false;
+    return !(ps + 14u < sub_end && io_byte(io, ps + 14u) == '\n');
+}
+
+struct TailOut { uint32_t kind, e, high; };
+R2_DEV_NOINLINE TailOut tail_event(const StepArgs* ap, const R2Shared* sh, R2Io io, uint32_t lane, uint32_t seg, uint32_t ready, uint32_t skip_slot,
+                                   uint32_t ps, uint32_t sub_end) {
+    TailOut o; o.kind = 0; o.e = R2_NONE; o.high = 0;
+    if (done_event(io, lane, ps, sub_end, ap->t.carry_cap)) { o.kind = 1; o.e = ps + 12u; return o; }
+    const uint32_t ev_end = r2_min(sub_end, ps + ap->t.carry_cap + 2u);
+    bool head = false;
+    for (uint32_t slot = 0; slot < R2_SLOTS && !head; ++slot)
+        if ((ready & (1u << slot)) && slot != skip_slot && !head_differs(R2Bytes{io}, &sh->tpl[slot], lane, ps, ev_end)) head = true;
+    if (!head) return o;
+    const uint32_t e = find_lflf(io, lane, ps, ev_end, o.high);
+    if (e == R2_NONE) { o.kind = ev_end < sub_end ? 2u : 3u; return o; }
+    if (e + 2u < sub_end && io_byte(io, e + 2u) == '\n') { o.kind = 2; return o; }
+    uint32_t idx = 0;
+    if (lane == 0) {
+        idx = atomicAdd(&ap->s.plan[seg].n_tails, 1u);
+        if (idx < R2_TAILS) ap->s.tails[(size_t)seg * R2_TAILS + idx] = make_uint2(ps, e);
+    }
+    if (__shfl_sync(R2_FULL, idx, 0) >= R2_TAILS) return o;
+    o.kind = 1; o.e = e;
     return o;
 }
 
@@ -940,7 +960,7 @@
         }
         bool try_pass = have_dflt;
         if (have_dflt && c.single && c.t == 0u && c.pos == c.s_open && c.in_kept != 2u) {
-            const SingleOut so = match_single(io_of(c), &sh->tpl[c.dflt], lane, c.pos, r2_min(sub_end, c.pos + c.a->t.carry_cap + 2u));
+            const SingleOut so = match_single(R2Bytes{io_of(c)}, &sh->tpl[c.dflt], lane, c.pos, r2_min(sub_end, c.pos + c.a->t.carry_cap + 2u));
             if (so.ok) {
                 const TplMeta& dm = sh->tpl[c.dflt].m;
                 c.high |= so.high; ++c.hits_d;
@@ -951,7 +971,7 @@
             }
             try_pass = false;
         }
-        if (try_pass && c.t == 0u && c.pos == c.s_open && head_differs(io_of(c), &sh->tpl[c.dflt], lane, c.pos, sub_end)) try_pass = false;
+        if (try_pass && c.t == 0u && c.pos == c.s_open && head_differs(R2Bytes{io_of(c)}, &sh->tpl[c.dflt], lane, c.pos, sub_end)) try_pass = false;
         if (try_pass) {
             const PassOut po = pass_step(io_of(c), lane, c.dflt, c.fast, c.pos, c.t, c.s_open, c.last_ra, sub_end, range_hi, c.in_kept == 1u ? 1u : 0u, c.a->t.carry_cap);
             c.high |= po.high;
@@ -972,6 +992,13 @@
         } else if (c.in_kept == 2u && c.s_open < c.kept_end) {
             c.in_kept = 1u; c.pos = c.s_open = c.tb; c.t = 0; c.ev_a = c.ev_b = c.a_usage = 0; c.primed = 0; c.last_ra = R2_NONE;
             continue;
+        }
+        {
+            const TailOut to = tail_event(c.a, sh, io_of(c), lane, c.seg, c.in_kept == 0u && have_dflt ? c.ready : 0u, c.dflt, c.s_open, sub_end);
+            c.high |= to.high;
+            if (to.kind == 2u) { mark_irregular(c); return false; }
+            if (to.kind == 3u) { c.pos = sub_end; continue; }
+            if (to.kind == 1u) { c.pos = c.s_open = to.e + 2u; c.t = 0; c.last_ra = R2_NONE; continue; }
         }
         {
             const OddOut oo = odd_event(c.a, sh, io_of(c), lane, c.seg, c.tb, c.s_open, sub_end, c.in_kept == 1u ? 1u : 0u, c.primed, have_dflt ? c.dflt : R2_NONE);
@@ -1085,7 +1112,7 @@
     const StreamHdr st = a.t.state[slot].h;
     SegPlan p;
     p.seg_end = a.chunk_off[c1]; p.relay_begin = p.seg_end; p.irregular = 0; p.last_usage = 0; p.a_usage = 0;
-    p.n_events_a = p.n_events_b = p.n_usage_b = 0; p.tail_start = 0xFFFFFFFFu; p.cand_ps = 0;
+    p.n_events_a = p.n_events_b = p.n_usage_b = 0; p.tail_start = 0xFFFFFFFFu; p.n_tails = 0;
     p.kept_chunk = 0xFFFFFFFFu; p.kept_end = 0; p.prime_ok = 0;
     p.resume_chunk = c0; p.emit_chunk_begin = (st.phase == PH_COMMITTED) ? c0 : c1;
     if (st.phase == PH_COMMITTED && c0 < c1) {
@@ -1128,10 +1155,57 @@
     st.flags |= SF_REC_VALID; ++st.n_usage_b;
     if (io.rec->exotic) { ++st.n_exotic; st.flags |= SF_EXOTIC_SEEN; }
 }
+#if !R2_HOST_EMU
+R2_DEV uint4 commit_ld16(const uint8_t* p) { return __ldg(reinterpret_cast<const uint4*>(p)); }
+#else
+R2_DEV uint4 commit_ld16(const uint8_t* p) { uint4 v; memcpy(&v, p, 16); return v; }
+#endif
 struct TextReader {
     const uint8_t* text; uint32_t base, n;
     R2_MEM uint32_t at(uint32_t p) const { return p - base < n ? (uint32_t)text[p - base] : 0u; }
+    R2_MEM uint32_t cls(uint32_t ch) const { return lean_tables().cls[ch]; }
+    R2_MEM uint32_t trans(uint32_t i) const { return lean_tables().trans[i]; }
 };
+R2_DEV void stage_text(uint8_t* stage, const uint8_t* d, uint32_t n_bytes, uint32_t ps, uint32_t n, uint32_t lane) {
+    const uint32_t ab = ps & ~15u, nvec = ((ps & 15u) + n + 15u) >> 4;
+    const bool d_aligned = (reinterpret_cast<uintptr_t>(d) & 15u) == 0u;
+    __syncwarp();
+    for (uint32_t k = lane; k < nvec; k += 32) {
+        const uint32_t o = ab + (k << 4);
+        if (o + 16u <= n_bytes && d_aligned) *reinterpret_cast<uint4*>(stage + (k << 4)) = commit_ld16(d + o);
+        else for (uint32_t j = 0; j < 16u && o + j < n_bytes; ++j) stage[(k << 4) + j] = __ldg(d + o + j);
+    }
+    __syncwarp();
+}
+
+struct Judged { uint32_t cls, f, slot, f_start, f_word; };
+R2_DEV_NOINLINE Judged commit_judge(TemplateCache2* tc, TextReader rd, uint32_t lane, uint32_t ps, uint32_t e, uint32_t count) {
+    Judged j; j.cls = PC_NONE; j.f = 0; j.slot = R2_NONE; j.f_start = 0; j.f_word = 0xFFFFFFFFu;
+    const uint32_t ready = __ballot_sync(R2_FULL, lane < R2_SLOTS && tc->state[lane] == 2u);
+    for (uint32_t slot = 0; slot < R2_SLOTS; ++slot) {
+        if (!(ready & (1u << slot))) continue;
+        const Tpl2* tp = &tc->tpl[slot];
+        if (head_differs(rd, tp, lane, ps, e + 2u)) continue;
+        const SingleOut so = match_single(rd, tp, lane, ps, e + 2u);
+        if (!so.ok || so.e != e) continue;
+        j.cls = tp->m.cls; j.f = tp->m.flags; j.slot = slot;
+        if (lane < 8u && tp->m.field_span[lane] != 0xffu) { j.f_start = so.f_start; j.f_word = so.f_len | (so.f_esc << 31); }
+        if (lane == 0 && count) atomicAdd(&tc->hits[slot], 1u);
+        return j;
+    }
+    if (lane == 0) {
+        const uint32_t c0 = rd.at(ps);
+        if (c0 == '{') j.cls = PC_BRACE;
+        else if (c0 == 'd' && rd.at(ps + 1) == 'a' && rd.at(ps + 2) == 't' && rd.at(ps + 3) == 'a' && rd.at(ps + 4) == ':' && rd.at(ps + 5) == ' ' && rd.at(ps + 6) == '{') j.cls = PC_DATA;
+        if (j.cls != PC_NONE) {
+            j.f = lean_parse(rd, ps + (j.cls == PC_DATA ? 6u : 0u), e, j.cls == PC_DATA);
+            if (count) atomicAdd(&tc->general, 1u);
+        }
+    }
+    j.cls = __shfl_sync(R2_FULL, j.cls, 0); j.f = __shfl_sync(R2_FULL, j.f, 0);
+    return j;
+}
+
 R2_DEV_NOINLINE void commit_usage_fields(const uint8_t* text, uint32_t ups, uint32_t ulen, uint32_t full_flags, const UsageRaw* tpl_raw, UsageRaw* raw, UsageRec* cand, uint32_t lane,
                                          uint32_t f_start, uint32_t f_word) {
     TextReader rd{text, ups, ulen};
@@ -1182,11 +1256,6 @@
 }
 
 R2_DEV_NOINLINE void commit_settle_pending(StepIO io) { resolve_pending(io); }
-#if !R2_HOST_EMU
-R2_DEV uint4 commit_ld16(const uint8_t* p) { return __ldg(reinterpret_cast<const uint4*>(p)); }
-#else
-R2_DEV uint4 commit_ld16(const uint8_t* p) { uint4 v; memcpy(&v, p, 16); return v; }
-#endif
 
 R2_GLOBAL void
 #if !R2_HOST_EMU
@@ -1218,31 +1287,47 @@
     const bool any_empty = __any_sync(R2_FULL, empty);
     griddep_wait();
     const SegPlan p = a.s.plan[seg];
+    const uint2 tl = lane < R2_TAILS ? a.s.tails[(size_t)seg * R2_TAILS + lane] : make_uint2(0u, 0u);
     const StepIO io = make_io(a, slot, &st);
     uint32_t emit_begin = p.emit_chunk_begin;
     const bool speculated = p.kept_chunk != 0xFFFFFFFFu;
     if ((st.phase == PH_COMMITTED || st.phase == PH_PRIMING) && p.resume_chunk < c1) {
         const uint8_t* __restrict__ d = a.data;
-        const uint32_t ups = (uint32_t)(p.last_usage >> 32) - 1u, ulen = (uint32_t)p.last_usage;
-        const bool staged = p.last_usage && ulen <= LGW_PENDING_CAP && (uint64_t)ups + ulen <= a.n_bytes;
-        const bool has_cand = staged && p.cand_ps == ups + 1u;
-        uint2 fld = make_uint2(0u, 0xFFFFFFFFu), gf = make_uint2(0u, 0u);
-        if (has_cand) { const uint2* uf = a.s.usage_fields + (size_t)seg * 9u; if (lane < 8u) fld = uf[lane]; gf = uf[8]; }
-        const uint32_t ab = ups & ~15u, skew = ups - ab;
-        const bool d_aligned = (reinterpret_cast<uintptr_t>(d) & 15u) == 0u;
-        const uint8_t* const utext = stage[warp] + skew;
-        if (staged) {
-            const uint32_t nvec = (skew + ulen + 15u) >> 4;
-            for (uint32_t k = lane; k < nvec; k += 32) {
-                const uint32_t o = ab + (k << 4);
-                if (o + 16u <= a.n_bytes && d_aligned) *reinterpret_cast<uint4*>(stage[warp] + (k << 4)) = commit_ld16(d + o);
-                else for (uint32_t j = 0; j < 16u && o + j < a.n_bytes; ++j) stage[warp][(k << 4) + j] = __ldg(d + o + j);
-            }
-        }
+        TemplateCache2* tc = a.s.tpl_cache2;
         bool sequential = p.irregular || p.n_usage_b > 1 || any_empty;
         if (st.phase == PH_PRIMING && !(speculated && p.prime_ok)) sequential = true;
-        if (!sequential && p.last_usage && !staged) sequential = true;
         if (!sequential && p.tail_start == 0xFFFFFFFFu) sequential = true;
+        const uint32_t n_tails = p.n_tails < R2_TAILS ? p.n_tails : R2_TAILS;
+        uint32_t ev_a = 0, ev_b = 0, a_usage = 0, n_usage = p.n_usage_b, judged = 0, judged_ps = R2_NONE;
+        unsigned long long last = p.last_usage;
+        Judged ju; ju.cls = PC_NONE; ju.f = 0; ju.slot = R2_NONE; ju.f_start = 0; ju.f_word = 0xFFFFFFFFu;
+        for (uint32_t i = 0; i < n_tails && !sequential; ++i) {
+            const uint32_t ps = __shfl_sync(R2_FULL, tl.x, (int)i), e = __shfl_sync(R2_FULL, tl.y, (int)i);
+            if (e - ps > LGW_PENDING_CAP || (uint64_t)e + 2u > a.n_bytes) { sequential = true; break; }
+            stage_text(stage[warp], d, a.n_bytes, ps, e + 2u - ps, lane);
+            ju = commit_judge(tc, TextReader{stage[warp] + (ps & 15u), ps, e + 2u - ps}, lane, ps, e, 1u);
+            judged_ps = ps; ++judged;
+            if (ju.cls == PC_NONE) continue;
+            if (ju.cls == PC_DATA) { ++ev_a; if ((ju.f & PF_VALID_A) && !(ju.f & TK_CODE) && (ju.f & TK_USAGE)) a_usage = 1; }
+            if (ju.f & PF_VALID_B) {
+                ++ev_b;
+                if (ju.f & TK_ERROR) { sequential = true; break; }
+                if (ju.f & TK_USAGE) {
+                    ++n_usage;
+                    const unsigned long long key = ((unsigned long long)(ps + 1u) << 32) | (e - ps);
+                    if (key > last) last = key;
+                }
+            }
+        }
+        if (lane == 0 && judged) atomicAdd(a.s.counters + 4, judged);
+        if (n_usage > 1) sequential = true;
+        const uint32_t ups = (uint32_t)(last >> 32) - 1u, ulen = (uint32_t)last;
+        if (!sequential && last && (ulen > LGW_PENDING_CAP || (uint64_t)ups + ulen + 2u > a.n_bytes)) sequential = true;
+        if (!sequential && last && judged_ps != ups) {
+            stage_text(stage[warp], d, a.n_bytes, ups, ulen + 2u, lane);
+            ju = commit_judge(tc, TextReader{stage[warp] + (ups & 15u), ups, ulen + 2u}, lane, ups, ups + ulen, 0u);
+        }
+        const uint8_t* const utext = stage[warp] + (ups & 15u);
         if (lane == 0) atomicAdd(a.s.counters + (sequential ? 0 : 1), 1u);
         if (sequential) {
             if (lane == 0) emit_begin = commit_sequential(io, a.data, a.chunk_off, p.resume_chunk, c1, (st.phase == PH_COMMITTED) ? p.resume_chunk : c1);
@@ -1257,13 +1342,14 @@
             }
             const uint32_t nch = c1 - first, nby = p.seg_end - p.relay_begin;
             st.n_chunks_in += nch; st.n_chunks_emitted += nch; st.bytes_in += nby; st.bytes_emitted += nby;
-            st.n_events_a += p.n_events_a; st.n_events_b += p.n_events_b;
-            if (p.a_usage) st.flags |= SF_A_USAGE_BOUND;
-            if (p.last_usage) {
+            st.n_events_a += p.n_events_a + ev_a; st.n_events_b += p.n_events_b + ev_b;
+            if (p.a_usage || a_usage) st.flags |= SF_A_USAGE_BOUND;
+            if (last) {
                 if (lane == 0 && (st.flags & SF_PENDING)) commit_settle_pending(io);
                 __syncwarp();
-                if (has_cand) {
-                    commit_usage_fields(utext, ups, ulen, gf.y, &a.s.tpl_cache2->raw[gf.x], &stage_raw[warp], io.rec, lane, fld.x, fld.y);
+                const Tpl2* tp = ju.slot != R2_NONE ? &tc->tpl[ju.slot] : nullptr;
+                if (tp && (tp->m.flags & TK_USAGE) && (tp->m.flags & PF_VALID_B) && tp->m.usage_ok) {
+                    commit_usage_fields(utext, ups, ulen, tp->m.full_flags, &tc->raw[ju.slot], &stage_raw[warp], io.rec, lane, ju.f_start, ju.f_word);
                     __syncwarp();
                     st.flags |= SF_REC_VALID; ++st.n_usage_b;
                     if (io.rec->exotic) { ++st.n_exotic; st.flags |= SF_EXOTIC_SEEN; }
diff --git a/llmapigateway_b200/csrc/sse_kernels.cuh b/llmapigateway_b200/csrc/sse_kernels.cuh
--- a/llmapigateway_b200/csrc/sse_kernels.cuh
+++ b/llmapigateway_b200/csrc/sse_kernels.cuh
@@ -59,7 +59,7 @@
     if ((r = cudaMalloc((void**)&s.tpl_cache2, sizeof(TemplateCache2))) != cudaSuccess) return r;
     if ((r = cudaMemset(s.tpl_cache2, 0, sizeof(TemplateCache2))) != cudaSuccess) return r;
     (void)sm_count;
-    if ((r = cudaMalloc((void**)&s.usage_fields, max_streams * 9 * sizeof(uint2))) != cudaSuccess) return r;
+    if ((r = cudaMalloc((void**)&s.tails, max_streams * R2_TAILS * sizeof(uint2))) != cudaSuccess) return r;
     if ((r = cudaMalloc((void**)&s.tile_seg, (max_bytes / R2_TILE + 4) * 4)) != cudaSuccess) return r;
     if ((r = cudaMemset(s.tile_seg, 0, (max_bytes / R2_TILE + 4) * 4)) != cudaSuccess) return r;
     if ((r = cudaMalloc((void**)&s.counters, 64)) != cudaSuccess) return r;
@@ -68,8 +68,8 @@
     return cudaSuccess;
 }
 static inline void scratch_free(StepScratch& s) {
-    cudaFree(s.plan); cudaFree(s.tpl_cache2); cudaFree(s.usage_fields); cudaFree(s.counters); s.counters = nullptr; cudaFree(s.tile_seg); s.tile_seg = nullptr;
-    s.plan = nullptr; s.tpl_cache2 = nullptr; s.usage_fields = nullptr;
+    cudaFree(s.plan); cudaFree(s.tpl_cache2); cudaFree(s.tails); cudaFree(s.counters); s.counters = nullptr; cudaFree(s.tile_seg); s.tile_seg = nullptr;
+    s.plan = nullptr; s.tpl_cache2 = nullptr; s.tails = nullptr;
 }
 
 static inline cudaError_t launch_step(const StepArgs& a, int mode, int sm_count, cudaStream_t stream, cudaEvent_t* ev, int* launched, bool per_kernel) {
diff --git a/llmapigateway_b200/csrc/step_types.cuh b/llmapigateway_b200/csrc/step_types.cuh
--- a/llmapigateway_b200/csrc/step_types.cuh
+++ b/llmapigateway_b200/csrc/step_types.cuh
@@ -23,7 +23,7 @@
     uint32_t kept_end;
     uint32_t prime_ok;
     uint32_t tail_start;
-    uint32_t cand_ps;
+    uint32_t n_tails;
 };
 static_assert(sizeof(SegPlan) == 64, "SegPlan");
 
@@ -32,7 +32,10 @@
 struct StepScratch {
     SegPlan* plan;
     TemplateCache2* tpl_cache2;
-    uint2* usage_fields;
+    union {
+        uint2* tails;
+        uint2* usage_fields;
+    };
     uint32_t* tile_seg;
     uint32_t* counters;
 };
diff --git a/llmapigateway_b200/engine.py b/llmapigateway_b200/engine.py
--- a/llmapigateway_b200/engine.py
+++ b/llmapigateway_b200/engine.py
@@ -191,9 +191,9 @@
         self._ck(self._lib.lgw_engine_set_kernel_timing(self._h, 1 if on else 0), "set_kernel_timing")
 
     def debug_counters(self):
-        out = (C.c_uint32 * 4)()
+        out = (C.c_uint32 * 5)()
         self._ck(self._lib.lgw_debug_counters(self._h, out), "debug_counters")
-        return dict(sequential=out[0], bulk=out[1], from_template=out[2], stashed=out[3])
+        return dict(sequential=out[0], bulk=out[1], from_template=out[2], stashed=out[3], tail_deferred=out[4])
 
     def launch_count(self) -> int:
         n = C.c_uint64(0)
```

Result: faster. 16.03 billion, median of 6 (+1.7%).
